# r-barnes/richdem

Hardware: NVIDIA H100
Metric: Priority-Flood fill + D8 flow accumulation throughput (higher is better)
Workload: dtype f32

## Files before the change

### include/richdem_b200.h

```cpp
#ifndef RICHDEM_B200_H_
#define RICHDEM_B200_H_

#include <stdint.h>

#ifdef __cplusplus
extern "C" {
#endif

#define RDB200_VERSION 100

#if defined(__GNUC__)
#define RDB200_API __attribute__((visibility("default")))
#else
#define RDB200_API
#endif


RDB200_API int rdb200_init(int device);
RDB200_API void rdb200_shutdown(void);
RDB200_API const char *rdb200_last_error(void);
RDB200_API int rdb200_version(void);

RDB200_API int rdb200_set_stream(void *cuda_stream);

typedef struct rdb200_stats {
  int64_t cells;
  int64_t kernel_launches;
  int64_t fill_rounds;
  int64_t fill_tile_visits;
  int64_t fill_tile_cells;
  int64_t fill_tile_iters;
  int64_t accum_rounds;
  int64_t flat_bfs_levels;
  int64_t flat_cells_raised;
  double ms_total;
  double ms_main_kernel;
  double ms_h2d, ms_d2h;
} rdb200_stats;
RDB200_API int rdb200_get_stats(rdb200_stats *out);

RDB200_API int rdb200_set_param(const char *name, int64_t value);


RDB200_API int rdb200_fill_depressions_d8_f32(float *dem, int32_t width, int32_t height);

RDB200_API int rdb200_fill_depressions_d4_f32(float *dem, int32_t width, int32_t height);

RDB200_API int rdb200_pit_mask_d8_f32(const float *dem, uint8_t *mask, int32_t width, int32_t height, float nodata);
RDB200_API int rdb200_pit_mask_d4_f32(const float *dem, uint8_t *mask, int32_t width, int32_t height, float nodata);

RDB200_API int rdb200_has_depressions_d8_f32(const float *dem, int32_t width, int32_t height, int32_t *out);
RDB200_API int rdb200_has_depressions_d4_f32(const float *dem, int32_t width, int32_t height, int32_t *out);

RDB200_API int rdb200_resolve_flats_epsilon_f32(float *dem, int32_t width, int32_t height, float nodata);

RDB200_API int rdb200_get_flat_mask_f32(const float *dem, int32_t *flat_mask, int32_t *labels, int32_t width,
                             int32_t height, float nodata);

RDB200_API int rdb200_d8_flow_directions_f32(const float *dem, uint8_t *flowdirs, int32_t width,
                                  int32_t height, float nodata);

RDB200_API int rdb200_d8_flow_directions_flats_f32(float *dem, uint8_t *flowdirs, int32_t width, int32_t height,
                                                   float nodata, int32_t alter);

RDB200_API int rdb200_d8_flow_accum_u8_i32(const uint8_t *flowdirs, int32_t *area, int32_t width,
                                int32_t height);

RDB200_API int rdb200_fm_d8_f32(const float *dem, float *props9, int32_t width, int32_t height, float nodata);

RDB200_API int rdb200_fm_tarboton_f32(const float *dem, float *props9, int32_t width, int32_t height,
                           float nodata);

RDB200_API int rdb200_fm_d4_f32(const float *dem, float *props9, int32_t width, int32_t height, float nodata);
RDB200_API int rdb200_fm_quinn_f32(const float *dem, float *props9, int32_t width, int32_t height, float nodata);
RDB200_API int rdb200_fm_holmgren_f32(const float *dem, float *props9, int32_t width, int32_t height, float nodata,
                                      double xparam);
RDB200_API int rdb200_fm_freeman_f32(const float *dem, float *props9, int32_t width, int32_t height, float nodata,
                                     double xparam);

RDB200_API int rdb200_fa_d4_f32_f64(const float *dem, double *accum_inout, int32_t width, int32_t height, float nodata);
RDB200_API int rdb200_fa_quinn_f32_f64(const float *dem, double *accum_inout, int32_t width, int32_t height,
                                       float nodata);
RDB200_API int rdb200_fa_holmgren_f32_f64(const float *dem, double *accum_inout, int32_t width, int32_t height,
                                          float nodata, double xparam);
RDB200_API int rdb200_fa_freeman_f32_f64(const float *dem, double *accum_inout, int32_t width, int32_t height,
                                         float nodata, double xparam);

RDB200_API int rdb200_fill_depressions_d8_f64(double *dem, int32_t width, int32_t height);
RDB200_API int rdb200_fill_depressions_d4_f64(double *dem, int32_t width, int32_t height);
RDB200_API int rdb200_pit_mask_d8_f64(const double *dem, uint8_t *mask, int32_t width, int32_t height, double nodata);
RDB200_API int rdb200_pit_mask_d4_f64(const double *dem, uint8_t *mask, int32_t width, int32_t height, double nodata);
RDB200_API int rdb200_has_depressions_d8_f64(const double *dem, int32_t width, int32_t height, int32_t *out);
RDB200_API int rdb200_has_depressions_d4_f64(const double *dem, int32_t width, int32_t height, int32_t *out);
RDB200_API int rdb200_resolve_flats_epsilon_f64(double *dem, int32_t width, int32_t height, double nodata);
RDB200_API int rdb200_d8_flow_directions_f64(const double *dem, uint8_t *flowdirs, int32_t width, int32_t height,
                                             double nodata);
RDB200_API int rdb200_fa_d8_f64_f64(const double *dem, double *accum_inout, int32_t width, int32_t height, double nodata,
                                    int32_t accum_is_ones);
RDB200_API int rdb200_fa_d4_f64_f64(const double *dem, double *accum_inout, int32_t width, int32_t height, double nodata);
RDB200_API int rdb200_f64_order_keys(const double *dem, float *keys, int32_t width, int32_t height, double nodata,
                                     float *nodata_key, int32_t *ranked);

enum {
  RDB200_TA_SLOPE_RISERUN = 0,
  RDB200_TA_SLOPE_PERCENTAGE = 1,
  RDB200_TA_SLOPE_DEGREES = 2,
  RDB200_TA_SLOPE_RADIANS = 3,
  RDB200_TA_ASPECT = 4,
  RDB200_TA_CURVATURE = 5,
  RDB200_TA_PLANFORM_CURVATURE = 6,
  RDB200_TA_PROFILE_CURVATURE = 7
};
RDB200_API int rdb200_terrain_attribute_f32(int32_t attribute, const float *dem, float *out, int32_t width, int32_t height,
                                            float nodata_in, float nodata_out, float zscale, double cell_x, double cell_y);

RDB200_API int rdb200_flow_accumulation_props_f64(const float *props9, double *accum_inout, int32_t width,
                                       int32_t height);

RDB200_API int rdb200_fa_d8_f32_f64(const float *dem, double *accum_inout, int32_t width, int32_t height,
                         float nodata, int32_t accum_is_ones);
RDB200_API int rdb200_fa_tarboton_f32_f64(const float *dem, double *accum_inout, int32_t width,
                               int32_t height, float nodata, int32_t accum_is_ones);


RDB200_API int rdb200_dev_fill_depressions_d8_f32(float *d_dem, int32_t width, int32_t height);
RDB200_API int rdb200_dev_fill_depressions_d4_f32(float *d_dem, int32_t width, int32_t height);
RDB200_API int rdb200_dev_pit_mask_d8_f32(const float *d_dem, uint8_t *d_mask, int32_t width, int32_t height, float nodata);
RDB200_API int rdb200_dev_pit_mask_d4_f32(const float *d_dem, uint8_t *d_mask, int32_t width, int32_t height, float nodata);
RDB200_API int rdb200_dev_has_depressions_d8_f32(const float *d_dem, int32_t width, int32_t height, int32_t *out);
RDB200_API int rdb200_dev_has_depressions_d4_f32(const float *d_dem, int32_t width, int32_t height, int32_t *out);
RDB200_API int rdb200_dev_resolve_flats_epsilon_f32(float *d_dem, int32_t width, int32_t height, float nodata);
RDB200_API int rdb200_dev_d8_flow_directions_f32(const float *d_dem, uint8_t *d_flowdirs, int32_t width,
                                      int32_t height, float nodata);
RDB200_API int rdb200_dev_d8_flow_directions_flats_f32(float *d_dem, uint8_t *d_flowdirs, int32_t width, int32_t height,
                                                       float nodata, int32_t alter);
RDB200_API int rdb200_dev_d8_flow_accum_u8_i32(const uint8_t *d_flowdirs, int32_t *d_area, int32_t width,
                                    int32_t height);
RDB200_API int rdb200_dev_fm_d8_f32(const float *d_dem, float *d_props9, int32_t width, int32_t height,
                         float nodata);
RDB200_API int rdb200_dev_fm_tarboton_f32(const float *d_dem, float *d_props9, int32_t width, int32_t height,
                               float nodata);
RDB200_API int rdb200_dev_fm_method_f32(int32_t method, const float *d_dem, float *d_props9, int32_t width,
                                        int32_t height, float nodata, double xparam);
RDB200_API int rdb200_dev_fa_method_f32_f64(int32_t method, const float *d_dem, double *d_accum_inout, int32_t width,
                                            int32_t height, float nodata, double xparam);
RDB200_API int rdb200_dev_terrain_attribute_f32(int32_t attribute, const float *d_dem, float *d_out, int32_t width,
                                                int32_t height, float nodata_in, float nodata_out, float zscale,
                                                double cell_x, double cell_y);
RDB200_API int rdb200_dev_flow_accumulation_props_f64(const float *d_props9, double *d_accum_inout,
                                           int32_t width, int32_t height);
RDB200_API int rdb200_dev_fa_d8_f32_f64(const float *d_dem, double *d_accum_inout, int32_t width,
                             int32_t height, float nodata, int32_t accum_is_ones);
RDB200_API int rdb200_dev_fa_tarboton_f32_f64(const float *d_dem, double *d_accum_inout, int32_t width,
                                   int32_t height, float nodata, int32_t accum_is_ones);
RDB200_API int rdb200_dev_fill_depressions_d8_f64(double *d_dem, int32_t width, int32_t height);
RDB200_API int rdb200_dev_fill_depressions_d4_f64(double *d_dem, int32_t width, int32_t height);
RDB200_API int rdb200_dev_pit_mask_d8_f64(const double *d_dem, uint8_t *d_mask, int32_t width, int32_t height, double nodata);
RDB200_API int rdb200_dev_pit_mask_d4_f64(const double *d_dem, uint8_t *d_mask, int32_t width, int32_t height, double nodata);
RDB200_API int rdb200_dev_has_depressions_d8_f64(const double *d_dem, int32_t width, int32_t height, int32_t *out);
RDB200_API int rdb200_dev_has_depressions_d4_f64(const double *d_dem, int32_t width, int32_t height, int32_t *out);
RDB200_API int rdb200_dev_resolve_flats_epsilon_f64(double *d_dem, int32_t width, int32_t height, double nodata);
RDB200_API int rdb200_dev_d8_flow_directions_f64(const double *d_dem, uint8_t *d_flowdirs, int32_t width, int32_t height,
                                                 double nodata);
RDB200_API int rdb200_dev_fa_d8_f64_f64(const double *d_dem, double *d_accum_inout, int32_t width, int32_t height,
                                        double nodata, int32_t accum_is_ones);
RDB200_API int rdb200_dev_fa_d4_f64_f64(const double *d_dem, double *d_accum_inout, int32_t width, int32_t height,
                                        double nodata);
RDB200_API int rdb200_dev_f64_order_keys(const double *d_dem, float *d_keys, int32_t width, int32_t height, double nodata,
                                         float *nodata_key, int32_t *ranked);

RDB200_API int rdb200_dev_generate_fbm_f32(float *d_dem, int32_t width, int32_t height, int32_t y0,
                                uint32_t seed, int32_t octaves, float quantum);

typedef struct rdb200_comm rdb200_comm;
enum { RDB200_MAX_F32 = 0, RDB200_MIN_F32 = 1, RDB200_MAX_I32 = 2, RDB200_SUM_I32 = 3 };
typedef int (*rdb200_exchange_fn)(void *user, const void *send_up, void *recv_up, const void *send_dn, void *recv_dn,
                                  size_t bytes);
typedef int (*rdb200_allreduce_fn)(void *user, void *buf, size_t count, int op);
RDB200_API int rdb200_nccl_unique_id(uint8_t *out128);
RDB200_API int rdb200_comm_create_nccl(rdb200_comm **comm, int32_t rank, int32_t world, const uint8_t *id128);
RDB200_API int rdb200_comm_create_callbacks(rdb200_comm **comm, int32_t rank, int32_t world, void *user,
                                            rdb200_exchange_fn exchange, rdb200_allreduce_fn allreduce);
RDB200_API int rdb200_comm_destroy(rdb200_comm *comm);

RDB200_API int rdb200_mgpu_fill_depressions_d8_f32(const rdb200_comm *comm, float *d_band, int32_t width, int32_t local_rows,
                                                   int32_t ghost_top, int32_t ghost_bottom, int32_t row0, int32_t height,
                                                   int32_t *exchange_rounds);
RDB200_API int rdb200_mgpu_fill_depressions_d4_f32(const rdb200_comm *comm, float *d_band, int32_t width, int32_t local_rows,
                                                   int32_t ghost_top, int32_t ghost_bottom, int32_t row0, int32_t height,
                                                   int32_t *exchange_rounds);
RDB200_API int rdb200_mgpu_pit_mask_d8_f32(const rdb200_comm *comm, const float *d_band, uint8_t *d_band_mask, int32_t width,
                                           int32_t local_rows, float nodata, int32_t ghost_top, int32_t ghost_bottom, int32_t row0,
                                           int32_t height);
RDB200_API int rdb200_mgpu_pit_mask_d4_f32(const rdb200_comm *comm, const float *d_band, uint8_t *d_band_mask, int32_t width,
                                           int32_t local_rows, float nodata, int32_t ghost_top, int32_t ghost_bottom, int32_t row0,
                                           int32_t height);
RDB200_API int rdb200_mgpu_has_depressions_d8_f32(const rdb200_comm *comm, const float *d_band, int32_t width, int32_t local_rows,
                                                  int32_t ghost_top, int32_t ghost_bottom, int32_t row0, int32_t height,
                                                  int32_t *out);
RDB200_API int rdb200_mgpu_has_depressions_d4_f32(const rdb200_comm *comm, const float *d_band, int32_t width, int32_t local_rows,
                                                  int32_t ghost_top, int32_t ghost_bottom, int32_t row0, int32_t height,
                                                  int32_t *out);
RDB200_API int rdb200_mgpu_resolve_flats_epsilon_f32(const rdb200_comm *comm, float *d_band, int32_t width, int32_t local_rows,
                                                     float nodata, int32_t ghost_top, int32_t ghost_bottom,
                                                     int32_t *seam_iterations);
RDB200_API int rdb200_mgpu_fa_f32_f64(const rdb200_comm *comm, const float *d_band_dem, double *d_band_accum_inout,
                                      int32_t width, int32_t local_rows, float nodata, int32_t ghost_top,
                                      int32_t ghost_bottom, int32_t dinf, int32_t accum_is_ones, int32_t *exchange_rounds);
RDB200_API int rdb200_mgpu_fa_method_f32_f64(const rdb200_comm *comm, const float *d_band_dem, double *d_band_accum_inout,
                                             int32_t width, int32_t local_rows, float nodata, int32_t ghost_top,
                                             int32_t ghost_bottom, int32_t method, double xparam, int32_t accum_is_ones,
                                             int32_t *exchange_rounds);
RDB200_API int rdb200_mgpu_d8_flow_directions_flats_f32(const rdb200_comm *comm, float *d_band_dem, uint8_t *d_band_dirs,
                                                        int32_t width, int32_t local_rows, float nodata, int32_t ghost_top,
                                                        int32_t ghost_bottom, int32_t alter, int32_t *seam_iterations);
RDB200_API int rdb200_mgpu_d8_flow_accum_u8_i32(const rdb200_comm *comm, const uint8_t *d_band_dirs, int32_t *d_band_area,
                                                int32_t width, int32_t local_rows, int32_t ghost_top, int32_t ghost_bottom,
                                                int32_t *exchange_rounds);
RDB200_API int rdb200_mgpu_fm_method_f32(const rdb200_comm *comm, int32_t method, float *d_band_dem, float *d_band_props9,
                                         int32_t width, int32_t local_rows, float nodata, int32_t ghost_top, int32_t ghost_bottom,
                                         double xparam);
RDB200_API int rdb200_mgpu_terrain_attribute_f32(const rdb200_comm *comm, int32_t attribute, float *d_band_dem, float *d_band_out,
                                                 int32_t width, int32_t local_rows, float nodata_in, float nodata_out, float zscale,
                                                 double cell_x, double cell_y, int32_t ghost_top, int32_t ghost_bottom);
RDB200_API int rdb200_mgpu_flow_accumulation_props_f64(const rdb200_comm *comm, float *d_band_props9, double *d_band_accum_inout,
                                                       int32_t width, int32_t local_rows, int32_t ghost_top, int32_t ghost_bottom,
                                                       int32_t *exchange_rounds);

typedef struct rdb200_fill_state rdb200_fill_state;
RDB200_API int rdb200_dev_fill_begin(rdb200_fill_state **state, const float *d_dem, int32_t width,
                          int32_t height);
RDB200_API int rdb200_dev_fill_begin_lifted(rdb200_fill_state **state, const float *d_dem, int32_t width, int32_t height,
                                 const float *d_coarse, int32_t coarse_width, int32_t pool, int32_t row_offset);
RDB200_API int rdb200_dev_fill_blockmax(rdb200_fill_state *state, float *d_blockmax, int32_t coarse_width, int32_t coarse_height,
                             int32_t pool, int32_t row_offset, int32_t skip_top, int32_t skip_bottom);
RDB200_API int rdb200_dev_fill_relax_from_f32(const float *d_dem, float *d_w_inout, int32_t width, int32_t height);
RDB200_API int rdb200_dev_fill_prolong(rdb200_fill_state *state, const float *d_coarse, int32_t coarse_width, int32_t pool,
                            int32_t row_offset, int32_t *tiles_lowered);
RDB200_API int rdb200_dev_maxpool_rows_f32(const float *d_src, int32_t width, int32_t height, int32_t row_offset, int32_t pool,
                                float *d_coarse, int32_t coarse_width, int32_t coarse_height);
RDB200_API int rdb200_dev_fill_run(rdb200_fill_state *state, int32_t *changed_rows);
RDB200_API int rdb200_dev_fill_read_row(rdb200_fill_state *state, int32_t y, float *d_row);
RDB200_API int rdb200_dev_fill_update_row(rdb200_fill_state *state, int32_t y, const float *d_row);
RDB200_API int rdb200_dev_fill_finish(rdb200_fill_state *state, float *d_out);

typedef struct rdb200_facc_state rdb200_facc_state;
RDB200_API int rdb200_dev_facc_begin(rdb200_facc_state **state, const float *d_dem, double *d_accum_inout,
                                     int32_t width, int32_t height, float nodata, int32_t ghost_top,
                                     int32_t ghost_bottom, int32_t dinf, int32_t accum_is_ones);
RDB200_API int rdb200_dev_facc_begin_method(rdb200_facc_state **state, const float *d_dem, double *d_accum_inout,
                                            int32_t width, int32_t height, float nodata, int32_t ghost_top,
                                            int32_t ghost_bottom, int32_t method, double xparam, int32_t accum_is_ones);
RDB200_API int rdb200_dev_facc_get_edge_codes(rdb200_facc_state *state, int32_t which, uint8_t *d_code_row,
                                              float *d_rmax_row);
RDB200_API int rdb200_dev_facc_set_ghost_codes(rdb200_facc_state *state, int32_t which,
                                               const uint8_t *d_code_row, const float *d_rmax_row);
RDB200_API int rdb200_dev_facc_run(rdb200_facc_state *state, int32_t *sent_top, int32_t *sent_bottom);
RDB200_API int rdb200_dev_facc_take_outflow(rdb200_facc_state *state, int32_t which, double *d_sum_row,
                                            int32_t *d_cnt_row);
RDB200_API int rdb200_dev_facc_apply_inflow(rdb200_facc_state *state, int32_t which, const double *d_sum_row,
                                            const int32_t *d_cnt_row);
RDB200_API int rdb200_dev_facc_finish(rdb200_facc_state *state);

typedef struct rdb200_flats_state rdb200_flats_state;
RDB200_API int rdb200_dev_flats_begin(rdb200_flats_state **state, float *d_dem, int32_t width, int32_t height,
                                      float nodata, int32_t ghost_top, int32_t ghost_bottom);
RDB200_API int rdb200_dev_flats_arrays(rdb200_flats_state *state, uint64_t *out6);
RDB200_API int rdb200_dev_flats_edges(rdb200_flats_state *state);
RDB200_API int rdb200_dev_flats_components(rdb200_flats_state *state);
RDB200_API int rdb200_dev_flats_labels(rdb200_flats_state *state);
RDB200_API int rdb200_dev_flats_gradient_begin(rdb200_flats_state *state, int32_t away,
                                               rdb200_fill_state **dist_state);
RDB200_API int rdb200_dev_flats_gradient_end(rdb200_flats_state *state, int32_t away,
                                             rdb200_fill_state *dist_state);
RDB200_API int rdb200_dev_flats_apply(rdb200_flats_state *state);
RDB200_API int rdb200_dev_flats_finish(rdb200_flats_state *state);

#ifdef __cplusplus
}
#endif
#endif
```

### richdem_b200/_lib.py

```python
from __future__ import annotations

import ctypes as C
import os

import numpy as np

_HERE = os.path.dirname(os.path.abspath(__file__))
LIB_PATH = os.environ.get("RICHDEM_B200_LIB") or os.path.join(_HERE, "librichdem_b200.so")

_lib = None


class RichdemB200Error(RuntimeError):
    """Raised for any non-zero status from the C ABI (mirrors the std::runtime_error ->
    RuntimeError translation pybind11 does for the reference, pywrapper.hpp:109-123)."""


class Stats(C.Structure):
    _fields_ = [
        ("cells", C.c_int64), ("kernel_launches", C.c_int64), ("fill_rounds", C.c_int64),
        ("fill_tile_visits", C.c_int64), ("fill_tile_cells", C.c_int64), ("fill_tile_iters", C.c_int64),
        ("accum_rounds", C.c_int64), ("flat_bfs_levels", C.c_int64), ("flat_cells_raised", C.c_int64),
        ("ms_total", C.c_double), ("ms_main_kernel", C.c_double), ("ms_h2d", C.c_double),
        ("ms_d2h", C.c_double),
    ]

    def as_dict(self):
        return {k: getattr(self, k) for k, _ in self._fields_}


_i32, _f32, _f64, _vp = C.c_int32, C.c_float, C.c_double, C.c_void_p
SIGNATURES = {
    "rdb200_init": [C.c_int],
    "rdb200_set_stream": [C.c_void_p],
    "rdb200_get_stats": [C.POINTER(Stats)],
    "rdb200_set_param": [C.c_char_p, C.c_int64],
    "rdb200_fill_depressions_d8_f32": [_vp, _i32, _i32],
    "rdb200_fill_depressions_d4_f32": [_vp, _i32, _i32],
    "rdb200_dev_fill_depressions_d4_f32": [_vp, _i32, _i32],
    "rdb200_pit_mask_d8_f32": [_vp, _vp, _i32, _i32, _f32],
    "rdb200_pit_mask_d4_f32": [_vp, _vp, _i32, _i32, _f32],
    "rdb200_has_depressions_d8_f32": [_vp, _i32, _i32, C.POINTER(_i32)],
    "rdb200_has_depressions_d4_f32": [_vp, _i32, _i32, C.POINTER(_i32)],
    "rdb200_dev_pit_mask_d8_f32": [_vp, _vp, _i32, _i32, _f32],
    "rdb200_dev_pit_mask_d4_f32": [_vp, _vp, _i32, _i32, _f32],
    "rdb200_dev_has_depressions_d8_f32": [_vp, _i32, _i32, C.POINTER(_i32)],
    "rdb200_dev_has_depressions_d4_f32": [_vp, _i32, _i32, C.POINTER(_i32)],
    "rdb200_mgpu_pit_mask_d8_f32": [_vp, _vp, _vp, _i32, _i32, _f32, _i32, _i32, _i32, _i32],
    "rdb200_mgpu_pit_mask_d4_f32": [_vp, _vp, _vp, _i32, _i32, _f32, _i32, _i32, _i32, _i32],
    "rdb200_mgpu_has_depressions_d8_f32": [_vp, _vp, _i32, _i32, _i32, _i32, _i32, _i32, C.POINTER(_i32)],
    "rdb200_mgpu_has_depressions_d4_f32": [_vp, _vp, _i32, _i32, _i32, _i32, _i32, _i32, C.POINTER(_i32)],
    "rdb200_resolve_flats_epsilon_f32": [_vp, _i32, _i32, _f32],
    "rdb200_get_flat_mask_f32": [_vp, _vp, _vp, _i32, _i32, _f32],
    "rdb200_d8_flow_directions_f32": [_vp, _vp, _i32, _i32, _f32],
    "rdb200_d8_flow_directions_flats_f32": [_vp, _vp, _i32, _i32, _f32, _i32],
    "rdb200_dev_d8_flow_directions_flats_f32": [_vp, _vp, _i32, _i32, _f32, _i32],
    "rdb200_d8_flow_accum_u8_i32": [_vp, _vp, _i32, _i32],
    "rdb200_fm_d8_f32": [_vp, _vp, _i32, _i32, _f32],
    "rdb200_fm_tarboton_f32": [_vp, _vp, _i32, _i32, _f32],
    "rdb200_fm_d4_f32": [_vp, _vp, _i32, _i32, _f32],
    "rdb200_fm_quinn_f32": [_vp, _vp, _i32, _i32, _f32],
    "rdb200_fm_holmgren_f32": [_vp, _vp, _i32, _i32, _f32, C.c_double],
    "rdb200_fm_freeman_f32": [_vp, _vp, _i32, _i32, _f32, C.c_double],
    "rdb200_terrain_attribute_f32": [_i32, _vp, _vp, _i32, _i32, _f32, _f32, _f32, C.c_double, C.c_double],
    "rdb200_dev_terrain_attribute_f32": [_i32, _vp, _vp, _i32, _i32, _f32, _f32, _f32, C.c_double, C.c_double],
    "rdb200_fa_d4_f32_f64": [_vp, _vp, _i32, _i32, _f32],
    "rdb200_fa_quinn_f32_f64": [_vp, _vp, _i32, _i32, _f32],
    "rdb200_fa_holmgren_f32_f64": [_vp, _vp, _i32, _i32, _f32, C.c_double],
    "rdb200_fa_freeman_f32_f64": [_vp, _vp, _i32, _i32, _f32, C.c_double],
    "rdb200_dev_fm_method_f32": [_i32, _vp, _vp, _i32, _i32, _f32, C.c_double],
    "rdb200_dev_fa_method_f32_f64": [_i32, _vp, _vp, _i32, _i32, _f32, C.c_double],
    "rdb200_flow_accumulation_props_f64": [_vp, _vp, _i32, _i32],
    "rdb200_fa_d8_f32_f64": [_vp, _vp, _i32, _i32, _f32, _i32],
    "rdb200_fa_tarboton_f32_f64": [_vp, _vp, _i32, _i32, _f32, _i32],
    "rdb200_dev_fill_depressions_d8_f32": [_vp, _i32, _i32],
    "rdb200_dev_resolve_flats_epsilon_f32": [_vp, _i32, _i32, _f32],
    "rdb200_dev_d8_flow_directions_f32": [_vp, _vp, _i32, _i32, _f32],
    "rdb200_dev_d8_flow_accum_u8_i32": [_vp, _vp, _i32, _i32],
    "rdb200_dev_fm_d8_f32": [_vp, _vp, _i32, _i32, _f32],
    "rdb200_dev_fm_tarboton_f32": [_vp, _vp, _i32, _i32, _f32],
    "rdb200_dev_flow_accumulation_props_f64": [_vp, _vp, _i32, _i32],
    "rdb200_dev_fa_d8_f32_f64": [_vp, _vp, _i32, _i32, _f32, _i32],
    "rdb200_dev_fa_tarboton_f32_f64": [_vp, _vp, _i32, _i32, _f32, _i32],
    "rdb200_fill_depressions_d8_f64": [_vp, _i32, _i32],
    "rdb200_fill_depressions_d4_f64": [_vp, _i32, _i32],
    "rdb200_pit_mask_d8_f64": [_vp, _vp, _i32, _i32, _f64],
    "rdb200_pit_mask_d4_f64": [_vp, _vp, _i32, _i32, _f64],
    "rdb200_has_depressions_d8_f64": [_vp, _i32, _i32, C.POINTER(_i32)],
    "rdb200_has_depressions_d4_f64": [_vp, _i32, _i32, C.POINTER(_i32)],
    "rdb200_resolve_flats_epsilon_f64": [_vp, _i32, _i32, _f64],
    "rdb200_d8_flow_directions_f64": [_vp, _vp, _i32, _i32, _f64],
    "rdb200_fa_d8_f64_f64": [_vp, _vp, _i32, _i32, _f64, _i32],
    "rdb200_fa_d4_f64_f64": [_vp, _vp, _i32, _i32, _f64],
    "rdb200_f64_order_keys": [_vp, _vp, _i32, _i32, _f64, C.POINTER(_f32), C.POINTER(_i32)],
    "rdb200_dev_fill_depressions_d8_f64": [_vp, _i32, _i32],
    "rdb200_dev_fill_depressions_d4_f64": [_vp, _i32, _i32],
    "rdb200_dev_pit_mask_d8_f64": [_vp, _vp, _i32, _i32, _f64],
    "rdb200_dev_pit_mask_d4_f64": [_vp, _vp, _i32, _i32, _f64],
    "rdb200_dev_has_depressions_d8_f64": [_vp, _i32, _i32, C.POINTER(_i32)],
    "rdb200_dev_has_depressions_d4_f64": [_vp, _i32, _i32, C.POINTER(_i32)],
    "rdb200_dev_resolve_flats_epsilon_f64": [_vp, _i32, _i32, _f64],
    "rdb200_dev_d8_flow_directions_f64": [_vp, _vp, _i32, _i32, _f64],
    "rdb200_dev_fa_d8_f64_f64": [_vp, _vp, _i32, _i32, _f64, _i32],
    "rdb200_dev_fa_d4_f64_f64": [_vp, _vp, _i32, _i32, _f64],
    "rdb200_dev_f64_order_keys": [_vp, _vp, _i32, _i32, _f64, C.POINTER(_f32), C.POINTER(_i32)],
    "rdb200_dev_generate_fbm_f32": [_vp, _i32, _i32, _i32, C.c_uint32, _i32, _f32],
    "rdb200_nccl_unique_id": [_vp],
    "rdb200_comm_create_nccl": [C.POINTER(_vp), _i32, _i32, _vp],
    "rdb200_comm_create_callbacks": [C.POINTER(_vp), _i32, _i32, _vp, _vp, _vp],
    "rdb200_comm_destroy": [_vp],
    "rdb200_mgpu_fill_depressions_d8_f32": [_vp, _vp, _i32, _i32, _i32, _i32, _i32, _i32, C.POINTER(_i32)],
    "rdb200_mgpu_fill_depressions_d4_f32": [_vp, _vp, _i32, _i32, _i32, _i32, _i32, _i32, C.POINTER(_i32)],
    "rdb200_mgpu_fa_f32_f64": [_vp, _vp, _vp, _i32, _i32, _f32, _i32, _i32, _i32, _i32, C.POINTER(_i32)],
    "rdb200_mgpu_fa_method_f32_f64": [_vp, _vp, _vp, _i32, _i32, _f32, _i32, _i32, _i32, C.c_double, _i32, C.POINTER(_i32)],
    "rdb200_mgpu_resolve_flats_epsilon_f32": [_vp, _vp, _i32, _i32, _f32, _i32, _i32, C.POINTER(_i32)],
    "rdb200_mgpu_d8_flow_directions_flats_f32": [_vp, _vp, _vp, _i32, _i32, _f32, _i32, _i32, _i32, C.POINTER(_i32)],
    "rdb200_mgpu_d8_flow_accum_u8_i32": [_vp, _vp, _vp, _i32, _i32, _i32, _i32, C.POINTER(_i32)],
    "rdb200_mgpu_fm_method_f32": [_vp, _i32, _vp, _vp, _i32, _i32, _f32, _i32, _i32, C.c_double],
    "rdb200_mgpu_terrain_attribute_f32": [_vp, _i32, _vp, _vp, _i32, _i32, _f32, _f32, _f32, C.c_double, C.c_double, _i32, _i32],
    "rdb200_mgpu_flow_accumulation_props_f64": [_vp, _vp, _vp, _i32, _i32, _i32, _i32, C.POINTER(_i32)],
    "rdb200_dev_fill_begin": [C.POINTER(_vp), _vp, _i32, _i32],
    "rdb200_dev_fill_begin_lifted": [C.POINTER(_vp), _vp, _i32, _i32, _vp, _i32, _i32, _i32],
    "rdb200_dev_maxpool_rows_f32": [_vp, _i32, _i32, _i32, _i32, _vp, _i32, _i32],
    "rdb200_dev_fill_blockmax": [_vp, _vp, _i32, _i32, _i32, _i32, _i32, _i32],
    "rdb200_dev_fill_relax_from_f32": [_vp, _vp, _i32, _i32],
    "rdb200_dev_fill_prolong": [_vp, _vp, _i32, _i32, _i32, C.POINTER(C.c_int32)],
    "rdb200_dev_fill_run": [_vp, C.POINTER(_i32)],
    "rdb200_dev_fill_read_row": [_vp, _i32, _vp],
    "rdb200_dev_fill_update_row": [_vp, _i32, _vp],
    "rdb200_dev_fill_finish": [_vp, _vp],
    "rdb200_dev_facc_begin": [C.POINTER(_vp), _vp, _vp, _i32, _i32, _f32, _i32, _i32, _i32, _i32],
    "rdb200_dev_facc_begin_method": [C.POINTER(_vp), _vp, _vp, _i32, _i32, _f32, _i32, _i32, _i32, C.c_double, _i32],
    "rdb200_dev_facc_get_edge_codes": [_vp, _i32, _vp, _vp],
    "rdb200_dev_facc_set_ghost_codes": [_vp, _i32, _vp, _vp],
    "rdb200_dev_facc_run": [_vp, C.POINTER(_i32), C.POINTER(_i32)],
    "rdb200_dev_facc_take_outflow": [_vp, _i32, _vp, _vp],
    "rdb200_dev_facc_apply_inflow": [_vp, _i32, _vp, _vp],
    "rdb200_dev_facc_finish": [_vp],
    "rdb200_dev_flats_begin": [C.POINTER(_vp), _vp, _i32, _i32, _f32, _i32, _i32],
    "rdb200_dev_flats_arrays": [_vp, C.POINTER(C.c_uint64)],
    "rdb200_dev_flats_edges": [_vp],
    "rdb200_dev_flats_components": [_vp],
    "rdb200_dev_flats_labels": [_vp],
    "rdb200_dev_flats_gradient_begin": [_vp, _i32, C.POINTER(_vp)],
    "rdb200_dev_flats_gradient_end": [_vp, _i32, _vp],
    "rdb200_dev_flats_apply": [_vp],
    "rdb200_dev_flats_finish": [_vp],
}
OTHER_SYMBOLS = ["rdb200_shutdown", "rdb200_last_error", "rdb200_version"]


def lib():
    global _lib
    if _lib is None:
        if not os.path.exists(LIB_PATH):
            raise RichdemB200Error(
                f"{LIB_PATH} not found: build it with `python -m richdem_b200.build` "
                "(there is no CPU fallback)")
        L = C.CDLL(LIB_PATH)
        if hasattr(L, "rdb200_emulated"):
            raise RichdemB200Error(
                f"{LIB_PATH} is the CPU kernel-emulation test build, not librichdem_b200 "
                "(there is no CPU fallback)")
        for name, argtypes in SIGNATURES.items():
            f = getattr(L, name)
            f.argtypes = argtypes
            f.restype = C.c_int
        L.rdb200_last_error.restype = C.c_char_p
        L.rdb200_last_error.argtypes = []
        L.rdb200_version.restype = C.c_int
        L.rdb200_shutdown.restype = None
        _lib = L
        for kv in filter(None, os.environ.get("RDB200_PARAMS", "").split(",")):
            k, _, v = kv.partition("=")
            if L.rdb200_set_param(k.strip().encode(), int(v)):
                msg = L.rdb200_last_error()
                raise RichdemB200Error(f"RDB200_PARAMS: {msg.decode('utf-8', 'replace') if msg else kv}")
    return _lib


def check(rc: int) -> None:
    if rc != 0:
        msg = lib().rdb200_last_error()
        raise RichdemB200Error(msg.decode("utf-8", "replace") if msg else f"librichdem_b200 error {rc}")


def ptr(a: np.ndarray) -> int:
    return a.ctypes.data


def stats() -> dict:
    s = Stats()
    check(lib().rdb200_get_stats(C.byref(s)))
    return s.as_dict()


_param_values: dict = {}


def set_param(name: str, value: int) -> None:
    check(lib().rdb200_set_param(name.encode(), int(value)))
    if name == "reset_defaults":
        _param_values.clear()
    elif name != "trim_workspace":
        _param_values[name] = int(value)


def reset_params() -> None:
    set_param("reset_defaults", 1)


class scoped_param:

    def __init__(self, name: str, value: int, default: int = 0):
        self.name, self.value, self.default = name, int(value), int(default)

    def __enter__(self):
        self.previous = _param_values.get(self.name)
        set_param(self.name, self.value)
        return self

    def __exit__(self, *exc):
        if self.previous is None:
            set_param(self.name, self.default)
            _param_values.pop(self.name, None)
        else:
            set_param(self.name, self.previous)
        return False


def init(device: int = 0) -> None:
    check(lib().rdb200_init(int(device)))


def set_stream(cuda_stream) -> None:
    if cuda_stream is None:
        check(lib().rdb200_set_stream(C.c_void_p(None)))
    else:
        h = int(cuda_stream)
        check(lib().rdb200_set_stream(C.c_void_p(h if h != 0 else 1)))


def use_torch_stream() -> None:
    import torch
    set_stream(torch.cuda.current_stream().cuda_stream)


def shutdown() -> None:
    lib().rdb200_shutdown()
```

### richdem_b200/csrc/capi.cu

```cuda
#include "common.cuh"

#include <algorithm>
#include <cstdlib>

namespace rdb {

static thread_local std::string g_last_error;

void capi_set_error(const char *msg) { g_last_error = msg ? msg : "unknown error"; }

Ctx &ctx() {
  static Ctx c;
  return c;
}

static void init_device(int device) {
  Ctx &c = ctx();
  if (c.inited && c.device == device) return;
  if (c.inited) fail("rdb200_init: already initialised on device %d (call rdb200_shutdown first)", c.device);
  int ndev = 0;
  cudaError_t e = cudaGetDeviceCount(&ndev);
  if (e != cudaSuccess || ndev == 0)
    fail("no CUDA device available (%s); librichdem_b200 has no CPU fallback",
         e == cudaSuccess ? "device count is 0" : cudaGetErrorString(e));
  if (device < 0 || device >= ndev) fail("rdb200_init: device %d out of range (0..%d)", device, ndev - 1);
  RDB_CK(cudaSetDevice(device));
  cudaDeviceProp prop;
  RDB_CK(cudaGetDeviceProperties(&prop, device));
  if (prop.major != 9 || prop.minor != 0)
    fail("device %d is sm_%d%d; librichdem_b200 is built for sm_90a (H100) only", device, prop.major,
         prop.minor);
  c.device = device;
  c.num_sms = prop.multiProcessorCount;
  RDB_CK(cudaStreamCreate(&c.own_stream));
  c.stream = c.own_stream;
  RDB_CK(cudaEventCreate(&c.ev0));
  RDB_CK(cudaEventCreate(&c.ev1));
  RDB_CK(cudaEventCreate(&c.evk0));
  RDB_CK(cudaEventCreate(&c.evk1));
  c.pinned_bytes = 1 << 16;
  RDB_CK(cudaMallocHost(&c.pinned, c.pinned_bytes));
  memset(&c.stats, 0, sizeof(c.stats));
  c.inited = true;
}

void ensure_init() {
  Ctx &c = ctx();
  if (c.inited) {
    RDB_CK(cudaSetDevice(c.device));
    return;
  }
  int dev = 0;
  cudaError_t e = cudaGetDevice(&dev);
  if (e != cudaSuccess) dev = 0;
  init_device(dev);
}

void *ws_alloc(size_t bytes) {
  Ctx &c = ctx();
  bytes = (bytes + 511) & ~(size_t)511;
  int best = -1;
  for (int i = 0; i < (int)c.ws.size(); i++)
    if (!c.ws[i].in_use && c.ws[i].bytes >= bytes && (best < 0 || c.ws[i].bytes < c.ws[best].bytes)) best = i;
  if (best >= 0 && c.ws[best].bytes <= bytes + bytes / 4 + (1 << 20)) {
    c.ws[best].in_use = true;
    return c.ws[best].ptr;
  }
  void *p = nullptr;
  cudaError_t e = cudaMalloc(&p, bytes);
  if (e != cudaSuccess) {
    cudaGetLastError();
    for (auto it = c.ws.begin(); it != c.ws.end();) {
      if (!it->in_use) {
        cudaFree(it->ptr);
        it = c.ws.erase(it);
      } else {
        ++it;
      }
    }
    e = cudaMalloc(&p, bytes);
    if (e != cudaSuccess) fail("cudaMalloc(%zu bytes) failed: %s", bytes, cudaGetErrorString(e));
  }
  c.ws.push_back({p, bytes, true});
  return p;
}

void ws_free(void *p) {
  for (auto &b : ctx().ws)
    if (b.ptr == p) {
      b.in_use = false;
      return;
    }
}

void ws_trim() {
  Ctx &c = ctx();
  for (auto it = c.ws.begin(); it != c.ws.end();) {
    if (!it->in_use) {
      cudaFree(it->ptr);
      it = c.ws.erase(it);
    } else {
      ++it;
    }
  }
}

void ws_release_all() {
  Ctx &c = ctx();
  for (auto &b : c.ws) cudaFree(b.ptr);
  c.ws.clear();
}

struct CallScope {
  explicit CallScope(int64_t cells) {
    ensure_init();
    Ctx &c = ctx();
    memset(&c.stats, 0, sizeof(c.stats));
    c.stats.cells = cells;
    RDB_CK(cudaEventRecord(c.ev0, c.stream));
  }
  void done() {
    Ctx &c = ctx();
    RDB_CK(cudaEventRecord(c.ev1, c.stream));
    RDB_CK(cudaStreamSynchronize(c.stream));
    float ms = 0;
    RDB_CK(cudaEventElapsedTime(&ms, c.ev0, c.ev1));
    c.stats.ms_total = ms;
  }
};

static void check_dims(int w, int h) {
  if (w <= 0 || h <= 0) fail("raster dimensions must be positive (got %d x %d)", w, h);
  if ((int64_t)w * h > ((int64_t)1 << 31) - ((int64_t)1 << 25))
    fail("rasters above 2^31 - 2^25 cells per GPU are not supported (got %d x %d); shard by rows", w, h);
}

template <class T>
static void h2d(T *dst, const T *src, size_t n) {
  Ctx &c = ctx();
  cudaEvent_t a = c.evk0, b = c.evk1;
  RDB_CK(cudaEventRecord(a, c.stream));
  RDB_CK(cudaMemcpyAsync(dst, src, n * sizeof(T), cudaMemcpyHostToDevice, c.stream));
  RDB_CK(cudaEventRecord(b, c.stream));
  RDB_CK(cudaStreamSynchronize(c.stream));
  float ms = 0;
  RDB_CK(cudaEventElapsedTime(&ms, a, b));
  c.stats.ms_h2d += ms;
}
template <class T>
static void d2h(T *dst, const T *src, size_t n) {
  Ctx &c = ctx();
  cudaEvent_t a = c.evk0, b = c.evk1;
  RDB_CK(cudaEventRecord(a, c.stream));
  RDB_CK(cudaMemcpyAsync(dst, src, n * sizeof(T), cudaMemcpyDeviceToHost, c.stream));
  RDB_CK(cudaEventRecord(b, c.stream));
  RDB_CK(cudaStreamSynchronize(c.stream));
  float ms = 0;
  RDB_CK(cudaEventElapsedTime(&ms, a, b));
  c.stats.ms_d2h += ms;
}

}

using namespace rdb;

#define CAPI_TRY try {
#define CAPI_END                    \
  }                                 \
  catch (const std::exception &e) { \
    capi_set_error(e.what());       \
    return 1;                       \
  }                                 \
  catch (...) {                     \
    capi_set_error("unknown C++ exception"); \
    return 1;                       \
  }                                 \
  return 0;

extern "C" {

int rdb200_init(int device) {
  CAPI_TRY
  init_device(device);
  CAPI_END
}

void rdb200_shutdown(void) {
  Ctx &c = ctx();
  if (!c.inited) return;
  cudaSetDevice(c.device);
  cudaStreamSynchronize(c.stream);
  ws_release_all();
  if (c.pinned) cudaFreeHost(c.pinned);
  cudaEventDestroy(c.ev0);
  cudaEventDestroy(c.ev1);
  cudaEventDestroy(c.evk0);
  cudaEventDestroy(c.evk1);
  cudaStreamDestroy(c.own_stream);
  for (int k = 0; k < 2; k++)
    if (c.aux_stream[k]) cudaStreamDestroy(c.aux_stream[k]);
  for (int k = 0; k < 3; k++)
    if (c.aux_event[k]) cudaEventDestroy(c.aux_event[k]);
  const Params keep = c.params;
  c = Ctx();
  c.params = keep;
}

const char *rdb200_last_error(void) { return g_last_error.c_str(); }
int rdb200_version(void) { return RDB200_VERSION; }

int rdb200_set_stream(void *cuda_stream) {
  CAPI_TRY
  ensure_init();
  Ctx &c = ctx();
  RDB_CK(cudaStreamSynchronize(c.stream));
  c.stream = cuda_stream ? (cudaStream_t)cuda_stream : c.own_stream;
  CAPI_END
}

int rdb200_get_stats(rdb200_stats *out) {
  CAPI_TRY
  if (!out) fail("rdb200_get_stats: null pointer");
  *out = ctx().stats;
  CAPI_END
}

int rdb200_set_param(const char *name, int64_t value) {
  CAPI_TRY
  if (!name) fail("rdb200_set_param: null name");
  Params &p = ctx().params;
  const std::string n(name);
  if (n == "reset_defaults") p = Params();
  else if (n == "trim_workspace") {
    if (ctx().inited) {
      RDB_CK(cudaStreamSynchronize(ctx().stream));
      ws_trim();
    }
  }
  else if (n == "fill_max_iters") p.fill_max_iters = value;
  else if (n == "fill_rounds_per_sync") p.fill_rounds_per_sync = value > 0 ? value : 16;
  else if (n == "fill_use_tma") p.fill_use_tma = value;
  else if (n == "fill_external_z") p.fill_external_z = value;
  else if (n == "fill_profile") p.fill_profile = value;
  else if (n == "fill_wake_filter") p.fill_wake_filter = value;
  else if (n == "fill_trace") p.fill_trace = value;
  else if (n == "fill_ordered") p.fill_ordered = value;
  else if (n == "fill_order_rounds") p.fill_order_rounds = value;
  else if (n == "fill_band_rounds") p.fill_band_rounds = value;
  else if (n == "accum_threads") p.accum_threads = value > 0 ? value : 256;
  else if (n == "accum_budget") p.accum_budget = value;
  else if (n == "accum_walk_lanes") p.accum_walk_lanes = value;
  else if (n == "accum_fused_prep") p.accum_fused_prep = value;
  else if (n == "flats_tiled") p.flats_tiled = value;
  else if (n == "flats_pair") p.flats_pair = value;
  else if (n == "flats_fused_classify") p.flats_fused_classify = value;
  else if (n == "fill_multigrid") p.fill_multigrid = value;
  else if (n == "fill_multigrid_min") p.fill_multigrid_min = value;
  else if (n == "fill_vcycle") p.fill_vcycle = value;
  else if (n == "fill_band_multigrid") p.fill_band_multigrid = value;
  else if (n == "flats_uf_tiled") p.flats_uf_tiled = value;
  else if (n == "flowdirs_rolling") p.flowdirs_rolling = value;
  else if (n == "accum_packed") p.accum_packed = value;
  else if (n == "accum_dinf_packed") p.accum_dinf_packed = value;
  else if (n == "accum_dinf_share") p.accum_dinf_share = value;
  else if (n == "flowmet_tarboton_filter") p.flowmet_tarboton_filter = value;
  else if (n == "accum_walk_scan") p.accum_walk_scan = value;
  else if (n == "accum_walk_ahead") p.accum_walk_ahead = value;
  else if (n == "accum_dinf_stats") p.accum_dinf_stats = value;
  else if (n == "accum_dinf_wait") p.accum_dinf_wait = value;
  else fail("rdb200_set_param: unknown parameter '%s'", name);
  CAPI_END
}


int rdb200_fill_depressions_d8_f32(float *dem, int32_t w, int32_t h) {
  CAPI_TRY
  if (!dem) fail("fill_depressions: null dem");
  check_dims(w, h);
  CallScope cs((int64_t)w * h);
  const size_t n = (size_t)w * h;
  DevBuf<float> d(n);
  h2d(d.p, dem, n);
  fill_depressions_dev(d.p, w, h);
  d2h(dem, d.p, n);
  cs.done();
  CAPI_END
}

int rdb200_fill_depressions_d4_f32(float *dem, int32_t w, int32_t h) {
  CAPI_TRY
  if (!dem) fail("fill_depressions: null dem");
  check_dims(w, h);
  CallScope cs((int64_t)w * h);
  const size_t n = (size_t)w * h;
  DevBuf<float> d(n);
  h2d(d.p, dem, n);
  fill_depressions_dev(d.p, w, h, true);
  d2h(dem, d.p, n);
  cs.done();
  CAPI_END
}

static int pit_mask_host(const float *dem, uint8_t *mask, int32_t w, int32_t h, float nodata, bool topo4) {
  CAPI_TRY
  if (!dem || !mask) fail("pit_mask: null pointer");
  check_dims(w, h);
  CallScope cs((int64_t)w * h);
  const size_t n = (size_t)w * h;
  DevBuf<float> d(n);
  DevBuf<uint8_t> m(n);
  h2d(d.p, dem, n);
  pit_mask_dev(d.p, m.p, w, h, nodata, topo4);
  d2h(mask, m.p, n);
  cs.done();
  CAPI_END
}
int rdb200_pit_mask_d8_f32(const float *dem, uint8_t *mask, int32_t w, int32_t h, float nodata) {
  return pit_mask_host(dem, mask, w, h, nodata, false);
}
int rdb200_pit_mask_d4_f32(const float *dem, uint8_t *mask, int32_t w, int32_t h, float nodata) {
  return pit_mask_host(dem, mask, w, h, nodata, true);
}

static int has_depressions_host(const float *dem, int32_t w, int32_t h, int32_t *out, bool topo4) {
  CAPI_TRY
  if (!dem || !out) fail("has_depressions: null pointer");
  check_dims(w, h);
  CallScope cs((int64_t)w * h);
  const size_t n = (size_t)w * h;
  DevBuf<float> d(n);
  h2d(d.p, dem, n);
  const bool any = has_depressions_dev(d.p, w, h, topo4);
  cs.done();
  *out = any ? 1 : 0;
  CAPI_END
}
int rdb200_has_depressions_d8_f32(const float *dem, int32_t w, int32_t h, int32_t *out) {
  return has_depressions_host(dem, w, h, out, false);
}
int rdb200_has_depressions_d4_f32(const float *dem, int32_t w, int32_t h, int32_t *out) {
  return has_depressions_host(dem, w, h, out, true);
}

int rdb200_resolve_flats_epsilon_f32(float *dem, int32_t w, int32_t h, float nodata) {
  CAPI_TRY
  if (!dem) fail("resolve_flats: null dem");
  check_dims(w, h);
  CallScope cs((int64_t)w * h);
  const size_t n = (size_t)w * h;
  DevBuf<float> d(n);
  h2d(d.p, dem, n);
  resolve_flats_dev(d.p, w, h, nodata, nullptr, nullptr, true);
  d2h(dem, d.p, n);
  cs.done();
  CAPI_END
}

int rdb200_get_flat_mask_f32(const float *dem, int32_t *flat_mask, int32_t *labels, int32_t w, int32_t h,
                             float nodata) {
  CAPI_TRY
  if (!dem || !flat_mask || !labels) fail("get_flat_mask: null pointer");
  check_dims(w, h);
  CallScope cs((int64_t)w * h);
  const size_t n = (size_t)w * h;
  DevBuf<float> d(n);
  DevBuf<int32_t> m(n), l(n);
  h2d(d.p, dem, n);
  resolve_flats_dev(d.p, w, h, nodata, m.p, l.p, false);
  d2h(flat_mask, m.p, n);
  d2h(labels, l.p, n);
  cs.done();
  CAPI_END
}

int rdb200_d8_flow_directions_f32(const float *dem, uint8_t *dirs, int32_t w, int32_t h, float nodata) {
  CAPI_TRY
  if (!dem || !dirs) fail("d8_flow_directions: null pointer");
  check_dims(w, h);
  CallScope cs((int64_t)w * h);
  const size_t n = (size_t)w * h;
  DevBuf<float> d(n);
  DevBuf<uint8_t> o(n);
  h2d(d.p, dem, n);
  d8_flow_directions_dev(d.p, o.p, w, h, nodata);
  d2h(dirs, o.p, n);
  cs.done();
  CAPI_END
}

int rdb200_d8_flow_directions_flats_f32(float *dem, uint8_t *dirs, int32_t w, int32_t h, float nodata, int32_t alter) {
  CAPI_TRY
  if (!dem || !dirs) fail("d8_flow_directions_flats: null pointer");
  check_dims(w, h);
  CallScope cs((int64_t)w * h);
  const size_t n = (size_t)w * h;
  DevBuf<float> d(n);
  DevBuf<uint8_t> o(n);
  h2d(d.p, dem, n);
  d8_flow_directions_flats_dev(d.p, o.p, w, h, nodata, alter != 0);
  d2h(dirs, o.p, n);
  if (alter) d2h(dem, d.p, n);
  cs.done();
  CAPI_END
}

int rdb200_d8_flow_accum_u8_i32(const uint8_t *dirs, int32_t *area, int32_t w, int32_t h) {
  CAPI_TRY
  if (!dirs || !area) fail("d8_flow_accum: null pointer");
  check_dims(w, h);
  CallScope cs((int64_t)w * h);
  const size_t n = (size_t)w * h;
  DevBuf<uint8_t> d(n);
  DevBuf<int32_t> o(n);
  h2d(d.p, dirs, n);
  d8_flow_accum_dev(d.p, o.p, w, h);
  d2h(area, o.p, n);
  cs.done();
  CAPI_END
}

static void fm_dispatch_dev(int method, const float *d_dem, float *d_props, int w, int h, float nodata, double xparam) {
  switch (method) {
    case 0: fm_d8_dev(d_dem, d_props, w, h, nodata); break;
    case 1: fm_tarboton_dev(d_dem, d_props, w, h, nodata); break;
    case 2: fm_d4_dev(d_dem, d_props, w, h, nodata); break;
    case 3: fm_holmgren_dev(d_dem, d_props, w, h, nodata, xparam); break;
    case 4: fm_freeman_dev(d_dem, d_props, w, h, nodata, xparam); break;
    default: fail("unknown flow metric %d", method);
  }
}

static int fm_host(const float *dem, float *props, int32_t w, int32_t h, float nodata, int method, double xparam = 0) {
  CAPI_TRY
  if (!dem || !props) fail("flow metric: null pointer");
  check_dims(w, h);
  CallScope cs((int64_t)w * h);
  const size_t n = (size_t)w * h;
  DevBuf<float> d(n), p(9 * n);
  h2d(d.p, dem, n);
  fm_dispatch_dev(method, d.p, p.p, w, h, nodata, xparam);
  d2h(props, p.p, 9 * n);
  cs.done();
  CAPI_END
}
int rdb200_fm_d8_f32(const float *dem, float *props, int32_t w, int32_t h, float nodata) {
  return fm_host(dem, props, w, h, nodata, 0);
}
int rdb200_fm_tarboton_f32(const float *dem, float *props, int32_t w, int32_t h, float nodata) {
  return fm_host(dem, props, w, h, nodata, 1);
}
int rdb200_fm_d4_f32(const float *dem, float *props, int32_t w, int32_t h, float nodata) {
  return fm_host(dem, props, w, h, nodata, 2);
}
int rdb200_fm_quinn_f32(const float *dem, float *props, int32_t w, int32_t h, float nodata) {
  return fm_host(dem, props, w, h, nodata, 3, 1.0);
}
int rdb200_fm_holmgren_f32(const float *dem, float *props, int32_t w, int32_t h, float nodata, double xparam) {
  return fm_host(dem, props, w, h, nodata, 3, xparam);
}
int rdb200_fm_freeman_f32(const float *dem, float *props, int32_t w, int32_t h, float nodata, double xparam) {
  return fm_host(dem, props, w, h, nodata, 4, xparam);
}

int rdb200_terrain_attribute_f32(int32_t attribute, const float *dem, float *out, int32_t w, int32_t h, float nodata_in,
                                 float nodata_out, float zscale, double cell_x, double cell_y) {
  CAPI_TRY
  if (!dem || !out) fail("terrain attribute: null pointer");
  check_dims(w, h);
  CallScope cs((int64_t)w * h);
  const size_t n = (size_t)w * h;
  DevBuf<float> d(n), o(n);
  h2d(d.p, dem, n);
  terrain_attribute_dev(attribute, d.p, o.p, w, h, nodata_in, nodata_out, zscale, cell_x, cell_y);
  d2h(out, o.p, n);
  cs.done();
  CAPI_END
}

static void fa_via_props_dev(int method, const float *d_dem, double *d_accum, int w, int h, float nodata, double xparam) {
  DevBuf<float> p(9 * (size_t)w * h);
  fm_dispatch_dev(method, d_dem, p.p, w, h, nodata, xparam);
  flow_accumulation_props_dev(p.p, d_accum, w, h);
}
static int fa_via_props_host(int method, const float *dem, double *accum, int32_t w, int32_t h, float nodata, double xparam) {
  CAPI_TRY
  if (!dem || !accum) fail("flow accumulation: null pointer");
  check_dims(w, h);
  CallScope cs((int64_t)w * h);
  const size_t n = (size_t)w * h;
  DevBuf<float> d(n);
  DevBuf<double> a(n);
  h2d(d.p, dem, n);
  h2d(a.p, accum, n);
  fa_via_props_dev(method, d.p, a.p, w, h, nodata, xparam);
  d2h(accum, a.p, n);
  cs.done();
  CAPI_END
}
int rdb200_fa_d4_f32_f64(const float *dem, double *accum, int32_t w, int32_t h, float nodata) {
  return fa_via_props_host(2, dem, accum, w, h, nodata, 0);
}
int rdb200_fa_quinn_f32_f64(const float *dem, double *accum, int32_t w, int32_t h, float nodata) {
  return fa_via_props_host(3, dem, accum, w, h, nodata, 1.0);
}
int rdb200_fa_holmgren_f32_f64(const float *dem, double *accum, int32_t w, int32_t h, float nodata, double xparam) {
  return fa_via_props_host(3, dem, accum, w, h, nodata, xparam);
}
int rdb200_fa_freeman_f32_f64(const float *dem, double *accum, int32_t w, int32_t h, float nodata, double xparam) {
  return fa_via_props_host(4, dem, accum, w, h, nodata, xparam);
}

int rdb200_flow_accumulation_props_f64(const float *props, double *accum, int32_t w, int32_t h) {
  CAPI_TRY
  if (!props || !accum) fail("flow_accumulation: null pointer");
  check_dims(w, h);
  CallScope cs((int64_t)w * h);
  const size_t n = (size_t)w * h;
  DevBuf<float> p(9 * n);
  DevBuf<double> a(n);
  h2d(p.p, props, 9 * n);
  h2d(a.p, accum, n);
  flow_accumulation_props_dev(p.p, a.p, w, h);
  d2h(accum, a.p, n);
  cs.done();
  CAPI_END
}

static int fa_host(const float *dem, double *accum, int32_t w, int32_t h, float nodata, int32_t ones,
                   bool dinf) {
  CAPI_TRY
  if (!dem || !accum) fail("flow accumulation: null pointer");
  check_dims(w, h);
  CallScope cs((int64_t)w * h);
  const size_t n = (size_t)w * h;
  DevBuf<float> d(n);
  DevBuf<double> a(n);
  h2d(d.p, dem, n);
  if (!ones) h2d(a.p, accum, n);
  fa_fused_dev(d.p, a.p, w, h, nodata, ones != 0, dinf);
  d2h(accum, a.p, n);
  cs.done();
  CAPI_END
}
int rdb200_fa_d8_f32_f64(const float *dem, double *accum, int32_t w, int32_t h, float nodata, int32_t ones) {
  return fa_host(dem, accum, w, h, nodata, ones, false);
}
int rdb200_fa_tarboton_f32_f64(const float *dem, double *accum, int32_t w, int32_t h, float nodata,
// ... 487 lines not shown
```

### richdem_b200/csrc/common.cuh

```cuda
#pragma once

#include <cuda.h>
#include <cuda_runtime.h>

#include <cstdarg>
#include <cstdint>
#include <cstdio>
#include <cstring>
#include <stdexcept>
#include <string>
#include <vector>

#include "../../include/richdem_b200.h"

struct rdb200_fill_state;

namespace rdb {

struct Error : std::runtime_error {
  using std::runtime_error::runtime_error;
};

[[noreturn]] inline void fail(const char *fmt, ...) {
  char buf[1024];
  va_list ap;
  va_start(ap, fmt);
  vsnprintf(buf, sizeof(buf), fmt, ap);
  va_end(ap);
  throw Error(buf);
}

#define RDB_CK(expr)                                                                        \
  do {                                                                                      \
    cudaError_t _e = (expr);                                                                \
    if (_e != cudaSuccess)                                                                  \
      ::rdb::fail("%s failed at %s:%d: %s", #expr, __FILE__, __LINE__, cudaGetErrorString(_e)); \
  } while (0)

__host__ __device__ __forceinline__ int d8dx(int n) {
  return (int)((0x6a41u >> (2 * n)) & 3u) - 1;
}
__host__ __device__ __forceinline__ int d8dy(int n) {
  return (int)((0x2a405u >> (2 * n)) & 3u) - 1;
}

struct Params {
  int64_t fill_max_iters = 0;
  int64_t fill_rounds_per_sync = 16;
  int64_t fill_use_tma = 1;
  int64_t fill_external_z = 1;
  int64_t fill_ordered = 1;
  int64_t fill_order_rounds = 0;
  int64_t fill_band_rounds = 0;
  int64_t fill_profile = 0;
  int64_t fill_wake_filter = 1;
  int64_t fill_trace = 0;
  int64_t fill_multigrid = 8;
  int64_t fill_vcycle = 8;
  int64_t fill_band_multigrid = 0;
  int64_t fill_multigrid_min = 0;
  int64_t flowdirs_rolling = 1;
  int64_t flats_uf_tiled = 1;
  int64_t flats_fused_classify = 1;
  int64_t flats_pair = 1;
  int64_t flats_tiled = 1;
  int64_t accum_dinf_packed = 1;
  int64_t flowmet_tarboton_filter = 1;
  int64_t accum_walk_ahead = 0;
  int64_t accum_walk_scan = 0;
  int64_t accum_dinf_stats = 0;
  int64_t accum_dinf_share = -1;
  int64_t accum_dinf_wait = 0;
  int64_t accum_packed = 1;
  int64_t accum_fused_prep = 1;
  int64_t accum_walk_lanes = 1;
  int64_t accum_threads = 256;
  int64_t accum_budget = 0;
};

struct WsBlock {
  void *ptr;
  size_t bytes;
  bool in_use;
};

struct Ctx {
  bool inited = false;
  int device = -1;
  int num_sms = 0;
  cudaStream_t stream = nullptr;
  cudaStream_t own_stream = nullptr;
  cudaEvent_t ev0 = nullptr, ev1 = nullptr, evk0 = nullptr, evk1 = nullptr;
  cudaStream_t aux_stream[2] = {nullptr, nullptr};
  cudaEvent_t aux_event[3] = {nullptr, nullptr, nullptr};
  std::vector<WsBlock> ws;
  void *pinned = nullptr;
  size_t pinned_bytes = 0;
  rdb200_stats stats;
  Params params;
};

Ctx &ctx();
void ensure_init();
void *ws_alloc(size_t bytes);
void ws_free(void *p);
void ws_release_all();

template <class T>
struct DevBuf {
  T *p = nullptr;
  size_t n = 0;
  DevBuf() = default;
  explicit DevBuf(size_t count) { alloc(count); }
  void alloc(size_t count) {
    reset();
    n = count;
    p = (T *)ws_alloc((count ? count : 1) * sizeof(T));
  }
  void reset() {
    if (p) ws_free(p);
    p = nullptr;
    n = 0;
  }
  ~DevBuf() { reset(); }
  DevBuf(const DevBuf &) = delete;
  DevBuf &operator=(const DevBuf &) = delete;
  operator T *() const { return p; }
};

inline void count_launch(int64_t k = 1) { ctx().stats.kernel_launches += k; }

struct KernelTimer {
  bool active;
  explicit KernelTimer(bool on = true) : active(on) {
    if (active) RDB_CK(cudaEventRecord(ctx().evk0, ctx().stream));
  }
  void stop_async() {
    if (active) RDB_CK(cudaEventRecord(ctx().evk1, ctx().stream));
  }
  double ms() {
    float t = 0;
    if (active) RDB_CK(cudaEventElapsedTime(&t, ctx().evk0, ctx().evk1));
    return t;
  }
};

int comm_rank(const rdb200_comm *c);
int comm_world(const rdb200_comm *c);
void comm_exchange(const rdb200_comm *c, const void *send_up, void *recv_up, const void *send_dn, void *recv_dn, size_t bytes);
void comm_allreduce(const rdb200_comm *c, void *buf, size_t count, int op);
void check_band_args(const char *what, const rdb200_comm *comm, const void *d_band, int w, int hloc, int gt, int gb);
void exchange_band_rows(const rdb200_comm *comm, void *d_band, size_t elem, int w, int hloc, int gt, int gb);
void mgpu_fill_band(const rdb200_comm *comm, float *d_local, int w, int hloc, int gt, int gb, int row0, int H, int *xrounds,
                    bool topo4 = false);
void mgpu_fa_band(const rdb200_comm *comm, const float *d_dem, double *d_accum, int w, int hloc, float nodata, int gt, int gb,
                  int method, double xparam, bool ones, int *xrounds);
void mgpu_flow_accumulation_props_band(const rdb200_comm *comm, float *d_props, double *d_accum, int w, int hloc, int gt, int gb,
                                       int *xrounds);
void mgpu_resolve_flats_band(const rdb200_comm *comm, float *d_local, int w, int hloc, float nodata, int gt, int gb,
                             int *seam_iters);
void mgpu_d8_flow_directions_flats_band(const rdb200_comm *comm, float *d_dem, uint8_t *d_dirs, int w, int hloc, float nodata,
                                        int gt, int gb, bool alter, int *seam_iters);
void mgpu_d8_flow_accum_band(const rdb200_comm *comm, const uint8_t *d_dirs, int32_t *d_area, int w, int hloc, int gt, int gb,
                             int *xrounds);
int mgpu_relax_band(const rdb200_comm *comm, rdb200_fill_state *state, int gt, int gb, int R);

void fill_depressions_dev(float *d_dem, int w, int h, bool topo4 = false);
void geodesic_distance_dev(const uint8_t *d_open, int open_bit, float *d_w_inout, int w, int h);
void geodesic_distance_pair_dev(const uint8_t *d_open, int open_bit, float *d_wa, float *d_wb, int w, int h);
rdb200_fill_state *new_band_distance_state(const uint8_t *d_open, int open_bit, const float *d_winit, int w, int h,
                                           int ghost_top, int ghost_bottom);
void finish_band_distance_state(rdb200_fill_state *s, float *d_out);
void resolve_flats_dev(float *d_dem, int w, int h, float nodata, int32_t *d_mask_out,
                       int32_t *d_labels_out, bool apply, const uint8_t *d_dirs = nullptr);
void d8_flow_directions_flats_dev(float *d_dem, uint8_t *d_dirs, int w, int h, float nodata, bool alter);
void d8_flow_directions_dev(const float *d_dem, uint8_t *d_dirs, int w, int h, float nodata);
void d8_flow_accum_dev(const uint8_t *d_dirs, int32_t *d_area, int w, int h);
void fm_d8_dev(const float *d_dem, float *d_props, int w, int h, float nodata);
void fm_tarboton_dev(const float *d_dem, float *d_props, int w, int h, float nodata);
void fm_d4_dev(const float *d_dem, float *d_props, int w, int h, float nodata);
void fm_holmgren_dev(const float *d_dem, float *d_props, int w, int h, float nodata, double xparam);
void fm_freeman_dev(const float *d_dem, float *d_props, int w, int h, float nodata, double xparam);
void flow_accumulation_props_dev(const float *d_props, double *d_accum, int w, int h);
void fa_fused_dev(const float *d_dem, double *d_accum, int w, int h, float nodata, bool ones,
                  bool dinf);
void terrain_attribute_dev(int attribute_id, const float *d_dem, float *d_out, int w, int h, float nodata_in, float nodata_out,
                           float zscale, double cell_x, double cell_y);
void generate_fbm_dev(float *d_dem, int w, int h, int y0, uint32_t seed, int octaves, float quantum);
void pit_mask_dev(const float *d_dem, uint8_t *d_mask, int w, int h, float nodata, bool topo4);
bool has_depressions_dev(const float *d_dem, int w, int h, bool topo4);
void mgpu_pit_mask_band(const rdb200_comm *comm, const float *d_band, uint8_t *d_mask, int w, int hloc, float nodata, int gt,
                        int gb, int row0, int H, bool topo4);
bool mgpu_has_depressions_band(const rdb200_comm *comm, const float *d_band, int w, int hloc, int gt, int gb, int row0, int H,
                               bool topo4);
void pit_mask_compare_dev(const float *d_z, const float *d_l, uint8_t *d_mask, size_t n, float nodata, int *d_any);
void strict_pit_f64_dev(const double *d_z, int w, int h, bool topo4, int *d_flag);
void d8_flow_directions_f64_dev(const double *d_dem, uint8_t *d_dirs, int w, int h, double nodata);

float f64_keys_dev(const double *d_z, float *d_key, size_t n, double nodata, DevBuf<double> *table, int *ranked);
void fill_depressions_f64_dev(double *d_z, int w, int h, bool topo4);
void pit_mask_f64_dev(const double *d_z, uint8_t *d_mask, int w, int h, double nodata, bool topo4);
bool has_depressions_f64_dev(const double *d_z, int w, int h, bool topo4);
void resolve_flats_f64_dev(double *d_z, int w, int h, double nodata);
void fa_d8_f64_dev(const double *d_z, double *d_accum, int w, int h, double nodata, bool ones);

}
```

### richdem_b200/csrc/fill.cu

```cuda
#include "common.cuh"

#include <chrono>

namespace rdb {

namespace {

#ifndef RDB_TX
#define RDB_TX 64
#endif
#ifndef RDB_TY
#define RDB_TY 64
#endif
#ifndef RDB_FILL_THREADS
#define RDB_FILL_THREADS 128
#endif
#ifndef RDB_FILL_MIN_CTAS
#define RDB_FILL_MIN_CTAS 6
#endif
constexpr int TX = RDB_TX;
constexpr int TY = RDB_TY;
constexpr int BXN = TX / 4;
constexpr int BYN = TY / 4;
constexpr int PADL = 4;
constexpr int SP = TX + 2 * PADL;
constexpr int SROWS = TY + 2;
constexpr int FILL_THREADS = RDB_FILL_THREADS;
constexpr int FILL_MIN_CTAS = RDB_FILL_MIN_CTAS;
static_assert(BYN <= 16 && BXN * BYN <= 256 && TX % 4 == 0 && TY % 4 == 0, "tile shape");
constexpr uint32_t W_TILE_BYTES = SP * SROWS * 4;
constexpr uint32_t Z_TILE_BYTES = TX * TY * 4;

struct RoundCtl {
  int count;
  int take;
};

struct FillDev {
  RoundCtl ctl[3];
  RoundCtl proc[3];
  unsigned long long visits;
  unsigned long long iters;
  unsigned long long block_updates;
  unsigned long long warp_updates;
  unsigned long long idle_visits;
  unsigned long long wakes_dropped;
  unsigned long long iter_hist[8];
  int edge_changed;
  int zmin_ord, zmax_ord;
  unsigned long long deferred;
  unsigned long long live_rounds;
  float level, step, step_min, level_max;
  int target, ordered;
  int ndefer[3];
};

struct FillArgs {
  const float *Z;
  int zpitch, zox, zoy;
  int inplace;
  const float *coarse;
  int Wc, pool, yoff;
  int *staged;
  float *zcopy;
  float *Wp;
  int pitch;
  int wox, woy;
  int W, H;
  int tilesX, tilesY;
  int *list0, *list1;
  int *stamp;
  int *sides;
  int *keys;
  float level;
  int *plist;
  int use_proc;
  FillDev *dev;
  int round;
  int max_iters;
  int use_tma;
  int profile;
  int *dirty;
  unsigned long long *edge_above;
};

__device__ __forceinline__ uint32_t smem_u32(const void *p) {
  return (uint32_t)__cvta_generic_to_shared(p);
}
__device__ __forceinline__ void mbar_init(unsigned long long *bar, int count) {
  asm volatile("mbarrier.init.shared::cta.b64 [%0], %1;" ::"r"(smem_u32(bar)), "r"(count) : "memory");
}
__device__ __forceinline__ void mbar_arrive_expect_tx(unsigned long long *bar, uint32_t bytes) {
  asm volatile("mbarrier.arrive.expect_tx.shared::cta.b64 _, [%0], %1;" ::"r"(smem_u32(bar)),
               "r"(bytes)
               : "memory");
}
__device__ __forceinline__ void mbar_wait(unsigned long long *bar, uint32_t parity) {
  uint32_t ok;
  const uint32_t addr = smem_u32(bar);
  do {
    asm volatile(
        "{\n"
        "  .reg .pred p;\n"
        "  mbarrier.try_wait.parity.shared::cta.b64 p, [%1], %2;\n"
        "  selp.u32 %0, 1, 0, p;\n"
        "}\n"
        : "=r"(ok)
        : "r"(addr), "r"(parity)
        : "memory");
  } while (!ok);
}
__device__ __forceinline__ void tma_load_2d(void *smem_dst, const CUtensorMap *map, int c0, int c1,
                                            unsigned long long *bar) {
  asm volatile(
      "cp.async.bulk.tensor.2d.shared::cluster.global.mbarrier::complete_tx::bytes [%0], [%1, {%2, %3}], [%4];"
      ::"r"(smem_u32(smem_dst)),
      "l"((unsigned long long)map), "r"(c0), "r"(c1), "r"(smem_u32(bar))
      : "memory");
}
__device__ __forceinline__ void fence_proxy_async() {
  asm volatile("fence.proxy.async.shared::cta;" ::: "memory");
}
__device__ __forceinline__ void tma_store_2d(const CUtensorMap *map, int c0, int c1, const void *smem_src) {
  asm volatile("cp.async.bulk.tensor.2d.global.shared::cta.bulk_group [%0, {%1, %2}], [%3];" ::"l"((unsigned long long)map),
               "r"(c0), "r"(c1), "r"(smem_u32(smem_src))
               : "memory");
  asm volatile("cp.async.bulk.commit_group;" ::: "memory");
}
__device__ __forceinline__ void bulk_wait_read() { asm volatile("cp.async.bulk.wait_group.read 0;" ::: "memory"); }
__device__ __forceinline__ void bulk_wait_all() { asm volatile("cp.async.bulk.wait_group 0;" ::: "memory"); }

constexpr int NBLK = BXN * BYN;
constexpr int MKP = BXN + 2;
constexpr int NWARP = FILL_THREADS / 32;
constexpr int SEG = ((NBLK + NWARP - 1) / NWARP + 31) / 32 * 32;
enum : int { SIDE_N = 1, SIDE_S = 2, SIDE_W = 4, SIDE_E = 8, SIDE_NW = 16, SIDE_NE = 32, SIDE_SW = 64,
             SIDE_SE = 128, SIDE_FULL = 256 };

__host__ __device__ __forceinline__ int f2ord(float f) {
  int b;
  memcpy(&b, &f, 4);
  return b >= 0 ? b : (b ^ 0x7fffffff);
}
__host__ __device__ __forceinline__ float ord2f(int o) {
  const int b = o >= 0 ? o : (o ^ 0x7fffffff);
  float f;
  memcpy(&f, &b, 4);
  return f;
}
constexpr int ORD_POS_INF = 0x7f800000;

__device__ __forceinline__ void enqueue_tile(const FillArgs &a, RoundCtl *next, int *list_next, int t,
                                             int stampval, int side_bits, int key_ord) {
  atomicOr(&a.sides[(stampval & 1) * a.tilesX * a.tilesY + t], side_bits);
  atomicMin(&a.keys[(stampval & 1) * a.tilesX * a.tilesY + t], key_ord);
  if (atomicExch(&a.stamp[t], stampval) != stampval) {
    const int idx = atomicAdd(&next->count, 1);
    list_next[idx] = t;
  }
}

__device__ __forceinline__ float min3f(float a, float b, float c) { return fminf(fminf(a, b), c); }

constexpr bool WAKE_WORDS = TX <= 64 && TY <= 64;

struct EdgeLine {
  int len, o, st, da, zo, zs;
};
__device__ __forceinline__ EdgeLine edge_line(int s) {
  switch (s) {
    case 0: return {TX, SP + PADL, 1, -SP, 0, 1};
    case 1: return {TX, TY * SP + PADL, 1, SP, (TY - 1) * TX, 1};
    case 2: return {TY, SP + PADL, SP, -1, 0, TX};
    default: return {TY, SP + PADL + TX - 1, SP, 1, TX - 1, TX};
  }
}

constexpr bool DRAIN_SWEEPS = TX == 64 && TY == 64 && FILL_THREADS == 128;

template <bool TOPO4>
__device__ __forceinline__ void fill_drain_sweeps(float *sW, const float *sZ, int y0, int H, int *sFlags, int *sKey) {
  const unsigned FULL = 0xffffffffu;
  const int tid = threadIdx.x, lane = tid & 31, wrp = tid >> 5;
  const int x = 32 * (wrp & 1) + lane;
  const bool down = wrp < 2;
  const int dy = down ? 1 : -1;
  const bool ecol = x < 4 || x >= TX - 4;
  unsigned long long rows = 0;
  float kmin = __int_as_float(0x7f800000);
  int y = down ? 0 : TY - 1;
  float p = sW[(y - dy + 1) * SP + PADL + x];
#pragma unroll 1
  for (int half = 0; half < 2; half++) {
#pragma unroll 8
    for (int s = 0; s < TY / 2; s++, y += dy) {
      const float zz = sZ[y * TX + x];
      float *cell = &sW[(y + 1) * SP + PADL + x];
      const float w = *cell;
      float m = p;
      if (!TOPO4) {
        float pl = __shfl_up_sync(FULL, p, 1), pr = __shfl_down_sync(FULL, p, 1);
        const float *prow = &sW[(y - dy + 1) * SP + PADL + x];
        if (lane == 0) pl = prow[-1];
        if (lane == 31) pr = prow[1];
        m = min3f(pl, p, pr);
      }
      const float nw = fminf(w, fmaxf(zz, m));
      p = w;
      if (nw < w) {
        *cell = nw;
        p = nw;
        rows |= 1ull << y;
        if (ecol || y < 4 || y >= TY - 4) kmin = fminf(kmin, nw);
      }
    }
    __syncthreads();
  }
  int f = 0;
#pragma unroll
  for (int by = 0; by < BYN; by++)
    if ((rows >> (4 * by)) & 0xFull) f |= 1 << (12 + by);
  if (rows & 1ull) f |= SIDE_N;
  if (rows >> (TY - 1)) f |= SIDE_S;
  if (x == 0 && rows) f |= SIDE_W | (rows & 1ull ? SIDE_NW : 0) | (rows >> (TY - 1) ? SIDE_SW : 0);
  if (x == TX - 1 && rows) f |= SIDE_E | (rows & 1ull ? SIDE_NE : 0) | (rows >> (TY - 1) ? SIDE_SE : 0);
  const int j1 = 1 - y0, j2 = (H - 2) - y0;
  if (j1 >= 0 && j1 < TY && ((rows >> j1) & 1ull)) f |= 1 << 9;
  if (j2 >= 0 && j2 < TY && ((rows >> j2) & 1ull)) f |= 1 << 10;
#pragma unroll
  for (int o = 16; o > 0; o >>= 1) {
    f |= __shfl_xor_sync(FULL, f, o);
    kmin = fminf(kmin, __shfl_xor_sync(FULL, kmin, o));
  }
  if (lane == 0 && f) {
    atomicOr(sFlags, f);
    if (f & 0xFF) atomicMin(sKey, f2ord(kmin));
  }
}

#ifndef __noinline__
#define __noinline__ __attribute__((noinline))
#endif
template <bool TOPO4>
__device__ __noinline__ void fill_wake_neighbours(const FillArgs &a, const float *sW, const float *sZ, int t, int fl, int key,
                                                  RoundCtl *next, int *list_next) {
  const unsigned FULL = 0xffffffffu;
  const int lane = threadIdx.x & 31;
  const int tyT = t / a.tilesX, txT = t - tyT * a.tilesX;
  const bool n_ok = tyT > 0, s_ok = tyT < a.tilesY - 1, w_ok = txT > 0, e_ok = txT < a.tilesX - 1;
  const int sv = a.round + 1;
  for (int s = threadIdx.x >> 5; s < 4; s += NWARP) {
    const EdgeLine e = edge_line(s);
    unsigned long long word = 0;
    for (int i0 = 0; i0 < e.len; i0 += 32) {
      const int i = i0 + lane;
      const bool above = i < e.len && !(sW[e.o + i * e.st] == sZ[e.zo + i * e.zs]);
      word |= (unsigned long long)__ballot_sync(FULL, above) << i0;
    }
    if (lane == 0) __stcg(&a.edge_above[(size_t)t * 4 + s], word);
    if (!((fl >> 12) & 0xFFFF)) continue;
    if (!TOPO4 && lane == 1 && (fl & (SIDE_NW << s))) {
      const bool north = s < 2, west = (s & 1) == 0;
      if ((north ? n_ok : s_ok) && (west ? w_ok : e_ok)) {
        const int nb = t + (north ? -a.tilesX : a.tilesX) + (west ? -1 : 1);
        const int own = (north ? SP : TY * SP) + PADL + (west ? 0 : TX - 1);
        const int across = own + (north ? -SP : SP) + (west ? -1 : 1);
        const unsigned long long nword = __ldcg(&a.edge_above[(size_t)nb * 4 + (north ? 1 : 0)]);
        if (((nword >> (west ? TX - 1 : 0)) & 1ull) && sW[own] < sW[across])
          enqueue_tile(a, next, list_next, nb, sv, SIDE_NW << (3 - s), key);
        else if (a.profile)
          atomicAdd(&a.dev->wakes_dropped, 1ull);
      }
    }
    if (!((fl >> s) & 1) || !(s == 0 ? n_ok : s == 1 ? s_ok : s == 2 ? w_ok : e_ok)) continue;
    const int nb = s == 0 ? t - a.tilesX : s == 1 ? t + a.tilesX : s == 2 ? t - 1 : t + 1;
    const unsigned long long nword = __ldcg(&a.edge_above[(size_t)nb * 4 + (s ^ 1)]);
    bool need = false;
    for (int i = lane; i < e.len; i += 32) {
      if (!((nword >> i) & 1ull)) continue;
      float m = sW[e.o + i * e.st];
      if (!TOPO4) {
        if (i > 0) m = fminf(m, sW[e.o + (i - 1) * e.st]);
        if (i < e.len - 1) m = fminf(m, sW[e.o + (i + 1) * e.st]);
      }
      need |= m < sW[e.o + i * e.st + e.da];
    }
    if (__ballot_sync(FULL, need)) {
      if (lane == 0) enqueue_tile(a, next, list_next, nb, sv, 1 << (s ^ 1), key);
    } else if (lane == 0 && a.profile) {
      atomicAdd(&a.dev->wakes_dropped, 1ull);
    }
  }
}

template <int STEP, bool TOPO4 = false, bool STAGE = false>
__global__ void __launch_bounds__(FILL_THREADS, FILL_MIN_CTAS)
    fill_sweep_kernel(const __grid_constant__ CUtensorMap mapW, const __grid_constant__ CUtensorMap mapZ,
                      const __grid_constant__ CUtensorMap mapZout, const __grid_constant__ FillArgs a) {
  __shared__ __align__(128) float sW[SROWS * SP];
  __shared__ __align__(128) float sZ[TY * TX];
  __shared__ __align__(8) unsigned long long mbar;
  __shared__ unsigned char sMark[MKP * (BYN + 2)];
  __shared__ unsigned char sList[2][NWARP][SEG];
  __shared__ __align__(16) int sCnt[2][NWARP];
  __shared__ int sTile;
  __shared__ int sFlags;
  __shared__ int sKey;
  __shared__ int sProf[2];
  __shared__ int sNbDone;

  const int tid = threadIdx.x;
  const int r = a.round;
  RoundCtl *cur = &a.dev->ctl[r % 3];
  RoundCtl *next = &a.dev->ctl[(r + 1) % 3];
  const int *list_cur = (r & 1) ? a.list1 : a.list0;
  int *list_next = (r & 1) ? a.list0 : a.list1;
  const int ntiles = a.tilesX * a.tilesY;
  if (a.use_proc) {
    cur = &a.dev->proc[r % 3];
    list_cur = a.plist;
  }
  const int n = cur->count;

  if (blockIdx.x == 0 && tid == 0) {
    RoundCtl *z = &a.dev->ctl[(r + 2) % 3];
    z->count = 0;
    z->take = 0;
    RoundCtl *zp = &a.dev->proc[(r + 1) % 3];
    zp->count = 0;
    zp->take = 0;
    if (n > 0) {
      atomicAdd(&a.dev->visits, (unsigned long long)n);
      a.dev->live_rounds++;
    }
  }
  if (n == 0) return;

  if (tid == 0) {
    mbar_init(&mbar, 1);
    asm volatile("fence.mbarrier_init.release.cluster;" ::: "memory");
  }
  uint32_t phase = 0;
  const int max_iters = a.max_iters;

  for (;;) {
    if (tid == 0) sTile = atomicAdd(&cur->take, 1);
    for (int k = tid; k < MKP * (BYN + 2); k += FILL_THREADS) sMark[k] = 0;
    __syncthreads();
    const int li = sTile;
    if (li >= n) break;
    const int t = list_cur[li];
    const int tyT = t / a.tilesX, txT = t - tyT * a.tilesX;
    const int x0 = txT * TX, y0 = tyT * TY;

    constexpr bool stage = STAGE;
    if (tid == 0) {
      sFlags = 0;
      sKey = ORD_POS_INF;
      sProf[0] = sProf[1] = 0;
      if (stage) {
        int nb = 0;
        for (int dy = -1; dy <= 1; dy++)
          for (int dx = -1; dx <= 1; dx++) {
            const int ty = tyT + dy, tx = txT + dx;
            if ((dx | dy) && ty >= 0 && ty < a.tilesY && tx >= 0 && tx < a.tilesX &&
                *reinterpret_cast<volatile int *>(&a.staged[ty * a.tilesX + tx]))
              nb |= 1 << ((dy + 1) * 3 + dx + 1);
          }
        __threadfence();
        sNbDone = nb;
      }
    }
    if (a.use_tma) {
      if (tid == 0) {
        fence_proxy_async();
        if (STAGE) bulk_wait_read();
        mbar_arrive_expect_tx(&mbar, (stage ? 0u : W_TILE_BYTES) + Z_TILE_BYTES);
        if (!stage) tma_load_2d(sW, &mapW, x0 - PADL + a.wox, y0 - 1 + a.woy, &mbar);
        tma_load_2d(sZ, &mapZ, x0 + a.zox, y0 + a.zoy, &mbar);
      }
    } else {
      const float inf = __int_as_float(0x7f800000);
      if (!stage) {
        for (int k = tid; k < SROWS * (SP / 4); k += FILL_THREADS) {
          const int rr = k / (SP / 4), cc = k - rr * (SP / 4);
          const int y = y0 + rr - 1, x = x0 + 4 * cc - PADL;
          reinterpret_cast<float4 *>(sW)[k] =
              a.inplace && (y < 0 || y >= a.H || x < 0 || x >= a.W)
                  ? make_float4(inf, inf, inf, inf)
                  : __ldcg(reinterpret_cast<const float4 *>(a.Wp + (size_t)(y + a.woy) * a.pitch + x + a.wox));
        }
      }
      for (int k = tid; k < TY * (TX / 4); k += FILL_THREADS) {
        const int rr = k / (TX / 4), cc = k - rr * (TX / 4);
        reinterpret_cast<float4 *>(sZ)[k] =
            a.inplace && (y0 + rr >= a.H || x0 + 4 * cc >= a.W)
                ? make_float4(inf, inf, inf, inf)
                : __ldg(reinterpret_cast<const float4 *>(a.Z + (size_t)(y0 + a.zoy + rr) * a.zpitch + x0 + a.zox) + cc);
      }
    }
    int sides = a.sides[(r & 1) * ntiles + t];
    __syncthreads();
    if (tid == 0) {
      a.sides[(r & 1) * ntiles + t] = 0;
      a.keys[(r & 1) * ntiles + t] = ORD_POS_INF;
    }
    if (stage) {
      const float inf = __int_as_float(0x7f800000);
      const int nbdone = sNbDone;
      constexpr int C4N = SP / 4, RSTEP = FILL_THREADS / C4N;
      static_assert(RSTEP >= 1, "a CTA covers one row of the window");
      if (tid < RSTEP * C4N) {
        const int c4 = 4 * (tid % C4N);
        int rr = tid / C4N;
        const int dx = c4 < PADL ? -1 : (c4 >= PADL + TX ? 1 : 0);
        const int xb = x0 + c4 - PADL;
        const int cx = xb >= 0 ? xb / a.pool : 0, rx = xb - cx * a.pool;
        const int yy = y0 + rr - 1 + a.yoff;
        int cy = (yy + a.pool) / a.pool - 1, ry = yy - cy * a.pool;
        const int dq = RSTEP / a.pool, dr = RSTEP - dq * a.pool;
        for (; rr < SROWS; rr += RSTEP) {
          const int dy = rr == 0 ? -1 : (rr == SROWS - 1 ? 1 : 0);
          float4 v4;
          if (((nbdone >> ((dy + 1) * 3 + dx + 1)) & 1) && y0 + rr - 1 < a.H && xb < a.W) {
            v4 = __ldcg(reinterpret_cast<const float4 *>(a.Wp + (size_t)(y0 + rr - 1 + a.woy) * a.pitch + xb + a.wox));
          } else {
            const int y = y0 + rr - 1;
            float v[4] = {inf, inf, inf, inf};
            if (y >= 0 && y < a.H) {
              const float *crow = a.coarse + (size_t)cy * a.Wc;
              const float *zrow = a.Z + (size_t)(y + a.zoy) * a.zpitch + a.zox;
              const bool brow = y == 0 || y == a.H - 1;
              const float c0 = (a.pool & 3) == 0 && xb >= 0 && xb < a.W ? __ldg(crow + cx) : inf;
              int cc = cx, rc = rx;
#pragma unroll
              for (int j = 0; j < 4; j++) {
                const int x = xb + j;
                if (j > 0 && ++rc == a.pool) {
                  rc = 0;
                  cc++;
                }
                if (x >= 0 && x < a.W)
                  v[j] = brow || x == 0 || x == a.W - 1 ? __ldcg(zrow + x) : (a.pool & 3) == 0 ? c0 : __ldg(crow + cc);
              }
            }
            v4 = make_float4(v[0], v[1], v[2], v[3]);
          }
          *reinterpret_cast<float4 *>(&sW[rr * SP + c4]) = v4;
          cy += dq;
          ry += dr;
          if (ry >= a.pool) {
            ry -= a.pool;
            cy++;
          }
        }
      }
    }
#include "fill_relax_body.inc"

    if (f) {
      atomicOr(&sFlags, f);
      if (f & 0xFF) atomicMin(&sKey, f2ord(kmin));
    }
    __syncthreads();
    const int fl = sFlags;
    const int rowch = (fl >> 12) & 0xFFFF;
    const int rowout = stage ? (1 << BYN) - 1 : rowch;
    if (rowout) {
      for (int k = tid; k < TY * (TX / 4); k += FILL_THREADS) {
        const int rr = k / (TX / 4), cc = k % (TX / 4);
        const int y = y0 + rr, x = x0 + 4 * cc;
        if ((rowout & (1 << (rr >> 2))) && !(a.inplace && (y >= a.H || x >= a.W))) {
          const float4 val = *reinterpret_cast<const float4 *>(&sW[(rr + 1) * SP + PADL + 4 * cc]);
          __stcg(reinterpret_cast<float4 *>(a.Wp + (size_t)(y + a.woy) * a.pitch + x + a.wox), val);
          if (STAGE && !a.use_tma)
            __stcg(reinterpret_cast<float4 *>(a.zcopy + (size_t)y * a.W + x),
                   *reinterpret_cast<const float4 *>(&sZ[rr * TX + 4 * cc]));
        }
      }
    }
    if (stage) {
      __syncthreads();
      if (tid == 0) {
        __threadfence();
        atomicExch(&a.staged[t], 1);
      }
    }
    if (STEP == 0 && WAKE_WORDS && a.edge_above) {
      fill_wake_neighbours<TOPO4>(a, sW, sZ, t, fl, sKey, next, list_next);
      if (rowch && tid == 0) {
        if (fl & (3 << 9)) atomicOr(&a.dev->edge_changed, (fl >> 9) & 3);
        if (a.dirty) a.dirty[t] = 1;
      }
    } else if (rowch) {
      if (tid < 8) {
        const int sv = r + 1;
        const bool n_ok = tyT > 0, s_ok = tyT < a.tilesY - 1, w_ok = txT > 0, e_ok = txT < a.tilesX - 1;
        int nb = -1, bits = 0;
        switch (tid) {
          case 0: if ((fl & SIDE_N) && n_ok) { nb = t - a.tilesX; bits = SIDE_S; } break;
          case 1: if ((fl & SIDE_S) && s_ok) { nb = t + a.tilesX; bits = SIDE_N; } break;
          case 2: if ((fl & SIDE_W) && w_ok) { nb = t - 1; bits = SIDE_E; } break;
          case 3: if ((fl & SIDE_E) && e_ok) { nb = t + 1; bits = SIDE_W; } break;
          case 4: if ((fl & SIDE_NW) && n_ok && w_ok) { nb = t - a.tilesX - 1; bits = SIDE_SE; } break;
          case 5: if ((fl & SIDE_NE) && n_ok && e_ok) { nb = t - a.tilesX + 1; bits = SIDE_SW; } break;
          case 6: if ((fl & SIDE_SW) && s_ok && w_ok) { nb = t + a.tilesX - 1; bits = SIDE_NE; } break;
          default: if ((fl & SIDE_SE) && s_ok && e_ok) { nb = t + a.tilesX + 1; bits = SIDE_NW; } break;
        }
        if (nb >= 0) enqueue_tile(a, next, list_next, nb, sv, bits, sKey);
        if (tid == 0 && (fl & (3 << 9))) atomicOr(&a.dev->edge_changed, (fl >> 9) & 3);
        if (tid == 0 && a.dirty) a.dirty[t] = 1;
      }
    }
    if (tid == 0) {
      if (again) enqueue_tile(a, next, list_next, t, r + 1, SIDE_FULL, f2ord(-__int_as_float(0x7f800000)));
      atomicAdd(&a.dev->iters, (unsigned long long)iters);
      if (a.profile) {
        if (!rowch) atomicAdd(&a.dev->idle_visits, 1ull);
        atomicAdd(&a.dev->block_updates, (unsigned long long)sProf[0]);
        atomicAdd(&a.dev->warp_updates, (unsigned long long)sProf[1]);
        const int hb = iters <= 1 ? 0 : iters <= 2 ? 1 : iters <= 4 ? 2 : iters <= 8 ? 3 : iters <= 16 ? 4 : iters <= 32 ? 5 : iters <= 64 ? 6 : 7;
        atomicAdd(&a.dev->iter_hist[hb], 1ull);
      }
    }
  }
  if (STAGE && a.use_tma && tid == 0) bulk_wait_all();
}

__global__ void __launch_bounds__(256) fill_admit_kernel(const FillArgs a) {
  const int r = a.round;
  const RoundCtl *cur = &a.dev->ctl[r % 3];
  RoundCtl *next = &a.dev->ctl[(r + 1) % 3];
  RoundCtl *proc = &a.dev->proc[r % 3];
  const int *list_cur = (r & 1) ? a.list1 : a.list0;
  int *list_next = (r & 1) ? a.list0 : a.list1;
  const int n = cur->count;
  const int ntiles = a.tilesX * a.tilesY;
  const float level = a.level;
  int nd = 0;
  for (int i = blockIdx.x * blockDim.x + threadIdx.x; i < n; i += gridDim.x * blockDim.x) {
    const int t = list_cur[i];
    const int kord = a.keys[(r & 1) * ntiles + t];
    if (ord2f(kord) <= level) {
      a.plist[atomicAdd(&proc->count, 1)] = t;
    } else {
      int bits = a.sides[(r & 1) * ntiles + t];
      if (bits == 0) bits = SIDE_FULL;
      a.sides[(r & 1) * ntiles + t] = 0;
      a.keys[(r & 1) * ntiles + t] = ORD_POS_INF;
      enqueue_tile(a, next, list_next, t, r + 1, bits, kord);
      nd++;
    }
  }
  for (int o = 16; o > 0; o >>= 1) nd += __shfl_xor_sync(0xffffffffu, nd, o);
  if ((threadIdx.x & 31) == 0 && nd) atomicAdd(&a.dev->ndefer[r % 3], nd);
}

__global__ void __launch_bounds__(256) fill_seed_kernel(const FillArgs a, const int *__restrict__ tiles, int n) {
  const int i = blockIdx.x * blockDim.x + threadIdx.x;
  if (i >= n) return;
  const int r = a.round;
  RoundCtl *cur = &a.dev->ctl[r % 3];
  int *list_cur = (r & 1) ? a.list1 : a.list0;
  enqueue_tile(a, cur, list_cur, tiles[i], r, SIDE_FULL, f2ord(-__int_as_float(0x7f800000)));
}

__global__ void __launch_bounds__(256) fill_seed_flags_kernel(const FillArgs a, const int *__restrict__ flag, int ntiles,
                                                               int *count) {
  const int t = blockIdx.x * blockDim.x + threadIdx.x;
  if (t >= ntiles || !flag[t]) return;
  const int r = a.round;
  RoundCtl *cur = &a.dev->ctl[r % 3];
  int *list_cur = (r & 1) ? a.list1 : a.list0;
  enqueue_tile(a, cur, list_cur, t, r, SIDE_FULL, f2ord(-__int_as_float(0x7f800000)));
  if (count) atomicAdd(count, 1);
}

__global__ void __launch_bounds__(256) fill_ghost_update_kernel(float *Wp, float *Zp, int pitch, int W, int H, int y,
                                                                 const float *__restrict__ row, int *tile_flag, int tilesX,
                                                                 int *lowered) {
  const int x = blockIdx.x * blockDim.x + threadIdx.x;
  if (x >= W) return;
  const size_t o = (size_t)(y + 1) * pitch + x + PADL;
  const float v = row[x];
  if (v < Wp[o]) {
    Wp[o] = v;
    Zp[o] = v;
    *lowered = 1;
    const int ya = y > 0 ? y - 1 : 0, yb = y < H - 1 ? y + 1 : H - 1, xa = x > 0 ? x - 1 : 0, xb = x < W - 1 ? x + 1 : W - 1;
    const int ty0 = ya / TY, ty1 = yb / TY, tx0 = xa / TX, tx1 = xb / TX;
    tile_flag[ty0 * tilesX + tx0] = 1;
    if (tx1 != tx0) tile_flag[ty0 * tilesX + tx1] = 1;
    if (ty1 != ty0) {
      tile_flag[ty1 * tilesX + tx0] = 1;
      if (tx1 != tx0) tile_flag[ty1 * tilesX + tx1] = 1;
    }
  }
}

__global__ void __launch_bounds__(256) fill_lift_row_kernel(float *row, int W, const float *__restrict__ coarse_row, int k) {
  const int x = blockIdx.x * blockDim.x + threadIdx.x;
  if (x < W) row[x] = coarse_row[x / k];
}

template <bool LIFT>
__global__ void fill_init_kernel(const float *dem, float *__restrict__ Zo, float *Wo, int W, int H, int pitch, int rows,
                                 int ox, int oy, FillDev *dev, const float *__restrict__ coarse, int Wc, int pool, int yoff) {
  const int px4 = (blockIdx.x * blockDim.x + threadIdx.x) * 4;
  const float inf = __int_as_float(0x7f800000);
  float lo = inf, hi = -inf;
  for (int py = blockIdx.y; py < rows && px4 < pitch; py += gridDim.y) {
    float zv[4], wv[4];
    const int y = py - oy;
#pragma unroll
    for (int k = 0; k < 4; k++) {
      const int x = px4 + k - ox;
      float zz = inf, ww = inf;
      if (x >= 0 && x < W && y >= 0 && y < H) {
        zz = dem[(size_t)y * W + x];
        const bool border = (x == 0) | (y == 0) | (x == W - 1) | (y == H - 1);
        ww = border ? zz : (LIFT ? __ldg(coarse + (size_t)((y + yoff) / pool) * Wc + x / pool) : inf);
        if (zz < inf && zz > -inf) {
          lo = fminf(lo, zz);
          hi = fmaxf(hi, zz);
        }
      }
      zv[k] = zz;
      wv[k] = ww;
    }
    const size_t o = (size_t)py * pitch + px4;
    *reinterpret_cast<float4 *>(Zo + o) = make_float4(zv[0], zv[1], zv[2], zv[3]);
    *reinterpret_cast<float4 *>(Wo + o) = make_float4(wv[0], wv[1], wv[2], wv[3]);
  }
  for (int o = 16; o > 0; o >>= 1) {
    lo = fminf(lo, __shfl_xor_sync(0xffffffffu, lo, o));
    hi = fmaxf(hi, __shfl_xor_sync(0xffffffffu, hi, o));
  }
  __shared__ float slo[4], shi[4];
  if ((threadIdx.x & 31) == 0) {
    slo[threadIdx.x >> 5] = lo;
    shi[threadIdx.x >> 5] = hi;
  }
  __syncthreads();
  if (threadIdx.x == 0) {
    lo = fminf(fminf(slo[0], slo[1]), fminf(slo[2], slo[3]));
    hi = fmaxf(fmaxf(shi[0], shi[1]), fmaxf(shi[2], shi[3]));
    if (lo <= hi) {
      atomicMin(&dev->zmin_ord, f2ord(lo));
      atomicMax(&dev->zmax_ord, f2ord(hi));
    }
  }
}

constexpr int HIST_BINS = 1024;
__global__ void __launch_bounds__(256) fill_hist_kernel(const float *__restrict__ Z, int zpitch, int ncols, int nrows,
                                                         int row_stride, float zmin, float inv_range, unsigned int *hist) {
  __shared__ unsigned int sh[HIST_BINS];
  for (int k = threadIdx.x; k < HIST_BINS; k += blockDim.x) sh[k] = 0;
  __syncthreads();
  const int row = blockIdx.x * row_stride;
  if (row < nrows) {
    for (int x = threadIdx.x; x < ncols; x += blockDim.x) {
      const float zv = Z[(size_t)row * zpitch + x];
      if (zv < __int_as_float(0x7f800000) && zv > -__int_as_float(0x7f800000)) {
        int b = (int)((zv - zmin) * inv_range * HIST_BINS);
        b = b < 0 ? 0 : (b >= HIST_BINS ? HIST_BINS - 1 : b);
        atomicAdd(&sh[b], 1u);
      }
    }
  }
  __syncthreads();
  for (int k = threadIdx.x; k < HIST_BINS; k += blockDim.x)
    if (sh[k]) atomicAdd(&hist[k], sh[k]);
}

__global__ void __launch_bounds__(128) dist_pad_init_kernel(const uint8_t *__restrict__ open, int open_bit,
                                                             const float *__restrict__ winit, float *__restrict__ Zp,
                                                             float *__restrict__ Wp, int W, int H, int pitch, int rows,
                                                             int ghost_top, int ghost_bottom, int *tile_flag, int tilesX) {
  const int px = blockIdx.x * blockDim.x + threadIdx.x;
  if (px >= pitch) return;
  const float inf = __int_as_float(0x7f800000);
  for (int py = blockIdx.y; py < rows; py += gridDim.y) {
    const int x = px - PADL, y = py - 1;
    float zz = inf, ww = inf;
    if (x >= 0 && x < W && y >= 0 && y < H) {
      const size_t i = (size_t)y * W + x;
      if (!((ghost_top && y == 0) || (ghost_bottom && y == H - 1))) {
        if (open[i] & open_bit) zz = 0.0f;
        ww = winit[i];
        if (ww < inf) {
          const int ya = y > 0 ? y - 1 : 0, yb = y < H - 1 ? y + 1 : H - 1, xa = x > 0 ? x - 1 : 0, xb = x < W - 1 ? x + 1 : W - 1;
          const int ty0 = ya / TY, ty1 = yb / TY, tx0 = xa / TX, tx1 = xb / TX;
          tile_flag[ty0 * tilesX + tx0] = 1;
          if (tx1 != tx0) tile_flag[ty0 * tilesX + tx1] = 1;
          if (ty1 != ty0) {
            tile_flag[ty1 * tilesX + tx0] = 1;
            if (tx1 != tx0) tile_flag[ty1 * tilesX + tx1] = 1;
          }
        }
      }
    }
    Zp[(size_t)py * pitch + px] = zz;
    Wp[(size_t)py * pitch + px] = ww;
  }
}

__global__ void fill_i32_kernel(int *p, int v, int n) {
  const int i = blockIdx.x * blockDim.x + threadIdx.x;
  if (i < n) p[i] = v;
}

__global__ void __launch_bounds__(256) fill_maxpool_kernel(const float *__restrict__ src, int W, int H, int yoff, float *dst, int Wc,
                                                            int Hc, int k, int combine) {
  const int bx = blockIdx.x * blockDim.x + threadIdx.x;
  if (bx >= Wc) return;
  const int by_lo = yoff / k, by_hi = (yoff + H - 1) / k;
  for (int by = by_lo + blockIdx.y; by <= by_hi && by < Hc; by += gridDim.y) {
    float m = -__int_as_float(0x7f800000);
    const bool vec = (k & 3) == 0 && (W & 3) == 0 && bx * k + k <= W && ((uintptr_t)src & 15) == 0;
    for (int j = 0; j < k; j++) {
      const int y = by * k + j - yoff;
      if (y < 0) continue;
      if (y >= H) break;
      if (vec) {
        const float4 *row = reinterpret_cast<const float4 *>(src + (size_t)y * W + bx * k);
        for (int i = 0; i < k / 4; i++) {
          const float4 q = __ldg(row + i);
          m = fmaxf(fmaxf(m, fmaxf(q.x, q.y)), fmaxf(q.z, q.w));
        }
      } else {
        for (int i = 0; i < k; i++) {
          const int x = bx * k + i;
          if (x < W) m = fmaxf(m, __ldg(src + (size_t)y * W + x));
        }
      }
    }
    float *o = dst + (size_t)by * Wc + bx;
    *o = combine ? fmaxf(*o, m) : m;
  }
}

__global__ void __launch_bounds__(256) fill_restrict_kernel(const float *__restrict__ Wp, int pitch, int wox, int woy, int W,
                                                             int H, float *Wc, int cpitch, int cox, int coy, int Wcw, int Hc,
                                                             int k, const int *__restrict__ dirty, int tilesX,
                                                             int *ctile_flag, int ctilesX) {
  const int bx = blockIdx.x * blockDim.x + threadIdx.x;
  if (bx >= Wcw) return;
  for (int by = blockIdx.y; by < Hc; by += gridDim.y) {
    if (dirty && !dirty[((by * k) / TY) * tilesX + (bx * k) / TX]) continue;
    float m = -__int_as_float(0x7f800000);
    if ((k & 3) == 0 && bx * k + k <= W && by * k + k <= H) {
      for (int j = 0; j < k; j++) {
        const float4 *row = reinterpret_cast<const float4 *>(Wp + (size_t)(by * k + j + woy) * pitch + bx * k + wox);
        for (int i = 0; i < k / 4; i++) {
          const float4 q = __ldcg(row + i);
          m = fmaxf(fmaxf(m, fmaxf(q.x, q.y)), fmaxf(q.z, q.w));
        }
      }
    } else {
      for (int j = 0; j < k; j++) {
        const int y = by * k + j;
        if (y >= H) break;
        for (int i = 0; i < k; i++) {
          const int x = bx * k + i;
          if (x < W) m = fmaxf(m, __ldcg(Wp + (size_t)(y + woy) * pitch + x + wox));
        }
      }
    }
    float *o = Wc + (size_t)(by + coy) * cpitch + bx + cox;
    if (m < *o && bx > 0 && by > 0 && bx < Wcw - 1 && by < Hc - 1) {
      *o = m;
      const int ty0 = (by - 1) / TY, ty1 = (by + 1) / TY, tx0 = (bx - 1) / TX, tx1 = (bx + 1) / TX;
      ctile_flag[ty0 * ctilesX + tx0] = 1;
      if (tx1 != tx0) ctile_flag[ty0 * ctilesX + tx1] = 1;
      if (ty1 != ty0) {
        ctile_flag[ty1 * ctilesX + tx0] = 1;
        if (tx1 != tx0) ctile_flag[ty1 * ctilesX + tx1] = 1;
      }
    }
  }
}

__global__ void __launch_bounds__(256) fill_blockmax_kernel(const float *__restrict__ Wp, int pitch, int wox, int woy, int W,
                                                             int y_lo, int y_hi,
                                                             int yoff, float *out, int Wcw, int Hc, int k,
                                                             const int *__restrict__ dirty, int tilesX) {
  const int bx = blockIdx.x * blockDim.x + threadIdx.x;
  if (bx >= Wcw) return;
  const int by_lo = (yoff + y_lo) / k, by_hi = (yoff + y_hi - 1) / k;
  for (int by = by_lo + blockIdx.y; by <= by_hi && by < Hc; by += gridDim.y) {
    if (dirty) {
      int l0 = by * k - yoff, l1 = l0 + k - 1;
      l0 = l0 < y_lo ? y_lo : l0;
      l1 = l1 >= y_hi ? y_hi - 1 : l1;
      const int tx = (bx * k) / TX;
      if (!dirty[(l0 / TY) * tilesX + tx] && !dirty[(l1 / TY) * tilesX + tx]) {
        out[(size_t)by * Wcw + bx] = __int_as_float(0x7f800000);
        continue;
      }
    }
    float m = -__int_as_float(0x7f800000);
    for (int j = 0; j < k; j++) {
      const int y = by * k + j - yoff;
      if (y < y_lo) continue;
      if (y >= y_hi) break;
      for (int i = 0; i < k; i++) {
        const int x = bx * k + i;
        if (x < W) m = fmaxf(m, __ldcg(Wp + (size_t)(y + woy) * pitch + x + wox));
      }
    }
    float *o = out + (size_t)by * Wcw + bx;
    *o = fmaxf(*o, m);
  }
}

__global__ void __launch_bounds__(256) fill_prolong_kernel(float *Wp, int pitch, int wox, int woy, int W, int H,
                                                            const float *__restrict__ Wc,
                                                            int cpitch, int coff_x, int coff_y, int k, int *tile_flag,
                                                            int tilesX, int yoff, const int *__restrict__ cdirty,
                                                            int ctilesX) {
  const int t = blockIdx.x;
  const int tyT = t / tilesX, txT = t - tyT * tilesX;
  const int x0 = txT * TX, y0 = tyT * TY;
  if (cdirty) {
    const int cx0 = (x0 / k) / TX, cx1 = ((x0 + TX - 1) / k) / TX;
    const int cy0 = ((y0 + yoff) / k) / TY, cy1 = ((y0 + TY - 1 + yoff) / k) / TY;
    bool any = false;
    for (int cy = cy0; cy <= cy1; cy++)
      for (int cx = cx0; cx <= cx1; cx++) any |= cdirty[cy * ctilesX + cx] != 0;
    if (!any) return;
  }
  bool lowered = false, lo_n = false, lo_s = false, lo_w = false, lo_e = false;
  for (int g = threadIdx.x; g < TX * TY / 4; g += blockDim.x) {
    const int ly = g / (TX / 4), lx4 = (g - ly * (TX / 4)) * 4;
    const int y = y0 + ly;
    if (y < 1 || y >= H - 1 || x0 + lx4 >= W) continue;
    float4 *wp4 = reinterpret_cast<float4 *>(Wp + (size_t)(y + woy) * pitch + x0 + lx4 + wox);
    const float4 w4 = *wp4;
    float wv[4] = {w4.x, w4.y, w4.z, w4.w};
    const float *crow = Wc + (size_t)((y + yoff) / k + coff_y) * cpitch + coff_x;
    bool any = false;
#pragma unroll
    for (int j = 0; j < 4; j++) {
      const int lx = lx4 + j, x = x0 + lx;
      if (x < 1 || x >= W - 1) continue;
      const float l = __ldg(crow + x / k);
      if (l < wv[j]) {
        wv[j] = l;
        any = true;
        lo_w |= lx == 0;
        lo_e |= lx == TX - 1;
      }
    }
    if (any) {
      *wp4 = make_float4(wv[0], wv[1], wv[2], wv[3]);
      lowered = true;
      lo_n |= ly == 0;
      lo_s |= ly == TY - 1;
    }
  }
  if (lowered) {
    const int tilesY = (H + TY - 1) / TY;
    tile_flag[t] = 1;
    const bool n_ok = tyT > 0, s_ok = tyT < tilesY - 1, w_ok = txT > 0, e_ok = txT < tilesX - 1;
    if (lo_n && n_ok) tile_flag[t - tilesX] = 1;
    if (lo_s && s_ok) tile_flag[t + tilesX] = 1;
    if (lo_w && w_ok) tile_flag[t - 1] = 1;
    if (lo_e && e_ok) tile_flag[t + 1] = 1;
    if (lo_n && lo_w && n_ok && w_ok) tile_flag[t - tilesX - 1] = 1;
    if (lo_n && lo_e && n_ok && e_ok) tile_flag[t - tilesX + 1] = 1;
    if (lo_s && lo_w && s_ok && w_ok) tile_flag[t + tilesX - 1] = 1;
    if (lo_s && lo_e && s_ok && e_ok) tile_flag[t + tilesX + 1] = 1;
  }
}

__global__ void __launch_bounds__(256) fill_finish_x4_kernel(const float *__restrict__ Wp, float *__restrict__ out, int W,
                                                              int H, int pitch, int wox, int woy) {
  const int x4 = (blockIdx.x * blockDim.x + threadIdx.x) * 4;
  if (x4 >= W) return;
  for (int y = blockIdx.y; y < H; y += gridDim.y) {
    const float4 v = __ldcs(reinterpret_cast<const float4 *>(Wp + (size_t)(y + woy) * pitch + x4 + wox));
    __stcs(reinterpret_cast<float4 *>(out + (size_t)y * W + x4), v);
  }
}

__global__ void fill_finish_kernel(const float *__restrict__ Wp, float *__restrict__ out, int W, int H,
                                   int pitch, int wox, int woy) {
  const int x = blockIdx.x * blockDim.x + threadIdx.x;
  if (x >= W) return;
  for (int y = blockIdx.y; y < H; y += gridDim.y) out[(size_t)y * W + x] = Wp[(size_t)(y + woy) * pitch + x + wox];
}

typedef CUresult (*EncodeTiledFn)(CUtensorMap *, CUtensorMapDataType, cuuint32_t, void *, const cuuint64_t *,
                                  const cuuint64_t *, const cuuint32_t *, const cuuint32_t *,
                                  CUtensorMapInterleave, CUtensorMapSwizzle, CUtensorMapL2promotion,
                                  CUtensorMapFloatOOBfill);

EncodeTiledFn get_encode_fn() {
  static EncodeTiledFn fn = nullptr;
  if (!fn) {
    void *p = nullptr;
    cudaDriverEntryPointQueryResult q;
    RDB_CK(cudaGetDriverEntryPoint("cuTensorMapEncodeTiled", &p, cudaEnableDefault, &q));
    if (!p || q != cudaDriverEntryPointSuccess) fail("cuTensorMapEncodeTiled not available from the driver");
    fn = (EncodeTiledFn)p;
  }
  return fn;
}

CUtensorMap make_map(float *base, int pitch, int rows, int boxw, int boxh) {
  CUtensorMap m;
  const cuuint64_t gdim[2] = {(cuuint64_t)pitch, (cuuint64_t)rows};
  const cuuint64_t gstride[1] = {(cuuint64_t)pitch * 4};
  const cuuint32_t box[2] = {(cuuint32_t)boxw, (cuuint32_t)boxh};
  const cuuint32_t estr[2] = {1, 1};
  CUresult rc = get_encode_fn()(&m, CU_TENSOR_MAP_DATA_TYPE_FLOAT32, 2, base, gdim, gstride, box, estr,
                                CU_TENSOR_MAP_INTERLEAVE_NONE, CU_TENSOR_MAP_SWIZZLE_NONE,
                                CU_TENSOR_MAP_L2_PROMOTION_L2_128B, CU_TENSOR_MAP_FLOAT_OOB_FILL_NONE);
  if (rc != CUDA_SUCCESS) fail("cuTensorMapEncodeTiled failed with CUresult %d", (int)rc);
  return m;
}

}

struct FillState {
  int W = 0, H = 0, pitch = 0, rows = 0, tilesX = 0, tilesY = 0;
  DevBuf<float> Zp, Wp;
  DevBuf<int> list0, list1, plist, stamp, sides, keys;
  DevBuf<int> dirty, tflag;
  DevBuf<int> staged;
  DevBuf<unsigned long long> edge_above;
  float zmin = 0.f, zmax = 0.f;
  bool first_run = true;
  bool ordered = false;
  int step_mode = 0;
  bool topo4 = false;
  std::vector<float> levels;
  DevBuf<FillDev> dev;
  CUtensorMap mapW, mapZ;
  int round = 0;
  int grid = 0;
  int64_t rounds_run = 0;
  int64_t live_rounds = 0;
  int64_t visits_seen = 0;
  bool still_active = false;
  int64_t sched_round = 0;

  float *Wb = nullptr;
  int wpitch = 0, wox = 0, woy = 0;
  bool inplace = false;
  DevBuf<float> Zc;
  const float *stage_coarse = nullptr;
  int stage_wc = 0, stage_k = 1, stage_yoff = 0;
  CUtensorMap mapZstage;

  void use_padded_layout(size_t np) {
    inplace = false;
    Zc.reset();
    Zp.alloc(np);
    Wp.alloc(np);
    Wb = Wp.p;
    wpitch = pitch;
    wox = PADL;
    woy = 1;
  }

  void begin(const float *d_dem, int w, int h, const float *d_coarse = nullptr, int coarse_w = 0, int coarse_k = 0,
             int coarse_yoff = 0, bool in_place = false) {
    Ctx &c = ctx();
    W = w;
    H = h;
    tilesX = (w + TX - 1) / TX;
    tilesY = (h + TY - 1) / TY;
    pitch = tilesX * TX + 2 * PADL;
    rows = tilesY * TY + 2;
    const size_t np = (size_t)pitch * rows;
    if (in_place && c.params.fill_external_z != 0 && (w & 3) == 0 && ((uintptr_t)d_dem & 15) == 0) {
      inplace = true;
      Zp.reset();
      Wp.reset();
      Zc.alloc((size_t)w * h);
      Wb = const_cast<float *>(d_dem);
      wpitch = w;
      wox = woy = 0;
    } else {
      use_padded_layout(np);
    }
    stage_coarse = inplace && d_coarse ? d_coarse : nullptr;
    stage_wc = coarse_w;
    stage_k = coarse_k;
    stage_yoff = coarse_yoff;
    const size_t nt = (size_t)tilesX * tilesY;
    list0.alloc(nt);
    list1.alloc(nt);
    plist.alloc(nt);
    stamp.alloc(nt);
    sides.alloc(2 * nt);
    keys.alloc(2 * nt);
    dev.alloc(1);
    RDB_CK(cudaMemsetAsync(stamp.p, 0, nt * sizeof(int), c.stream));
    RDB_CK(cudaMemsetAsync(sides.p, 0, 2 * nt * sizeof(int), c.stream));
    if (stage_coarse) {
      staged.alloc(nt);
      RDB_CK(cudaMemsetAsync(staged.p, 0, nt * sizeof(int), c.stream));
    }
    edge_above.alloc(4 * nt);
    RDB_CK(cudaMemsetAsync(edge_above.p, 0xff, 4 * nt * sizeof(unsigned long long), c.stream));
    {
      FillDev h0;
      memset(&h0, 0, sizeof(h0));
      h0.zmin_ord = ORD_POS_INF;
      h0.zmax_ord = f2ord(-__builtin_inff());
      memcpy(c.pinned, &h0, sizeof(h0));
      RDB_CK(cudaMemcpyAsync(dev.p, c.pinned, sizeof(FillDev), cudaMemcpyHostToDevice, c.stream));
    }
    {
      const int n2 = (int)(2 * nt);
      fill_i32_kernel<<<(n2 + 255) / 256, 256, 0, c.stream>>>(keys.p, ORD_POS_INF, n2);
      count_launch();
      dim3 blk(128), grd((pitch / 4 + 127) / 128, rows < 2048 ? rows : 2048);
      if (stage_coarse) {
      } else if (inplace) {
        dim3 grdc((W / 4 + 127) / 128, H < 2048 ? H : 2048);
        fill_init_kernel<false><<<grdc, blk, 0, c.stream>>>(d_dem, Zc.p, Wb, W, H, W, H, 0, 0, dev.p, nullptr, 0, 1, 0);
        count_launch();
      } else if (d_coarse) {
        fill_init_kernel<true><<<grd, blk, 0, c.stream>>>(d_dem, Zp.p, Wp.p, W, H, pitch, rows, PADL, 1, dev.p, d_coarse,
                                                         coarse_w, coarse_k, coarse_yoff);
        count_launch();
      } else {
        fill_init_kernel<false><<<grd, blk, 0, c.stream>>>(d_dem, Zp.p, Wp.p, W, H, pitch, rows, PADL, 1, dev.p, nullptr, 0, 1,
                                                          0);
        count_launch();
      }
      RDB_CK(cudaGetLastError());
      zmin = zmax = 0.f;
      if (!d_coarse) {
        FillDev *hd = (FillDev *)c.pinned;
        RDB_CK(cudaMemcpyAsync(hd, dev.p, sizeof(FillDev), cudaMemcpyDeviceToHost, c.stream));
        RDB_CK(cudaStreamSynchronize(c.stream));
        zmin = ord2f(hd->zmin_ord);
        zmax = ord2f(hd->zmax_ord);
        if (!(zmin <= zmax)) zmin = zmax = 0.f;
      }
      ordered = c.params.fill_ordered != 0 && zmax > zmin && !d_coarse;
      levels.clear();
      if (ordered) {
        int64_t R = c.params.fill_order_rounds;
        if (R <= 0) R = (int64_t)(0.8 * (tilesX > tilesY ? tilesX : tilesY));
        if (R < 8) {
          ordered = false;
        } else {
          DevBuf<unsigned int> hist(HIST_BINS);
          RDB_CK(cudaMemsetAsync(hist.p, 0, HIST_BINS * sizeof(unsigned int), c.stream));
          const int stride = rows > 4096 ? 16 : (rows > 512 ? 4 : 1);
          const int nb = (rows - 2 + stride - 1) / stride;
          if (inplace)
            fill_hist_kernel<<<nb, 256, 0, c.stream>>>(Zc.p, W, W, H, stride, zmin, 1.0f / (zmax - zmin), hist.p);
          else
            fill_hist_kernel<<<nb, 256, 0, c.stream>>>(Zp.p + pitch, pitch, pitch, rows - 1, stride, zmin, 1.0f / (zmax - zmin),
                                                       hist.p);
          RDB_CK(cudaGetLastError());
          count_launch();
          unsigned int *hh = (unsigned int *)c.pinned;
          RDB_CK(cudaMemcpyAsync(hh, hist.p, HIST_BINS * sizeof(unsigned int), cudaMemcpyDeviceToHost, c.stream));
          RDB_CK(cudaStreamSynchronize(c.stream));
          double total = 0;
          for (int k = 0; k < HIST_BINS; k++) total += hh[k];
          levels.resize((size_t)R);
          double cum = 0;
          int bin = 0;
          for (int64_t k = 0; k < R; k++) {
            const double want = total * (double)(k + 1) / (double)R;
            while (bin < HIST_BINS - 1 && cum + hh[bin] < want) cum += hh[bin++];
            levels[(size_t)k] = zmin + (zmax - zmin) * (float)(bin + 1) / (float)HIST_BINS;
          }
        }
      }
    }
    if (inplace) {
      mapW = make_map(Wb, W, H, SP, SROWS);
      mapZ = make_map(Zc.p, W, H, TX, TY);
      if (stage_coarse) mapZstage = make_map(Wb, W, H, TX, TY);
    } else {
      mapW = make_map(Wp.p, pitch, rows, SP, SROWS);
      mapZ = make_map(Zp.p, pitch, rows, TX, TY);
    }
    int per_sm = 0;
    RDB_CK(cudaOccupancyMaxActiveBlocksPerMultiprocessor(&per_sm, fill_sweep_kernel<0>, FILL_THREADS, 0));
    if (per_sm < 1) per_sm = 1;
    grid = c.num_sms * per_sm;
    round = 1;
    std::vector<int> init;
    for (int ty = 0; ty < tilesY; ty++)
      for (int tx = 0; tx < tilesX; tx++)
        if (d_coarse || ty == 0 || tx == 0 || ty == tilesY - 1 || tx == tilesX - 1) init.push_back(ty * tilesX + tx);
    seed_worklist(init);
  }

  void begin_dist(const uint8_t *d_open, int open_bit, const float *d_winit, int w, int h, int ghost_top = 0,
                  int ghost_bottom = 0) {
    Ctx &c = ctx();
    step_mode = 1;
    W = w;
    H = h;
    tilesX = (w + TX - 1) / TX;
    tilesY = (h + TY - 1) / TY;
    pitch = tilesX * TX + 2 * PADL;
    rows = tilesY * TY + 2;
    use_padded_layout((size_t)pitch * rows);
    const size_t nt = (size_t)tilesX * tilesY;
    list0.alloc(nt);
    list1.alloc(nt);
    plist.alloc(nt);
    stamp.alloc(nt);
    sides.alloc(2 * nt);
    keys.alloc(2 * nt);
    dev.alloc(1);
    RDB_CK(cudaMemsetAsync(stamp.p, 0, nt * sizeof(int), c.stream));
    RDB_CK(cudaMemsetAsync(sides.p, 0, 2 * nt * sizeof(int), c.stream));
    RDB_CK(cudaMemsetAsync(dev.p, 0, sizeof(FillDev), c.stream));
    const int n2 = (int)(2 * nt);
    fill_i32_kernel<<<(n2 + 255) / 256, 256, 0, c.stream>>>(keys.p, ORD_POS_INF, n2);
    dim3 blk(128), grd((pitch + 127) / 128, rows < 2048 ? rows : 2048);
    clear_flags();
    dist_pad_init_kernel<<<grd, blk, 0, c.stream>>>(d_open, open_bit, d_winit, Zp.p, Wp.p, W, H, pitch, rows, ghost_top,
                                                    ghost_bottom, tflag.p, tilesX);
    RDB_CK(cudaGetLastError());
    count_launch(2);
    ordered = false;
    mapW = make_map(Wp.p, pitch, rows, SP, SROWS);
    mapZ = make_map(Zp.p, pitch, rows, TX, TY);
    int per_sm = 0;
    RDB_CK(cudaOccupancyMaxActiveBlocksPerMultiprocessor(&per_sm, fill_sweep_kernel<1>, FILL_THREADS, 0));
    if (per_sm < 1) per_sm = 1;
    grid = c.num_sms * per_sm;
    round = 1;
    seed_from_flags();
  }

  void seed_worklist(const std::vector<int> &tiles) {
    Ctx &c = ctx();
    if (tiles.empty()) return;
    DevBuf<int> d(tiles.size());
    RDB_CK(cudaMemcpyAsync(d.p, tiles.data(), tiles.size() * sizeof(int), cudaMemcpyHostToDevice, c.stream));
    FillArgs a = make_args();
    a.round = round;
    fill_seed_kernel<<<(unsigned)((tiles.size() + 255) / 256), 256, 0, c.stream>>>(a, d.p, (int)tiles.size());
    RDB_CK(cudaGetLastError());
    count_launch();
    RDB_CK(cudaStreamSynchronize(c.stream));
  }

  FillArgs make_args() {
    Ctx &c = ctx();
    FillArgs a;
    memset(&a, 0, sizeof(a));
    if (inplace) {
      a.Z = Zc.p;
      a.zpitch = W;
      a.inplace = 1;
    } else {
      a.Z = Zp.p;
      a.zpitch = pitch;
      a.zox = PADL;
      a.zoy = 1;
    }
    a.Wc = stage_wc;
    a.pool = stage_k;
    a.yoff = stage_yoff;
    a.staged = staged.p;
    a.Wp = Wb;
    a.pitch = wpitch;
    a.wox = wox;
    a.woy = woy;
    a.W = W;
    a.H = H;
    a.tilesX = tilesX;
    a.tilesY = tilesY;
    a.list0 = list0.p;
    a.list1 = list1.p;
    a.stamp = stamp.p;
    a.sides = sides.p;
    a.keys = keys.p;
    a.plist = plist.p;
    a.dev = dev.p;
    a.max_iters = (int)c.params.fill_max_iters;
    a.use_tma = (int)c.params.fill_use_tma;
    a.profile = (int)c.params.fill_profile;
    a.level = __builtin_inff();
    a.dirty = dirty.p;
    a.edge_above = step_mode == 0 && c.params.fill_wake_filter != 0 ? edge_above.p : nullptr;
    return a;
  }

  bool timed = true;
  int batch_edge = 0;
  void launch_batch(int per_sync) {
    Ctx &c = ctx();
    FillArgs a = make_args();
    if (timed) RDB_CK(cudaEventRecord(c.evk0, c.stream));
    for (int k = 0; k < per_sync; k++) {
      a.round = round;
      if (ordered && sched_round < (int64_t)levels.size()) {
        a.level = levels[(size_t)sched_round];
        a.use_proc = 1;
        fill_admit_kernel<<<c.num_sms * 2, 256, 0, c.stream>>>(a);
        c.stats.kernel_launches++;
      } else {
        a.level = __builtin_inff();
        a.use_proc = 0;
      }
      sched_round++;
      a.coarse = round == 1 ? stage_coarse : nullptr;
      a.Z = a.coarse ? Wb : (inplace ? Zc.p : Zp.p);
      a.zcopy = a.coarse ? Zc.p : nullptr;
      const CUtensorMap &mz = a.coarse ? mapZstage : mapZ;
      if (step_mode) fill_sweep_kernel<1><<<grid, FILL_THREADS, 0, c.stream>>>(mapW, mz, mapZ, a);
      else if (a.coarse && topo4) fill_sweep_kernel<0, true, true><<<grid, FILL_THREADS, 0, c.stream>>>(mapW, mz, mapZ, a);
      else if (a.coarse) fill_sweep_kernel<0, false, true><<<grid, FILL_THREADS, 0, c.stream>>>(mapW, mz, mapZ, a);
      else if (topo4) fill_sweep_kernel<0, true><<<grid, FILL_THREADS, 0, c.stream>>>(mapW, mz, mapZ, a);
      else fill_sweep_kernel<0><<<grid, FILL_THREADS, 0, c.stream>>>(mapW, mz, mapZ, a);
      round++;
    }
    if (timed) RDB_CK(cudaEventRecord(c.evk1, c.stream));
    RDB_CK(cudaGetLastError());
    RDB_CK(cudaMemcpyAsync(c.pinned, dev.p, sizeof(FillDev), cudaMemcpyDeviceToHost, c.stream));
    c.stats.kernel_launches += per_sync;
    rounds_run += per_sync;
    if (round > (1 << 30)) fail("fill: round counter overflow");
  }
  bool collect() {
    Ctx &c = ctx();
    RDB_CK(cudaStreamSynchronize(c.stream));
    if (timed) {
      float t = 0;
      RDB_CK(cudaEventElapsedTime(&t, c.evk0, c.evk1));
      c.stats.ms_main_kernel += t;
    }
    const FillDev *hd = (const FillDev *)c.pinned;
    still_active = hd->ctl[round % 3].count != 0;
    if (!still_active) first_run = false;
    live_rounds = (int64_t)hd->live_rounds;
    visits_seen = (int64_t)hd->visits;
    iters_seen = (int64_t)hd->iters;
    batch_edge = hd->edge_changed;
    return still_active;
  }
  int64_t iters_seen = 0;

  int run(int64_t max_rounds = 0) {
    Ctx &c = ctx();
    int64_t rounds_this_call = 0;
    int per_sync = (int)(c.params.fill_rounds_per_sync > 0 ? c.params.fill_rounds_per_sync : 16);
    if (max_rounds > 0 && max_rounds < per_sync) per_sync = (int)max_rounds;
    RDB_CK(cudaMemsetAsync(&dev.p->edge_changed, 0, sizeof(int), c.stream));
    for (;;) {
      launch_batch(per_sync);
      collect();
      rounds_this_call += per_sync;
      if (!still_active) break;
      if (max_rounds > 0 && rounds_this_call >= max_rounds) break;
    }
    const FillDev *hd = (const FillDev *)c.pinned;
    c.stats.fill_rounds = live_rounds;
    c.stats.fill_tile_visits = visits_seen;
    c.stats.fill_tile_iters = iters_seen;
    c.stats.fill_tile_cells = TX * TY;
    if (c.params.fill_profile) {
      fprintf(stderr, "[fill profile] deferred=%llu visits=%llu iters=%llu block_updates=%llu (%.1f%% of 256/iter) warp_updates=%llu (%.1f%% of 8/iter) idle_visits=%llu wakes_dropped=%llu hist(1,2,3-4,5-8,9-16,17-32,33-64,65+)=",
              hd->deferred, hd->visits, hd->iters, hd->block_updates, 100.0 * hd->block_updates / (256.0 * hd->iters + 1),
              hd->warp_updates, 100.0 * hd->warp_updates / (8.0 * hd->iters + 1), hd->idle_visits, hd->wakes_dropped);
      for (int k = 0; k < 8; k++) fprintf(stderr, "%llu ", hd->iter_hist[k]);
      fprintf(stderr, "\n");
      fprintf(stderr, "[fill wake] visits=%llu idle_visits=%llu wakes_dropped=%llu\n", hd->visits - prof_seen[0],
              hd->idle_visits - prof_seen[1], hd->wakes_dropped - prof_seen[2]);
      prof_seen[0] = hd->visits;
      prof_seen[1] = hd->idle_visits;
      prof_seen[2] = hd->wakes_dropped;
    }
    return batch_edge | (still_active ? 4 : 0);
  }
  unsigned long long prof_seen[3] = {0, 0, 0};

  void track_dirty() {
    Ctx &c = ctx();
    const size_t nt = (size_t)tilesX * tilesY;
    dirty.alloc(nt);
    RDB_CK(cudaMemsetAsync(dirty.p, 0, nt * sizeof(int), c.stream));
  }
  void clear_dirty() {
    if (dirty.p) RDB_CK(cudaMemsetAsync(dirty.p, 0, (size_t)tilesX * tilesY * sizeof(int), ctx().stream));
  }
  void seed_from_flags(int *d_count = nullptr) {
    Ctx &c = ctx();
    const int nt = tilesX * tilesY;
    FillArgs a = make_args();
    a.round = round;
    fill_seed_flags_kernel<<<(nt + 255) / 256, 256, 0, c.stream>>>(a, tflag.p, nt, d_count);
    RDB_CK(cudaGetLastError());
    count_launch();
  }
  void clear_flags() {
    const size_t nt = (size_t)tilesX * tilesY;
    if (!tflag.p) tflag.alloc(nt);
    RDB_CK(cudaMemsetAsync(tflag.p, 0, nt * sizeof(int), ctx().stream));
  }
  void restrict_into(FillState &cs, int k) {
    Ctx &c = ctx();
    cs.clear_flags();
    const bool selective = dirty.p && TX % k == 0 && TY % k == 0;
    dim3 blk(256), grd((unsigned)((cs.W + 255) / 256), (unsigned)(cs.H < 4096 ? cs.H : 4096));
    fill_restrict_kernel<<<grd, blk, 0, c.stream>>>(Wb, wpitch, wox, woy, W, H, cs.Wb, cs.wpitch, cs.wox, cs.woy, cs.W, cs.H,
                                                    k, selective ? dirty.p : nullptr, tilesX, cs.tflag.p, cs.tilesX);
    RDB_CK(cudaGetLastError());
    count_launch();
    cs.seed_from_flags();
    clear_dirty();
  }
  void blockmax_into(float *d_out, int wc, int hc, int k, int yoff, int y_lo, int y_hi, bool selective = false) {
    Ctx &c = ctx();
    dim3 blk(256), grd((unsigned)((wc + 255) / 256), (unsigned)((y_hi - y_lo) / k + 2 < 4096 ? (y_hi - y_lo) / k + 2 : 4096));
    const bool sel = selective && dirty.p && TX % k == 0;
    fill_blockmax_kernel<<<grd, blk, 0, c.stream>>>(Wb, wpitch, wox, woy, W, y_lo, y_hi, yoff, d_out, wc, hc, k,
                                                    sel ? dirty.p : nullptr, tilesX);
    RDB_CK(cudaGetLastError());
    count_launch();
    if (sel) clear_dirty();
  }
  void prolong_from(const float *d_wc, int cpitch, int coff_x, int coff_y, int k, int yoff = 0, const int *cdirty = nullptr,
                    int ctilesX = 0, int *d_count = nullptr) {
    Ctx &c = ctx();
    clear_flags();
    const int nt = tilesX * tilesY;
    fill_prolong_kernel<<<nt, 256, 0, c.stream>>>(Wb, wpitch, wox, woy, W, H, d_wc, cpitch, coff_x, coff_y, k, tflag.p, tilesX,
                                                  yoff, cdirty, ctilesX);
    RDB_CK(cudaGetLastError());
    count_launch();
    seed_from_flags(d_count);
  }
  void prolong_from_level(FillState &cs, int k, int yoff = 0, int *d_count = nullptr) {
    prolong_from(cs.Wb, cs.wpitch, cs.wox, cs.woy, k, yoff, cs.dirty.p, cs.tilesX, d_count);
    cs.clear_dirty();
  }
  void ghost_update(int y, const float *d_row, int *d_lowered) {
    Ctx &c = ctx();
    clear_flags();
    fill_ghost_update_kernel<<<(W + 255) / 256, 256, 0, c.stream>>>(Wp.p, Zp.p, pitch, W, H, y, d_row, tflag.p, tilesX, d_lowered);
    RDB_CK(cudaGetLastError());
    count_launch();
    seed_from_flags();
  }

  void read_row(int y, float *d_row) {
    if (y < 0 || y >= H) fail("fill_read_row: row %d out of range", y);
    RDB_CK(cudaMemcpyAsync(d_row, Wb + (size_t)(y + woy) * wpitch + wox, (size_t)W * 4,
                           cudaMemcpyDeviceToDevice, ctx().stream));
  }

  void update_row(int y, const float *d_row) {
    if (y != 0 && y != H - 1) fail("fill_update_row: only boundary rows (0, height-1) can be replaced");
    Ctx &c = ctx();
    const size_t o = (size_t)(y + 1) * pitch + PADL;
    RDB_CK(cudaMemcpyAsync(Wp.p + o, d_row, (size_t)W * 4, cudaMemcpyDeviceToDevice, c.stream));
    RDB_CK(cudaMemcpyAsync(Zp.p + o, d_row, (size_t)W * 4, cudaMemcpyDeviceToDevice, c.stream));
    pending_rows.push_back(y);
  }
  std::vector<int> pending_rows;

  void activate_pending() {
    if (pending_rows.empty()) return;
    std::vector<char> mark((size_t)tilesX * tilesY, 0);
    std::vector<int> tiles;
    for (int y : pending_rows) {
      for (int yy = y - 1; yy <= y + 1; yy++) {
        if (yy < 0 || yy >= H) continue;
        const int tyT = yy / TY;
        for (int tx = 0; tx < tilesX; tx++) {
          const int t = tyT * tilesX + tx;
          if (!mark[t]) {
            mark[t] = 1;
            tiles.push_back(t);
          }
        }
      }
    }
    pending_rows.clear();
    seed_worklist(tiles);
  }

  void finish(float *d_out) {
    Ctx &c = ctx();
    if (d_out == Wb) return;
    if ((W & 3) == 0 && ((uintptr_t)d_out & 15) == 0) {
      dim3 blk(256), grd((W / 4 + 255) / 256, H < 4096 ? H : 4096);
      fill_finish_x4_kernel<<<grd, blk, 0, c.stream>>>(Wb, d_out, W, H, wpitch, wox, woy);
    } else {
      dim3 blk(256), grd((W + 255) / 256, H < 32768 ? H : 32768);
      fill_finish_kernel<<<grd, blk, 0, c.stream>>>(Wb, d_out, W, H, wpitch, wox, woy);
    }
    RDB_CK(cudaGetLastError());
    count_launch();
  }
};

void geodesic_distance_dev(const uint8_t *d_open, int open_bit, float *d_w_inout, int w, int h) {
  Ctx &c = ctx();
  FillState st;
  const rdb200_stats saved = c.stats;
  st.begin_dist(d_open, open_bit, d_w_inout, w, h);
  st.run();
  st.finish(d_w_inout);
  RDB_CK(cudaStreamSynchronize(c.stream));
  const int64_t launches = c.stats.kernel_launches;
  const int64_t rounds = c.stats.fill_rounds;
  c.stats = saved;
  c.stats.kernel_launches = launches;
  c.stats.flat_bfs_levels += rounds;
}

void geodesic_distance_pair_dev(const uint8_t *d_open, int open_bit, float *d_wa, float *d_wb, int w, int h) {
  Ctx &c = ctx();
  if (!c.aux_stream[0]) {
    RDB_CK(cudaStreamCreateWithFlags(&c.aux_stream[0], cudaStreamNonBlocking));
    RDB_CK(cudaStreamCreateWithFlags(&c.aux_stream[1], cudaStreamNonBlocking));
    RDB_CK(cudaEventCreateWithFlags(&c.aux_event[0], cudaEventDisableTiming));
    RDB_CK(cudaEventCreateWithFlags(&c.aux_event[1], cudaEventDisableTiming));
    RDB_CK(cudaEventCreateWithFlags(&c.aux_event[2], cudaEventDisableTiming));
  }
  const rdb200_stats saved = c.stats;
  cudaStream_t main_stream = c.stream;
  void *main_pinned = c.pinned;
  RDB_CK(cudaEventRecord(c.aux_event[2], main_stream));
  FillState st[2];
  float *wbuf[2] = {d_wa, d_wb};
  auto lane = [&](int k, auto &&fn) {
    c.stream = c.aux_stream[k];
    c.pinned = (char *)main_pinned + 8192 * (k + 1);
    try {
      fn(st[k]);
    } catch (...) {
      c.stream = main_stream;
      c.pinned = main_pinned;
      throw;
    }
    c.stream = main_stream;
    c.pinned = main_pinned;
  };
  static_assert(sizeof(FillDev) <= 8192, "pinned slot");
  try {
    for (int k = 0; k < 2; k++) {
      RDB_CK(cudaStreamWaitEvent(c.aux_stream[k], c.aux_event[2], 0));
      lane(k, [&](FillState &s) {
        s.timed = false;
        s.begin_dist(d_open, open_bit, wbuf[k], w, h);
        s.grid = s.grid > 1 ? s.grid / 2 : 1;
      });
    }
    const int per_sync = (int)(c.params.fill_rounds_per_sync > 0 ? c.params.fill_rounds_per_sync : 16);
    bool live[2] = {true, true};
    while (live[0] || live[1]) {
      for (int k = 0; k < 2; k++)
        if (live[k]) lane(k, [&](FillState &s) { s.launch_batch(per_sync); });
      for (int k = 0; k < 2; k++)
        if (live[k]) lane(k, [&](FillState &s) { live[k] = s.collect(); });
    }
    for (int k = 0; k < 2; k++) {
      lane(k, [&](FillState &s) { s.finish(wbuf[k]); });
      RDB_CK(cudaEventRecord(c.aux_event[k], c.aux_stream[k]));
      RDB_CK(cudaStreamWaitEvent(main_stream, c.aux_event[k], 0));
    }
  } catch (...) {
    cudaStreamSynchronize(c.aux_stream[0]);
    cudaStreamSynchronize(c.aux_stream[1]);
    throw;
  }
  RDB_CK(cudaStreamSynchronize(c.aux_stream[0]));
  RDB_CK(cudaStreamSynchronize(c.aux_stream[1]));
  const int64_t launches = c.stats.kernel_launches;
  c.stats = saved;
  c.stats.kernel_launches = launches;
  c.stats.flat_bfs_levels += st[0].live_rounds + st[1].live_rounds;
}

static void fill_depressions_level(float *d_dem, int w, int h, int depth, bool topo4 = false) {
  Ctx &c = ctx();
  const int k = (int)c.params.fill_multigrid;
  const int min_side = (int)(c.params.fill_multigrid_min > 0 ? c.params.fill_multigrid_min : 1024);
  FillState st;
  st.topo4 = topo4;
  if (k >= 2 && depth < 8 && w >= min_side && h >= min_side && w / k >= 3 && h / k >= 3) {
    const int wc = (w + k - 1) / k, hc = (h + k - 1) / k;
    DevBuf<float> coarse((size_t)wc * hc);
    dim3 blk(256), grd((unsigned)((wc + 255) / 256), (unsigned)(hc < 4096 ? hc : 4096));
    fill_maxpool_kernel<<<grd, blk, 0, c.stream>>>(d_dem, w, h, 0, coarse.p, wc, hc, k, 0);
    RDB_CK(cudaGetLastError());
    count_launch();
    const int every = (int)c.params.fill_vcycle;
    DevBuf<float> zc;
    if (every > 0) {
      zc.alloc((size_t)wc * hc);
      RDB_CK(cudaMemcpyAsync(zc.p, coarse.p, (size_t)wc * hc * sizeof(float), cudaMemcpyDeviceToDevice, c.stream));
    }
    const rdb200_stats before = c.stats;
    fill_depressions_level(coarse.p, wc, hc, depth + 1, topo4);
    rdb200_stats extra = c.stats;
    extra.fill_rounds -= before.fill_rounds;
    extra.fill_tile_visits -= before.fill_tile_visits;
    extra.fill_tile_iters -= before.fill_tile_iters;
    st.begin(d_dem, w, h, coarse.p, wc, k, 0, true);
    if (every <= 0) {
      st.run();
    } else {
      FillState cst;
      cst.topo4 = topo4;
      cst.begin(zc.p, wc, hc, coarse.p, wc, 1, 0, true);
      cst.run();
      cst.track_dirty();
      st.track_dirty();
      int64_t coarse_visits0 = c.stats.fill_tile_visits, coarse_iters0 = c.stats.fill_tile_iters;
      const bool trace = c.params.fill_trace != 0;
      auto now_ms = [&]() {
        RDB_CK(cudaStreamSynchronize(c.stream));
        return std::chrono::duration<double, std::milli>(std::chrono::steady_clock::now().time_since_epoch()).count();
      };
      for (int cycle = 0;; cycle++) {
        const double t0 = trace ? now_ms() : 0;
        const int64_t v0 = st.visits_seen, r0 = st.live_rounds;
        const bool active = (st.run(every) & 4) != 0;
        const double t1 = trace ? now_ms() : 0;
        if (trace)
          fprintf(stderr, "[fill trace] depth %d cycle %d: fine run %.3f ms (%lld live rounds, %lld visits)%s\n", depth, cycle,
                  t1 - t0, (long long)(st.live_rounds - r0), (long long)(st.visits_seen - v0), active ? "" : " -> converged");
        if (!active) break;
        if (cycle >= 1000) {
          st.run();
          break;
        }
        st.restrict_into(cst, k);
        const double t2 = trace ? now_ms() : 0;
        const int64_t cv0 = cst.visits_seen, cr0 = cst.live_rounds;
        cst.run();
        const double t3 = trace ? now_ms() : 0;
        st.prolong_from_level(cst, k);
        if (trace) {
          const double t4 = now_ms();
          fprintf(stderr, "[fill trace] depth %d cycle %d: restrict %.3f ms, coarse run %.3f ms (%lld live rounds, %lld visits), "
                          "prolong %.3f ms\n", depth, cycle, t2 - t1, t3 - t2, (long long)(cst.live_rounds - cr0),
                  (long long)(cst.visits_seen - cv0), t4 - t3);
        }
      }
      cst.run(1);
      extra.fill_rounds += cst.live_rounds;
      extra.fill_tile_visits += c.stats.fill_tile_visits;
      extra.fill_tile_iters += c.stats.fill_tile_iters;
      (void)coarse_visits0;
      (void)coarse_iters0;
      st.run(1);
    }
    st.finish(d_dem);
    RDB_CK(cudaStreamSynchronize(c.stream));
    c.stats.fill_rounds = st.live_rounds + extra.fill_rounds;
    c.stats.fill_tile_visits += extra.fill_tile_visits;
    c.stats.fill_tile_iters += extra.fill_tile_iters;
    return;
  }
  if (w <= 2 || h <= 2) return;
  st.begin(d_dem, w, h, nullptr, 0, 0, 0, true);
  st.run();
  st.finish(d_dem);
  RDB_CK(cudaStreamSynchronize(c.stream));
}

void fill_relax_from_dev(const float *d_dem, float *d_w, int w, int h) {
  Ctx &c = ctx();
  c.stats.cells = (int64_t)w * h;
  if (w <= 2 || h <= 2) {
    RDB_CK(cudaMemcpyAsync(d_w, d_dem, (size_t)w * h * sizeof(float), cudaMemcpyDeviceToDevice, c.stream));
    RDB_CK(cudaStreamSynchronize(c.stream));
    return;
  }
  FillState st;
  st.begin(d_dem, w, h, d_w, w, 1);
  st.run();
  st.finish(d_w);
  RDB_CK(cudaStreamSynchronize(c.stream));
}

void fill_maxpool_rows(const float *d_src, int w, int h, int yoff, float *d_coarse, int wc, int hc, int k, dim3 grd, dim3 blk) {
  fill_maxpool_kernel<<<grd, blk, 0, ctx().stream>>>(d_src, w, h, yoff, d_coarse, wc, hc, k, 1);
  RDB_CK(cudaGetLastError());
  count_launch();
}

void mgpu_fill_band(const rdb200_comm *comm, float *d_local, int w, int hloc, int gt, int gb, int row0, int H, int *xrounds,
                    bool topo4) {
  Ctx &c = ctx();
  const int world = comm_world(comm);
  gt = gt ? 1 : 0;
  gb = gb ? 1 : 0;
  if (w < 3 || hloc - gt - gb < 1 || hloc < 3) fail("mgpu_fill: band too small (%d x %d)", w, hloc);
  if (row0 < 0 || row0 + hloc > H) fail("mgpu_fill: rows [%d, %d) are outside the raster (%d rows)", row0, row0 + hloc, H);
  int k = (int)c.params.fill_band_multigrid;
  if (k <= 0) {
    k = (int)c.params.fill_multigrid;
    if (k >= 2 && world > 2 && TX % (2 * k) == 0) k *= 2;
  }
  const int min_side = (int)(c.params.fill_multigrid_min > 0 ? c.params.fill_multigrid_min : 1024);
  const bool mg = k >= 2 && w >= min_side && H >= min_side && w / k >= 3 && H / k >= 3 && c.params.fill_multigrid >= 2;
  const int R = (int)(c.params.fill_vcycle > 0 ? c.params.fill_vcycle : 8);
  const float inf = __builtin_inff();
  DevBuf<float> rows(4 * (size_t)w);
  DevBuf<int> flags(4);
  float *send_up = rows.p, *send_dn = rows.p + w, *recv_up = rows.p + 2 * (size_t)w, *recv_dn = rows.p + 3 * (size_t)w;
  FillState st, cst;
  DevBuf<float> zc, wcoarse, bm;
  int wc = 0, hc = 0;
  auto fill_f32 = [&](float *p, size_t n, float v) {
    int bits;
    memcpy(&bits, &v, 4);
    fill_i32_kernel<<<(unsigned)((n + 255) / 256), 256, 0, c.stream>>>(reinterpret_cast<int *>(p), bits, (int)n);
    RDB_CK(cudaGetLastError());
  };
  const bool trace0 = c.params.fill_trace != 0;
  double t0_prev = 0;
  auto lap0 = [&](const char *what) {
    if (!trace0) return;
    RDB_CK(cudaStreamSynchronize(c.stream));
    const double t = std::chrono::duration<double, std::milli>(std::chrono::steady_clock::now().time_since_epoch()).count();
    if (what) fprintf(stderr, "[mgpu fill trace] rank %d begin: %-32s %8.3f ms\n", comm_rank(comm), what, t - t0_prev);
    t0_prev = t;
  };
  lap0(nullptr);
  if (mg) {
    wc = (w + k - 1) / k;
    hc = (H + k - 1) / k;
    const size_t nc = (size_t)wc * hc;
    zc.alloc(nc);
    wcoarse.alloc(nc);
    bm.alloc(nc);
    fill_f32(zc.p, nc, -inf);
    {
      const int hown = hloc - gt - gb;
      dim3 blk(256), grd((unsigned)((wc + 255) / 256), (unsigned)(hown / k + 2 < 4096 ? hown / k + 2 : 4096));
      fill_maxpool_rows(d_local + (size_t)gt * w, w, hown, row0 + gt, zc.p, wc, hc, k, grd, blk);
    }
    lap0("max-pool own rows");
    comm_allreduce(comm, zc.p, nc, RDB200_MAX_F32);
    lap0("all-reduce pooled raster");
    RDB_CK(cudaMemcpyAsync(wcoarse.p, zc.p, nc * sizeof(float), cudaMemcpyDeviceToDevice, c.stream));
    fill_depressions_level(wcoarse.p, wc, hc, 1, topo4);
    lap0("coarse fill (replicated)");
    for (int side = 0; side < 2; side++) {
      if (!(side == 0 ? gt : gb)) continue;
      const int y = side == 0 ? 0 : hloc - 1;
      fill_lift_row_kernel<<<(w + 255) / 256, 256, 0, c.stream>>>(d_local + (size_t)y * w, w, wcoarse.p + (size_t)((row0 + y) / k) * wc, k);
    }
    RDB_CK(cudaGetLastError());
    st.topo4 = topo4;
    st.begin(d_local, w, hloc, wcoarse.p, wc, k, row0);
    lap0("band start (lifted)");
    cst.topo4 = topo4;
    cst.begin(zc.p, wc, hc, wcoarse.p, wc, 1);
    cst.run();
    cst.track_dirty();
    st.track_dirty();
    lap0("coarse solver setup");
  } else {
    if (gt) fill_f32(d_local, (size_t)w, inf);
    if (gb) fill_f32(d_local + (size_t)(hloc - 1) * w, (size_t)w, inf);
    st.topo4 = topo4;
    st.begin(d_local, w, hloc);
  }
  int cycles = 0;
  bool vcycle_on = true;
  int *hflags = (int *)c.pinned + 1024;
  const bool trace = c.params.fill_trace != 0;
  double t_prev = 0;
  auto lap = [&](const char *what) {
    if (!trace) return;
    RDB_CK(cudaStreamSynchronize(c.stream));
    const double t = std::chrono::duration<double, std::milli>(std::chrono::steady_clock::now().time_since_epoch()).count();
    if (what) fprintf(stderr, "[mgpu fill trace] rank %d cycle %d: %-28s %8.3f ms\n", comm_rank(comm), cycles, what, t - t_prev);
    t_prev = t;
  };
  lap(nullptr);
  for (;; cycles++) {
    if (cycles > 100000) fail("mgpu_fill: no convergence");
    const bool active = (st.run(world > 1 || mg ? R : 0) & 4) != 0;
    lap("band sweeps");
    RDB_CK(cudaMemsetAsync(flags.p, 0, 4 * sizeof(int), c.stream));
    if (world > 1) {
      if (gt) st.read_row(1, send_up);
      if (gb) st.read_row(hloc - 2, send_dn);
      comm_exchange(comm, send_up, recv_up, send_dn, recv_dn, (size_t)w * sizeof(float));
      if (gt) st.ghost_update(0, recv_up, flags.p + 1);
      if (gb) st.ghost_update(hloc - 1, recv_dn, flags.p + 1);
      lap("halo exchange");
    }
    if (mg && vcycle_on) {
      fill_f32(bm.p, (size_t)wc * hc, -inf);
      st.blockmax_into(bm.p, wc, hc, k, row0, gt, hloc - gb, true);
      lap("block maxima");
      comm_allreduce(comm, bm.p, (size_t)wc * hc, RDB200_MAX_F32);
      lap("all-reduce coarse");
      cst.prolong_from(bm.p, wc, 0, 0, 1, 0, nullptr, 0, flags.p + 2);
      cst.run();
      lap("coarse relaxation");
      st.prolong_from_level(cst, k, row0, flags.p + 3);
      lap("prolongation");
    }
    if (active) fill_i32_kernel<<<1, 1, 0, c.stream>>>(flags.p, 1, 1);
    comm_allreduce(comm, flags.p, 4, RDB200_MAX_I32);
    RDB_CK(cudaMemcpyAsync(hflags, flags.p, 4 * sizeof(int), cudaMemcpyDeviceToHost, c.stream));
    RDB_CK(cudaStreamSynchronize(c.stream));
    lap("termination vote");
    if (!(hflags[0] | hflags[1] | hflags[2] | hflags[3])) break;
    const int few = st.tilesX * st.tilesY / 64 > 32 ? st.tilesX * st.tilesY / 64 : 32;
    if (trace) fprintf(stderr, "[mgpu fill trace] rank %d cycle %d: flags active=%d ghost=%d coarse=%d fine=%d (cut-off %d)\n",
                       comm_rank(comm), cycles, hflags[0], hflags[1], hflags[2], hflags[3], few);
    if (hflags[2] + hflags[3] < few) vcycle_on = false;
  }
  st.run(1);
  const int64_t visits = st.visits_seen, iters = st.iters_seen, rounds = st.live_rounds;
  st.finish(d_local);
  RDB_CK(cudaStreamSynchronize(c.stream));
  lap("finish");
  c.stats.fill_rounds = rounds + (mg ? cst.live_rounds : 0);
  c.stats.fill_tile_visits = visits;
  c.stats.fill_tile_iters = iters;
  c.stats.fill_tile_cells = TX * TY;
  if (xrounds) *xrounds = cycles + 1;
}

void fill_depressions_dev(float *d_dem, int w, int h, bool topo4) {
  Ctx &c = ctx();
  c.stats.cells = (int64_t)w * h;
  if (w <= 2 || h <= 2) return;
  fill_depressions_level(d_dem, w, h, 0, topo4);
}

}

struct rdb200_fill_state {
  rdb::FillState st;
};

namespace rdb {
rdb200_fill_state *new_band_distance_state(const uint8_t *d_open, int open_bit, const float *d_winit, int w, int h,
                                           int ghost_top, int ghost_bottom) {
  auto *s = new rdb200_fill_state();
  try {
    s->st.begin_dist(d_open, open_bit, d_winit, w, h, ghost_top, ghost_bottom);
  } catch (...) {
    delete s;
    throw;
  }
  return s;
}
void finish_band_distance_state(rdb200_fill_state *s, float *d_out) {
  s->st.finish(d_out);
  RDB_CK(cudaStreamSynchronize(ctx().stream));
  delete s;
}

int mgpu_relax_band(const rdb200_comm *comm, rdb200_fill_state *state, int gt, int gb, int R) {
  Ctx &c = ctx();
  FillState &st = state->st;
  const int world = comm_world(comm), w = st.W, h = st.H;
  DevBuf<float> rows(4 * (size_t)w);
  DevBuf<int> flags(2);
  float *send_up = rows.p, *send_dn = rows.p + w, *recv_up = rows.p + 2 * (size_t)w, *recv_dn = rows.p + 3 * (size_t)w;
  int *hflags = (int *)c.pinned + 1024;
  for (int cycles = 1;; cycles++) {
    if (cycles > 100000) fail("mgpu_relax_band: no convergence");
    const bool active = (st.run(world > 1 ? R : 0) & 4) != 0;
    if (world == 1) {
      if (active) continue;
      RDB_CK(cudaStreamSynchronize(c.stream));
      return cycles;
    }
    RDB_CK(cudaMemsetAsync(flags.p, 0, 2 * sizeof(int), c.stream));
    if (gt) st.read_row(1, send_up);
    if (gb) st.read_row(h - 2, send_dn);
    comm_exchange(comm, send_up, recv_up, send_dn, recv_dn, (size_t)w * sizeof(float));
    if (gt) st.ghost_update(0, recv_up, flags.p + 1);
    if (gb) st.ghost_update(h - 1, recv_dn, flags.p + 1);
    if (active) fill_i32_kernel<<<1, 1, 0, c.stream>>>(flags.p, 1, 1);
    comm_allreduce(comm, flags.p, 2, RDB200_MAX_I32);
    RDB_CK(cudaMemcpyAsync(hflags, flags.p, 2 * sizeof(int), cudaMemcpyDeviceToHost, c.stream));
    RDB_CK(cudaStreamSynchronize(c.stream));
    if (!(hflags[0] | hflags[1])) return cycles;
  }
}
}

namespace rdb {
void capi_set_error(const char *msg);
}

#define RDB_CAPI_TRY try {
#define RDB_CAPI_END                 \
  }                                  \
  catch (const std::exception &e) {  \
    rdb::capi_set_error(e.what());   \
    return 1;                        \
  }                                  \
  return 0;

extern "C" {

int rdb200_dev_fill_begin(rdb200_fill_state **state, const float *d_dem, int32_t width, int32_t height) {
  RDB_CAPI_TRY
  rdb::ensure_init();
  if (!state) rdb::fail("fill_begin: null state pointer");
  if (width < 3 || height < 3) rdb::fail("fill_begin: band must be at least 3x3");
  auto *s = new rdb200_fill_state();
  try {
    s->st.begin(d_dem, width, height);
  } catch (...) {
    delete s;
    throw;
  }
  *state = s;
  RDB_CAPI_END
}

int rdb200_dev_fill_begin_lifted(rdb200_fill_state **state, const float *d_dem, int32_t width, int32_t height,
                                 const float *d_coarse, int32_t coarse_width, int32_t pool, int32_t row_offset) {
  RDB_CAPI_TRY
  rdb::ensure_init();
  if (!state) rdb::fail("fill_begin_lifted: null state pointer");
  if (width < 3 || height < 3) rdb::fail("fill_begin_lifted: band must be at least 3x3");
  if (!d_coarse || pool < 2 || coarse_width < (width + pool - 1) / pool || row_offset < 0)
    rdb::fail("fill_begin_lifted: bad coarse raster (pool %d, coarse_width %d, row_offset %d)", pool, coarse_width, row_offset);
  auto *s = new rdb200_fill_state();
  try {
    s->st.begin(d_dem, width, height, d_coarse, coarse_width, pool, row_offset);
  } catch (...) {
    delete s;
    throw;
  }
  *state = s;
  RDB_CAPI_END
}

int rdb200_dev_maxpool_rows_f32(const float *d_src, int32_t width, int32_t height, int32_t row_offset, int32_t pool,
                                float *d_coarse, int32_t coarse_width, int32_t coarse_height) {
  RDB_CAPI_TRY
  rdb::ensure_init();
  if (width < 1 || height < 1 || pool < 2 || row_offset < 0 || coarse_width < (width + pool - 1) / pool ||
      coarse_height < (row_offset + height + pool - 1) / pool)
    rdb::fail("maxpool_rows: bad geometry");
  rdb::Ctx &c = rdb::ctx();
  dim3 blk(256), grd((unsigned)((coarse_width + 255) / 256), (unsigned)(height / pool + 2 < 4096 ? height / pool + 2 : 4096));
  rdb::fill_maxpool_rows(d_src, width, height, row_offset, d_coarse, coarse_width, coarse_height, pool, grd, blk);
  RDB_CK(cudaStreamSynchronize(c.stream));
  RDB_CAPI_END
}

int rdb200_dev_fill_relax_from_f32(const float *d_dem, float *d_w_inout, int32_t width, int32_t height) {
  RDB_CAPI_TRY
  rdb::ensure_init();
  if (width < 1 || height < 1) rdb::fail("fill_relax_from: raster dimensions must be positive");
  rdb::fill_relax_from_dev(d_dem, d_w_inout, width, height);
  RDB_CAPI_END
}

int rdb200_dev_fill_blockmax(rdb200_fill_state *state, float *d_blockmax, int32_t coarse_width, int32_t coarse_height, int32_t pool,
                             int32_t row_offset, int32_t skip_top, int32_t skip_bottom) {
  RDB_CAPI_TRY
  if (!state) rdb::fail("fill_blockmax: null state");
  rdb::FillState &st = state->st;
  if (pool < 2 || row_offset < 0 || skip_top < 0 || skip_bottom < 0 || skip_top + skip_bottom >= st.H ||
      coarse_width < (st.W + pool - 1) / pool || coarse_height < (row_offset + st.H - skip_bottom + pool - 1) / pool)
    rdb::fail("fill_blockmax: bad geometry");
  st.blockmax_into(d_blockmax, coarse_width, coarse_height, pool, row_offset, skip_top, st.H - skip_bottom);
  RDB_CK(cudaStreamSynchronize(rdb::ctx().stream));
  RDB_CAPI_END
}

int rdb200_dev_fill_prolong(rdb200_fill_state *state, const float *d_coarse, int32_t coarse_width, int32_t pool, int32_t row_offset,
                            int32_t *tiles_lowered) {
  RDB_CAPI_TRY
  if (!state) rdb::fail("fill_prolong: null state");
  if (!d_coarse || pool < 2 || row_offset < 0) rdb::fail("fill_prolong: bad arguments");
  rdb::Ctx &c = rdb::ctx();
  rdb::DevBuf<int> cnt(1);
  RDB_CK(cudaMemsetAsync(cnt.p, 0, sizeof(int), c.stream));
  state->st.prolong_from(d_coarse, coarse_width, 0, 0, pool, row_offset, nullptr, 0, cnt.p);
  int *h = (int *)c.pinned;
  RDB_CK(cudaMemcpyAsync(h, cnt.p, sizeof(int), cudaMemcpyDeviceToHost, c.stream));
  RDB_CK(cudaStreamSynchronize(c.stream));
// ... 42 lines not shown
```

### richdem_b200/csrc/fill_relax_body.inc

```
    if (sides == 0) sides = SIDE_FULL;
    const int lane = tid & 31, wrp = tid >> 5;
    {
      int cntw = 0;
#pragma unroll
      for (int q = 0; q < SEG / 32; q++) {
        const int b = wrp * SEG + 32 * q + lane;
        const int bx = b % BXN, by = b / BXN;
        bool on = (sides & SIDE_FULL) != 0;
        on |= (sides & SIDE_N) && by == 0;
        on |= (sides & SIDE_S) && by == BYN - 1;
        on |= (sides & SIDE_W) && bx == 0;
        on |= (sides & SIDE_E) && bx == BXN - 1;
        on |= (sides & SIDE_NW) && b == 0;
        on |= (sides & SIDE_NE) && b == BXN - 1;
        on |= (sides & SIDE_SW) && b == NBLK - BXN;
        on |= (sides & SIDE_SE) && b == NBLK - 1;
        on &= b < NBLK;
        const unsigned bal = __ballot_sync(0xffffffffu, on);
        if (on) sList[0][wrp][cntw + __popc(bal & ((1u << lane) - 1u))] = (unsigned char)b;
        cntw += __popc(bal);
      }
      if (lane == 0) sCnt[0][wrp] = cntw;
    }
    if (a.use_tma) {
      mbar_wait(&mbar, phase);
      phase ^= 1;
      if (a.inplace) {
        const float inf = __int_as_float(0x7f800000);
        if (!STAGE && (x0 == 0 || y0 == 0 || x0 + TX + PADL > a.W || y0 + TY + 1 > a.H)) {
          for (int k = tid; k < SROWS * SP; k += FILL_THREADS) {
            const int rr = k / SP, cc = k - rr * SP;
            const int y = y0 + rr - 1, x = x0 + cc - PADL;
            if (y < 0 || y >= a.H || x < 0 || x >= a.W) sW[k] = inf;
          }
        }
        if (x0 + TX > a.W || y0 + TY > a.H) {
          for (int k = tid; k < TX * TY; k += FILL_THREADS) {
            const int rr = k / TX, cc = k - rr * TX;
            if (y0 + rr >= a.H || x0 + cc >= a.W) sZ[k] = inf;
          }
          if (STAGE) fence_proxy_async();
        }
      }
    }
    __syncthreads();
    if (STAGE && a.use_tma && tid == 0) tma_store_2d(&mapZout, x0, y0, sZ);
    if constexpr (STAGE && DRAIN_SWEEPS) fill_drain_sweeps<TOPO4>(sW, sZ, y0, a.H, &sFlags, &sKey);

    int f = 0;
    float kmin = __int_as_float(0x7f800000);
    int iters = 0;
    int cl = 0;
    bool again = false;
    int segn[NWARP];
    int nlist = 0;
#pragma unroll
    for (int w2 = 0; w2 < NWARP; w2++) {
      segn[w2] = sCnt[0][w2];
      nlist += segn[w2];
    }
    while (nlist > 0) {
      for (int i = tid; i < nlist; i += FILL_THREADS) {
        int seg = 0, off = i;
#pragma unroll
        for (int w2 = 0; w2 < NWARP - 1; w2++) {
          if (seg == w2 && off >= segn[w2]) {
            off -= segn[w2];
            seg = w2 + 1;
          }
        }
        const int b = sList[cl][seg][off];
        const int bx = b % BXN, by = b / BXN;
        const int srow = 4 * by + 1, scol = 4 * bx + PADL;
        float v[6][6];
        float z[4][4];
        bool at_floor = true;
#pragma unroll
        for (int j = 0; j < 4; j++) {
          const float4 z4 = *reinterpret_cast<const float4 *>(&sZ[(4 * by + j) * TX + 4 * bx]);
          const float4 m4 = *reinterpret_cast<const float4 *>(&sW[(srow + j) * SP + scol]);
          z[j][0] = z4.x; z[j][1] = z4.y; z[j][2] = z4.z; z[j][3] = z4.w;
          v[j + 1][1] = m4.x; v[j + 1][2] = m4.y; v[j + 1][3] = m4.z; v[j + 1][4] = m4.w;
          at_floor &= (z4.x == m4.x) & (z4.y == m4.y) & (z4.z == m4.z) & (z4.w == m4.w);
        }
        if (at_floor) continue;
#pragma unroll
        for (int j = 0; j < 6; j++) {
          const float *row = &sW[(srow - 1 + j) * SP + scol];
          if (j == 0 || j == 5) {
            const float4 m4 = *reinterpret_cast<const float4 *>(row);
            v[j][1] = m4.x; v[j][2] = m4.y; v[j][3] = m4.z; v[j][4] = m4.w;
          }
          v[j][0] = row[-1];
          v[j][5] = row[4];
        }
        uint32_t ch = 0;
#pragma unroll
        for (int j = 1; j <= 4; j++) {
#pragma unroll
          for (int i2 = 1; i2 <= 4; i2++) {
            const float zz = z[j - 1][i2 - 1];
            const float others = TOPO4 ? min3f(v[j - 1][i2], v[j + 1][i2], v[j][i2 + 1])
                                       : min3f(min3f(v[j - 1][i2 - 1], v[j - 1][i2], v[j - 1][i2 + 1]),
                                               min3f(v[j + 1][i2 - 1], v[j + 1][i2], v[j + 1][i2 + 1]), v[j][i2 + 1]);
            const float b0 = fminf(v[j][i2], fmaxf(zz, STEP ? others + 1.0f : others));
            const float nw = fminf(b0, fmaxf(zz, STEP ? v[j][i2 - 1] + 1.0f : v[j][i2 - 1]));
            if (nw < v[j][i2]) ch |= 1u << ((j - 1) * 4 + (i2 - 1));
            v[j][i2] = nw;
          }
        }
#pragma unroll
        for (int j = 4; j >= 1; j--) {
#pragma unroll
          for (int i2 = 4; i2 >= 1; i2--) {
            const float zz = z[j - 1][i2 - 1];
            const float others = TOPO4 ? min3f(v[j - 1][i2], v[j + 1][i2], v[j][i2 - 1])
                                       : min3f(min3f(v[j - 1][i2 - 1], v[j - 1][i2], v[j - 1][i2 + 1]),
                                               min3f(v[j + 1][i2 - 1], v[j + 1][i2], v[j + 1][i2 + 1]), v[j][i2 - 1]);
            const float b0 = fminf(v[j][i2], fmaxf(zz, STEP ? others + 1.0f : others));
            const float nw = fminf(b0, fmaxf(zz, STEP ? v[j][i2 + 1] + 1.0f : v[j][i2 + 1]));
            if (nw < v[j][i2]) ch |= 1u << ((j - 1) * 4 + (i2 - 1));
            v[j][i2] = nw;
          }
        }
        if (ch) {
#pragma unroll
          for (int j = 0; j < 4; j++) {
            if (ch & (0xFu << (4 * j))) {
              *reinterpret_cast<float4 *>(&sW[(srow + j) * SP + scol]) =
                  make_float4(v[j + 1][1], v[j + 1][2], v[j + 1][3], v[j + 1][4]);
            }
          }
          unsigned char *mk = &sMark[(by + 1) * MKP + (bx + 1)];
          mk[0] = 1;
          if (ch & 0x000Fu) mk[-MKP] = 1;
          if (ch & 0xF000u) mk[MKP] = 1;
          if (ch & 0x1111u) mk[-1] = 1;
          if (ch & 0x8888u) mk[1] = 1;
          if (ch & 0x0001u) mk[-MKP - 1] = 1;
          if (ch & 0x0008u) mk[-MKP + 1] = 1;
          if (ch & 0x1000u) mk[MKP - 1] = 1;
          if (ch & 0x8000u) mk[MKP + 1] = 1;
          if (by == 0 && (ch & 0x000Fu)) f |= SIDE_N;
          if (by == BYN - 1 && (ch & 0xF000u)) f |= SIDE_S;
          if (bx == 0 && (ch & 0x1111u)) f |= SIDE_W;
          if (bx == BXN - 1 && (ch & 0x8888u)) f |= SIDE_E;
          if (b == 0 && (ch & 0x0001u)) f |= SIDE_NW;
          if (b == BXN - 1 && (ch & 0x0008u)) f |= SIDE_NE;
          if (b == NBLK - BXN && (ch & 0x1000u)) f |= SIDE_SW;
          if (b == NBLK - 1 && (ch & 0x8000u)) f |= SIDE_SE;
          {
            const int gy0 = y0 + 4 * by;
            const int j1 = 1 - gy0, j2 = (a.H - 2) - gy0;
            if (j1 >= 0 && j1 < 4 && (ch & (0xFu << (4 * j1)))) f |= 1 << 9;
            if (j2 >= 0 && j2 < 4 && (ch & (0xFu << (4 * j2)))) f |= 1 << 10;
          }
          f |= 1 << (12 + by);
          if (bx == 0 || by == 0 || bx == BXN - 1 || by == BYN - 1) {
#pragma unroll
            for (int j = 0; j < 4; j++)
#pragma unroll
              for (int i2 = 0; i2 < 4; i2++)
                if (ch & (1u << (4 * j + i2))) kmin = fminf(kmin, v[j + 1][i2 + 1]);
          }
        }
      }
      if (a.profile && tid == 0) {
        sProf[0] += nlist;
        sProf[1] += (nlist + 31) / 32;
      }
      iters++;
      __syncthreads();
      {
        int cntw = 0;
#pragma unroll
        for (int q = 0; q < SEG / 32; q++) {
          const int b = wrp * SEG + 32 * q + lane;
          const int mi = (b / BXN + 1) * MKP + (b % BXN) + 1;
          const bool on = (b < NBLK) && sMark[mi] != 0;
          if (on) sMark[mi] = 0;
          const unsigned bal = __ballot_sync(0xffffffffu, on);
          if (on) sList[cl ^ 1][wrp][cntw + __popc(bal & ((1u << lane) - 1u))] = (unsigned char)b;
          cntw += __popc(bal);
        }
        if (lane == 0) sCnt[cl ^ 1][wrp] = cntw;
      }
      __syncthreads();
      cl ^= 1;
      nlist = 0;
#pragma unroll
      for (int w2 = 0; w2 < NWARP; w2++) {
        segn[w2] = sCnt[cl][w2];
        nlist += segn[w2];
      }
      if (nlist > 0 && max_iters > 0 && iters >= max_iters) {
        again = true;
        break;
      }
    }
```

Measured before the change: 22400.

## Relax fill in integer key space when DEM has no negative or NaN values

Adds an integer-key variant of the tiled fill relaxation. When a maxpool pre-pass finds no negative values or NaNs (bit patterns above 0x7f800000), floats are compared as signed ints, and the min/max network is rewritten as max(z, min3(self, others, prev)) using the three-way integer min instruction. The goal is fewer ALU ops per cell update in the hot relaxation loop. It adds a flag reduction in the maxpool kernel, a device-to-host flag copy into pinned memory, and more kernel template instantiations. Optional clock64 instrumentation is included behind a compile-time macro.

```diff
diff --git a/include/richdem_b200.h b/include/richdem_b200.h
--- a/include/richdem_b200.h
+++ b/include/richdem_b200.h
@@ -36,6 +36,7 @@
   double ms_total;
   double ms_main_kernel;
   double ms_h2d, ms_d2h;
+  int64_t fill_key_rounds;
 } rdb200_stats;
 RDB200_API int rdb200_get_stats(rdb200_stats *out);
 
diff --git a/richdem_b200/_lib.py b/richdem_b200/_lib.py
--- a/richdem_b200/_lib.py
+++ b/richdem_b200/_lib.py
@@ -22,7 +22,7 @@
         ("fill_tile_visits", C.c_int64), ("fill_tile_cells", C.c_int64), ("fill_tile_iters", C.c_int64),
         ("accum_rounds", C.c_int64), ("flat_bfs_levels", C.c_int64), ("flat_cells_raised", C.c_int64),
         ("ms_total", C.c_double), ("ms_main_kernel", C.c_double), ("ms_h2d", C.c_double),
-        ("ms_d2h", C.c_double),
+        ("ms_d2h", C.c_double), ("fill_key_rounds", C.c_int64),
     ]
 
     def as_dict(self):
diff --git a/richdem_b200/csrc/capi.cu b/richdem_b200/csrc/capi.cu
--- a/richdem_b200/csrc/capi.cu
+++ b/richdem_b200/csrc/capi.cu
@@ -243,6 +243,7 @@
   else if (n == "fill_external_z") p.fill_external_z = value;
   else if (n == "fill_profile") p.fill_profile = value;
   else if (n == "fill_wake_filter") p.fill_wake_filter = value;
+  else if (n == "fill_int_keys") p.fill_int_keys = value;
   else if (n == "fill_trace") p.fill_trace = value;
   else if (n == "fill_ordered") p.fill_ordered = value;
   else if (n == "fill_order_rounds") p.fill_order_rounds = value;
diff --git a/richdem_b200/csrc/common.cuh b/richdem_b200/csrc/common.cuh
--- a/richdem_b200/csrc/common.cuh
+++ b/richdem_b200/csrc/common.cuh
@@ -54,6 +54,7 @@
   int64_t fill_band_rounds = 0;
   int64_t fill_profile = 0;
   int64_t fill_wake_filter = 1;
+  int64_t fill_int_keys = 1;
   int64_t fill_trace = 0;
   int64_t fill_multigrid = 8;
   int64_t fill_vcycle = 8;
diff --git a/richdem_b200/csrc/fill.cu b/richdem_b200/csrc/fill.cu
--- a/richdem_b200/csrc/fill.cu
+++ b/richdem_b200/csrc/fill.cu
@@ -53,6 +53,7 @@
   float level, step, step_min, level_max;
   int target, ordered;
   int ndefer[3];
+  unsigned long long clk_visit, clk_update;
 };
 
 struct FillArgs {
@@ -162,6 +163,36 @@
 
 __device__ __forceinline__ float min3f(float a, float b, float c) { return fminf(fminf(a, b), c); }
 
+template <bool KEYS>
+struct Lv {
+  typedef float T;
+  static __device__ __forceinline__ T of(float f) { return f; }
+  static __device__ __forceinline__ float to_f(T v) { return v; }
+  static __device__ __forceinline__ T mn(T a, T b) { return fminf(a, b); }
+  static __device__ __forceinline__ T mx(T a, T b) { return fmaxf(a, b); }
+  static __device__ __forceinline__ T mn3(T a, T b, T c) { return min3f(a, b, c); }
+};
+template <>
+struct Lv<true> {
+  typedef int T;
+  static __device__ __forceinline__ T of(float f) { return __float_as_int(f); }
+  static __device__ __forceinline__ float to_f(T v) { return __int_as_float(v); }
+  static __device__ __forceinline__ T mn(T a, T b) { return a < b ? a : b; }
+  static __device__ __forceinline__ T mx(T a, T b) { return a > b ? a : b; }
+  static __device__ __forceinline__ T mn3(T a, T b, T c) {
+#ifdef __CUDA_ARCH__
+    return __vimin3_s32(a, b, c);
+#else
+    return mn(mn(a, b), c);
+#endif
+  }
+};
+template <int STEP, class T>
+__device__ __forceinline__ T step_up(T x) {
+  if constexpr (STEP != 0) return x + 1.0f;
+  else return x;
+}
+
 constexpr bool WAKE_WORDS = TX <= 64 && TY <= 64;
 
 struct EdgeLine {
@@ -178,8 +209,10 @@
 
 constexpr bool DRAIN_SWEEPS = TX == 64 && TY == 64 && FILL_THREADS == 128;
 
-template <bool TOPO4>
+template <bool TOPO4, bool KEYS>
 __device__ __forceinline__ void fill_drain_sweeps(float *sW, const float *sZ, int y0, int H, int *sFlags, int *sKey) {
+  typedef Lv<KEYS> L;
+  typedef typename L::T V;
   const unsigned FULL = 0xffffffffu;
   const int tid = threadIdx.x, lane = tid & 31, wrp = tid >> 5;
   const int x = 32 * (wrp & 1) + lane;
@@ -187,31 +220,31 @@
   const int dy = down ? 1 : -1;
   const bool ecol = x < 4 || x >= TX - 4;
   unsigned long long rows = 0;
-  float kmin = __int_as_float(0x7f800000);
+  V kmin = L::of(__int_as_float(0x7f800000));
   int y = down ? 0 : TY - 1;
-  float p = sW[(y - dy + 1) * SP + PADL + x];
+  V p = L::of(sW[(y - dy + 1) * SP + PADL + x]);
 #pragma unroll 1
   for (int half = 0; half < 2; half++) {
 #pragma unroll 8
     for (int s = 0; s < TY / 2; s++, y += dy) {
-      const float zz = sZ[y * TX + x];
+      const V zz = L::of(sZ[y * TX + x]);
       float *cell = &sW[(y + 1) * SP + PADL + x];
-      const float w = *cell;
-      float m = p;
+      const V w = L::of(*cell);
+      V m = p;
       if (!TOPO4) {
-        float pl = __shfl_up_sync(FULL, p, 1), pr = __shfl_down_sync(FULL, p, 1);
+        V pl = __shfl_up_sync(FULL, p, 1), pr = __shfl_down_sync(FULL, p, 1);
         const float *prow = &sW[(y - dy + 1) * SP + PADL + x];
-        if (lane == 0) pl = prow[-1];
-        if (lane == 31) pr = prow[1];
-        m = min3f(pl, p, pr);
-      }
-      const float nw = fminf(w, fmaxf(zz, m));
+        if (lane == 0) pl = L::of(prow[-1]);
+        if (lane == 31) pr = L::of(prow[1]);
+        m = L::mn3(pl, p, pr);
+      }
+      const V nw = L::mn(w, L::mx(zz, m));
       p = w;
       if (nw < w) {
-        *cell = nw;
+        *cell = L::to_f(nw);
         p = nw;
         rows |= 1ull << y;
-        if (ecol || y < 4 || y >= TY - 4) kmin = fminf(kmin, nw);
+        if (ecol || y < 4 || y >= TY - 4) kmin = L::mn(kmin, nw);
       }
     }
     __syncthreads();
@@ -230,20 +263,23 @@
 #pragma unroll
   for (int o = 16; o > 0; o >>= 1) {
     f |= __shfl_xor_sync(FULL, f, o);
-    kmin = fminf(kmin, __shfl_xor_sync(FULL, kmin, o));
+    kmin = L::mn(kmin, __shfl_xor_sync(FULL, kmin, o));
   }
   if (lane == 0 && f) {
     atomicOr(sFlags, f);
-    if (f & 0xFF) atomicMin(sKey, f2ord(kmin));
+    if (f & 0xFF) atomicMin(sKey, f2ord(L::to_f(kmin)));
   }
 }
 
 #ifndef __noinline__
 #define __noinline__ __attribute__((noinline))
 #endif
-template <bool TOPO4>
-__device__ __noinline__ void fill_wake_neighbours(const FillArgs &a, const float *sW, const float *sZ, int t, int fl, int key,
+template <bool TOPO4, bool KEYS>
+__device__ __noinline__ void fill_wake_neighbours(const FillArgs &a, const float *sWf, const float *sZf, int t, int fl, int key,
                                                   RoundCtl *next, int *list_next) {
+  typedef Lv<KEYS> L;
+  typedef typename L::T V;
+  const V *sW = reinterpret_cast<const V *>(sWf), *sZ = reinterpret_cast<const V *>(sZf);
   const unsigned FULL = 0xffffffffu;
   const int lane = threadIdx.x & 31;
   const int tyT = t / a.tilesX, txT = t - tyT * a.tilesX;
@@ -278,10 +314,10 @@
     bool need = false;
     for (int i = lane; i < e.len; i += 32) {
       if (!((nword >> i) & 1ull)) continue;
-      float m = sW[e.o + i * e.st];
+      V m = sW[e.o + i * e.st];
       if (!TOPO4) {
-        if (i > 0) m = fminf(m, sW[e.o + (i - 1) * e.st]);
-        if (i < e.len - 1) m = fminf(m, sW[e.o + (i + 1) * e.st]);
+        if (i > 0) m = L::mn(m, sW[e.o + (i - 1) * e.st]);
+        if (i < e.len - 1) m = L::mn(m, sW[e.o + (i + 1) * e.st]);
       }
       need |= m < sW[e.o + i * e.st + e.da];
     }
@@ -293,10 +329,11 @@
   }
 }
 
-template <int STEP, bool TOPO4 = false, bool STAGE = false>
+template <int STEP, bool TOPO4 = false, bool STAGE = false, bool KEYS = false>
 __global__ void __launch_bounds__(FILL_THREADS, FILL_MIN_CTAS)
     fill_sweep_kernel(const __grid_constant__ CUtensorMap mapW, const __grid_constant__ CUtensorMap mapZ,
                       const __grid_constant__ CUtensorMap mapZout, const __grid_constant__ FillArgs a) {
+  static_assert(!(KEYS && STEP), "the distance mode adds 1.0f: floats only");
   __shared__ __align__(128) float sW[SROWS * SP];
   __shared__ __align__(128) float sZ[TY * TX];
   __shared__ __align__(8) unsigned long long mbar;
@@ -349,6 +386,10 @@
     __syncthreads();
     const int li = sTile;
     if (li >= n) break;
+#ifdef RDB_FILL_CLOCKS
+    const long long clk_visit0 = clock64();
+    long long clk_update = 0;
+#endif
     const int t = list_cur[li];
     const int tyT = t / a.tilesX, txT = t - tyT * a.tilesX;
     const int x0 = txT * TX, y0 = tyT * TY;
@@ -460,7 +501,7 @@
 
     if (f) {
       atomicOr(&sFlags, f);
-      if (f & 0xFF) atomicMin(&sKey, f2ord(kmin));
+      if (f & 0xFF) atomicMin(&sKey, f2ord(L::to_f(kmin)));
     }
     __syncthreads();
     const int fl = sFlags;
@@ -487,7 +528,7 @@
       }
     }
     if (STEP == 0 && WAKE_WORDS && a.edge_above) {
-      fill_wake_neighbours<TOPO4>(a, sW, sZ, t, fl, sKey, next, list_next);
+      fill_wake_neighbours<TOPO4, KEYS>(a, sW, sZ, t, fl, sKey, next, list_next);
       if (rowch && tid == 0) {
         if (fl & (3 << 9)) atomicOr(&a.dev->edge_changed, (fl >> 9) & 3);
         if (a.dirty) a.dirty[t] = 1;
@@ -512,6 +553,12 @@
         if (tid == 0 && a.dirty) a.dirty[t] = 1;
       }
     }
+#ifdef RDB_FILL_CLOCKS
+    if ((tid & 31) == 0) {
+      atomicAdd(&a.dev->clk_visit, (unsigned long long)(clock64() - clk_visit0));
+      atomicAdd(&a.dev->clk_update, (unsigned long long)clk_update);
+    }
+#endif
     if (tid == 0) {
       if (again) enqueue_tile(a, next, list_next, t, r + 1, SIDE_FULL, f2ord(-__int_as_float(0x7f800000)));
       atomicAdd(&a.dev->iters, (unsigned long long)iters);
@@ -711,12 +758,14 @@
   if (i < n) p[i] = v;
 }
 
+__device__ __forceinline__ bool not_a_key(float v) { return __float_as_uint(v) > 0x7f800000u; }
+
 __global__ void __launch_bounds__(256) fill_maxpool_kernel(const float *__restrict__ src, int W, int H, int yoff, float *dst, int Wc,
-                                                            int Hc, int k, int combine) {
+                                                            int Hc, int k, int combine, int *unkeyed) {
   const int bx = blockIdx.x * blockDim.x + threadIdx.x;
-  if (bx >= Wc) return;
+  bool bad = false;
   const int by_lo = yoff / k, by_hi = (yoff + H - 1) / k;
-  for (int by = by_lo + blockIdx.y; by <= by_hi && by < Hc; by += gridDim.y) {
+  for (int by = by_lo + blockIdx.y; bx < Wc && by <= by_hi && by < Hc; by += gridDim.y) {
     float m = -__int_as_float(0x7f800000);
     const bool vec = (k & 3) == 0 && (W & 3) == 0 && bx * k + k <= W && ((uintptr_t)src & 15) == 0;
     for (int j = 0; j < k; j++) {
@@ -728,17 +777,24 @@
         for (int i = 0; i < k / 4; i++) {
           const float4 q = __ldg(row + i);
           m = fmaxf(fmaxf(m, fmaxf(q.x, q.y)), fmaxf(q.z, q.w));
+          if (unkeyed) bad |= not_a_key(q.x) | not_a_key(q.y) | not_a_key(q.z) | not_a_key(q.w);
         }
       } else {
         for (int i = 0; i < k; i++) {
           const int x = bx * k + i;
-          if (x < W) m = fmaxf(m, __ldg(src + (size_t)y * W + x));
+          if (x < W) {
+            const float q = __ldg(src + (size_t)y * W + x);
+            m = fmaxf(m, q);
+            if (unkeyed) bad |= not_a_key(q);
+          }
         }
       }
     }
     float *o = dst + (size_t)by * Wc + bx;
     *o = combine ? fmaxf(*o, m) : m;
   }
+  if (unkeyed && __ballot_sync(0xffffffffu, bad) && (threadIdx.x & 31) == 0 && !*(volatile int *)unkeyed)
+    atomicOr(unkeyed, 1);
 }
 
 __global__ void __launch_bounds__(256) fill_restrict_kernel(const float *__restrict__ Wp, int pitch, int wox, int woy, int W,
@@ -936,6 +992,8 @@
   bool ordered = false;
   int step_mode = 0;
   bool topo4 = false;
+  const volatile int *key_flag = nullptr;
+  bool int_keys = false;
   std::vector<float> levels;
   DevBuf<FillDev> dev;
   CUtensorMap mapW, mapZ;
@@ -1097,6 +1155,7 @@
       for (int tx = 0; tx < tilesX; tx++)
         if (d_coarse || ty == 0 || tx == 0 || ty == tilesY - 1 || tx == tilesX - 1) init.push_back(ty * tilesX + tx);
     seed_worklist(init);
+    int_keys = key_flag && *key_flag == 0 && inplace && c.params.fill_int_keys != 0;
   }
 
   void begin_dist(const uint8_t *d_open, int open_bit, const float *d_winit, int w, int h, int ghost_top = 0,
@@ -1218,6 +1277,10 @@
       a.zcopy = a.coarse ? Zc.p : nullptr;
       const CUtensorMap &mz = a.coarse ? mapZstage : mapZ;
       if (step_mode) fill_sweep_kernel<1><<<grid, FILL_THREADS, 0, c.stream>>>(mapW, mz, mapZ, a);
+      else if (int_keys && a.coarse && topo4) fill_sweep_kernel<0, true, true, true><<<grid, FILL_THREADS, 0, c.stream>>>(mapW, mz, mapZ, a);
+      else if (int_keys && a.coarse) fill_sweep_kernel<0, false, true, true><<<grid, FILL_THREADS, 0, c.stream>>>(mapW, mz, mapZ, a);
+      else if (int_keys && topo4) fill_sweep_kernel<0, true, false, true><<<grid, FILL_THREADS, 0, c.stream>>>(mapW, mz, mapZ, a);
+      else if (int_keys) fill_sweep_kernel<0, false, false, true><<<grid, FILL_THREADS, 0, c.stream>>>(mapW, mz, mapZ, a);
       else if (a.coarse && topo4) fill_sweep_kernel<0, true, true><<<grid, FILL_THREADS, 0, c.stream>>>(mapW, mz, mapZ, a);
       else if (a.coarse) fill_sweep_kernel<0, false, true><<<grid, FILL_THREADS, 0, c.stream>>>(mapW, mz, mapZ, a);
       else if (topo4) fill_sweep_kernel<0, true><<<grid, FILL_THREADS, 0, c.stream>>>(mapW, mz, mapZ, a);
@@ -1228,6 +1291,7 @@
     RDB_CK(cudaGetLastError());
     RDB_CK(cudaMemcpyAsync(c.pinned, dev.p, sizeof(FillDev), cudaMemcpyDeviceToHost, c.stream));
     c.stats.kernel_launches += per_sync;
+    if (int_keys) c.stats.fill_key_rounds += per_sync;
     rounds_run += per_sync;
     if (round > (1 << 30)) fail("fill: round counter overflow");
   }
@@ -1276,13 +1340,19 @@
       fprintf(stderr, "\n");
       fprintf(stderr, "[fill wake] visits=%llu idle_visits=%llu wakes_dropped=%llu\n", hd->visits - prof_seen[0],
               hd->idle_visits - prof_seen[1], hd->wakes_dropped - prof_seen[2]);
+      fprintf(stderr, "[fill engine] %s rounds=%lld\n", int_keys ? "int_keys" : "float", (long long)rounds_run);
+#ifdef RDB_FILL_CLOCKS
+      fprintf(stderr, "[fill clocks] visit=%llu update=%llu\n", hd->clk_visit - prof_seen[3], hd->clk_update - prof_seen[4]);
+      prof_seen[3] = hd->clk_visit;
+      prof_seen[4] = hd->clk_update;
+#endif
       prof_seen[0] = hd->visits;
       prof_seen[1] = hd->idle_visits;
       prof_seen[2] = hd->wakes_dropped;
     }
     return batch_edge | (still_active ? 4 : 0);
   }
-  unsigned long long prof_seen[3] = {0, 0, 0};
+  unsigned long long prof_seen[5] = {0, 0, 0, 0, 0};
 
   void track_dirty() {
     Ctx &c = ctx();
@@ -1484,7 +1554,8 @@
   c.stats.flat_bfs_levels += st[0].live_rounds + st[1].live_rounds;
 }
 
-static void fill_depressions_level(float *d_dem, int w, int h, int depth, bool topo4 = false) {
+static void fill_depressions_level(float *d_dem, int w, int h, int depth, bool topo4 = false,
+                                   const volatile int *key_flag = nullptr) {
   Ctx &c = ctx();
   const int k = (int)c.params.fill_multigrid;
   const int min_side = (int)(c.params.fill_multigrid_min > 0 ? c.params.fill_multigrid_min : 1024);
@@ -1494,9 +1565,21 @@
     const int wc = (w + k - 1) / k, hc = (h + k - 1) / k;
     DevBuf<float> coarse((size_t)wc * hc);
     dim3 blk(256), grd((unsigned)((wc + 255) / 256), (unsigned)(hc < 4096 ? hc : 4096));
-    fill_maxpool_kernel<<<grd, blk, 0, c.stream>>>(d_dem, w, h, 0, coarse.p, wc, hc, k, 0);
+    DevBuf<int> unkeyed;
+    if (depth == 0 && c.params.fill_int_keys != 0) {
+      unkeyed.alloc(1);
+      RDB_CK(cudaMemsetAsync(unkeyed.p, 0, sizeof(int), c.stream));
+    }
+    fill_maxpool_kernel<<<grd, blk, 0, c.stream>>>(d_dem, w, h, 0, coarse.p, wc, hc, k, 0, unkeyed.p);
     RDB_CK(cudaGetLastError());
     count_launch();
+    if (unkeyed.p) {
+      int *h_flag = (int *)((char *)c.pinned + c.pinned_bytes) - 1;
+      *h_flag = 1;
+      RDB_CK(cudaMemcpyAsync(h_flag, unkeyed.p, sizeof(int), cudaMemcpyDeviceToHost, c.stream));
+      key_flag = h_flag;
+    }
+    st.key_flag = key_flag;
     const int every = (int)c.params.fill_vcycle;
     DevBuf<float> zc;
     if (every > 0) {
@@ -1504,7 +1587,7 @@
       RDB_CK(cudaMemcpyAsync(zc.p, coarse.p, (size_t)wc * hc * sizeof(float), cudaMemcpyDeviceToDevice, c.stream));
     }
     const rdb200_stats before = c.stats;
-    fill_depressions_level(coarse.p, wc, hc, depth + 1, topo4);
+    fill_depressions_level(coarse.p, wc, hc, depth + 1, topo4, key_flag);
     rdb200_stats extra = c.stats;
     extra.fill_rounds -= before.fill_rounds;
     extra.fill_tile_visits -= before.fill_tile_visits;
@@ -1515,6 +1598,7 @@
     } else {
       FillState cst;
       cst.topo4 = topo4;
+      cst.key_flag = key_flag;
       cst.begin(zc.p, wc, hc, coarse.p, wc, 1, 0, true);
       cst.run();
       cst.track_dirty();
@@ -1567,6 +1651,7 @@
     return;
   }
   if (w <= 2 || h <= 2) return;
+  st.key_flag = key_flag;
   st.begin(d_dem, w, h, nullptr, 0, 0, 0, true);
   st.run();
   st.finish(d_dem);
@@ -1589,7 +1674,7 @@
 }
 
 void fill_maxpool_rows(const float *d_src, int w, int h, int yoff, float *d_coarse, int wc, int hc, int k, dim3 grd, dim3 blk) {
-  fill_maxpool_kernel<<<grd, blk, 0, ctx().stream>>>(d_src, w, h, yoff, d_coarse, wc, hc, k, 1);
+  fill_maxpool_kernel<<<grd, blk, 0, ctx().stream>>>(d_src, w, h, yoff, d_coarse, wc, hc, k, 1, nullptr);
   RDB_CK(cudaGetLastError());
   count_launch();
 }
diff --git a/richdem_b200/csrc/fill_relax_body.inc b/richdem_b200/csrc/fill_relax_body.inc
--- a/richdem_b200/csrc/fill_relax_body.inc
+++ b/richdem_b200/csrc/fill_relax_body.inc
@@ -1,3 +1,5 @@
+    typedef Lv<KEYS> L;
+    typedef typename L::T V;
     if (sides == 0) sides = SIDE_FULL;
     const int lane = tid & 31, wrp = tid >> 5;
     {
@@ -45,10 +47,10 @@
     }
     __syncthreads();
     if (STAGE && a.use_tma && tid == 0) tma_store_2d(&mapZout, x0, y0, sZ);
-    if constexpr (STAGE && DRAIN_SWEEPS) fill_drain_sweeps<TOPO4>(sW, sZ, y0, a.H, &sFlags, &sKey);
+    if constexpr (STAGE && DRAIN_SWEEPS) fill_drain_sweeps<TOPO4, KEYS>(sW, sZ, y0, a.H, &sFlags, &sKey);
 
     int f = 0;
-    float kmin = __int_as_float(0x7f800000);
+    V kmin = L::of(__int_as_float(0x7f800000));
     int iters = 0;
     int cl = 0;
     bool again = false;
@@ -60,6 +62,9 @@
       nlist += segn[w2];
     }
     while (nlist > 0) {
+#ifdef RDB_FILL_CLOCKS
+      const long long clk_update0 = clock64();
+#endif
       for (int i = tid; i < nlist; i += FILL_THREADS) {
         int seg = 0, off = i;
 #pragma unroll
@@ -72,16 +77,16 @@
         const int b = sList[cl][seg][off];
         const int bx = b % BXN, by = b / BXN;
         const int srow = 4 * by + 1, scol = 4 * bx + PADL;
-        float v[6][6];
-        float z[4][4];
+        V v[6][6];
+        V z[4][4];
         bool at_floor = true;
 #pragma unroll
         for (int j = 0; j < 4; j++) {
           const float4 z4 = *reinterpret_cast<const float4 *>(&sZ[(4 * by + j) * TX + 4 * bx]);
           const float4 m4 = *reinterpret_cast<const float4 *>(&sW[(srow + j) * SP + scol]);
-          z[j][0] = z4.x; z[j][1] = z4.y; z[j][2] = z4.z; z[j][3] = z4.w;
-          v[j + 1][1] = m4.x; v[j + 1][2] = m4.y; v[j + 1][3] = m4.z; v[j + 1][4] = m4.w;
-          at_floor &= (z4.x == m4.x) & (z4.y == m4.y) & (z4.z == m4.z) & (z4.w == m4.w);
+          z[j][0] = L::of(z4.x); z[j][1] = L::of(z4.y); z[j][2] = L::of(z4.z); z[j][3] = L::of(z4.w);
+          v[j + 1][1] = L::of(m4.x); v[j + 1][2] = L::of(m4.y); v[j + 1][3] = L::of(m4.z); v[j + 1][4] = L::of(m4.w);
+          at_floor &= (z[j][0] == v[j + 1][1]) & (z[j][1] == v[j + 1][2]) & (z[j][2] == v[j + 1][3]) & (z[j][3] == v[j + 1][4]);
         }
         if (at_floor) continue;
 #pragma unroll
@@ -89,22 +94,27 @@
           const float *row = &sW[(srow - 1 + j) * SP + scol];
           if (j == 0 || j == 5) {
             const float4 m4 = *reinterpret_cast<const float4 *>(row);
-            v[j][1] = m4.x; v[j][2] = m4.y; v[j][3] = m4.z; v[j][4] = m4.w;
-          }
-          v[j][0] = row[-1];
-          v[j][5] = row[4];
+            v[j][1] = L::of(m4.x); v[j][2] = L::of(m4.y); v[j][3] = L::of(m4.z); v[j][4] = L::of(m4.w);
+          }
+          v[j][0] = L::of(row[-1]);
+          v[j][5] = L::of(row[4]);
         }
         uint32_t ch = 0;
 #pragma unroll
         for (int j = 1; j <= 4; j++) {
 #pragma unroll
           for (int i2 = 1; i2 <= 4; i2++) {
-            const float zz = z[j - 1][i2 - 1];
-            const float others = TOPO4 ? min3f(v[j - 1][i2], v[j + 1][i2], v[j][i2 + 1])
-                                       : min3f(min3f(v[j - 1][i2 - 1], v[j - 1][i2], v[j - 1][i2 + 1]),
-                                               min3f(v[j + 1][i2 - 1], v[j + 1][i2], v[j + 1][i2 + 1]), v[j][i2 + 1]);
-            const float b0 = fminf(v[j][i2], fmaxf(zz, STEP ? others + 1.0f : others));
-            const float nw = fminf(b0, fmaxf(zz, STEP ? v[j][i2 - 1] + 1.0f : v[j][i2 - 1]));
+            const V zz = z[j - 1][i2 - 1];
+            const V others = TOPO4 ? L::mn3(v[j - 1][i2], v[j + 1][i2], v[j][i2 + 1])
+                                   : L::mn3(L::mn3(v[j - 1][i2 - 1], v[j - 1][i2], v[j - 1][i2 + 1]),
+                                            L::mn3(v[j + 1][i2 - 1], v[j + 1][i2], v[j + 1][i2 + 1]), v[j][i2 + 1]);
+            V nw;
+            if constexpr (KEYS) {
+              nw = L::mx(zz, L::mn3(v[j][i2], others, v[j][i2 - 1]));
+            } else {
+              const V b0 = L::mn(v[j][i2], L::mx(zz, step_up<STEP>(others)));
+              nw = L::mn(b0, L::mx(zz, step_up<STEP>(v[j][i2 - 1])));
+            }
             if (nw < v[j][i2]) ch |= 1u << ((j - 1) * 4 + (i2 - 1));
             v[j][i2] = nw;
           }
@@ -113,12 +123,17 @@
         for (int j = 4; j >= 1; j--) {
 #pragma unroll
           for (int i2 = 4; i2 >= 1; i2--) {
-            const float zz = z[j - 1][i2 - 1];
-            const float others = TOPO4 ? min3f(v[j - 1][i2], v[j + 1][i2], v[j][i2 - 1])
-                                       : min3f(min3f(v[j - 1][i2 - 1], v[j - 1][i2], v[j - 1][i2 + 1]),
-                                               min3f(v[j + 1][i2 - 1], v[j + 1][i2], v[j + 1][i2 + 1]), v[j][i2 - 1]);
-            const float b0 = fminf(v[j][i2], fmaxf(zz, STEP ? others + 1.0f : others));
-            const float nw = fminf(b0, fmaxf(zz, STEP ? v[j][i2 + 1] + 1.0f : v[j][i2 + 1]));
+            const V zz = z[j - 1][i2 - 1];
+            const V others = TOPO4 ? L::mn3(v[j - 1][i2], v[j + 1][i2], v[j][i2 - 1])
+                                   : L::mn3(L::mn3(v[j - 1][i2 - 1], v[j - 1][i2], v[j - 1][i2 + 1]),
+                                            L::mn3(v[j + 1][i2 - 1], v[j + 1][i2], v[j + 1][i2 + 1]), v[j][i2 - 1]);
+            V nw;
+            if constexpr (KEYS) {
+              nw = L::mx(zz, L::mn3(v[j][i2], others, v[j][i2 + 1]));
+            } else {
+              const V b0 = L::mn(v[j][i2], L::mx(zz, step_up<STEP>(others)));
+              nw = L::mn(b0, L::mx(zz, step_up<STEP>(v[j][i2 + 1])));
+            }
             if (nw < v[j][i2]) ch |= 1u << ((j - 1) * 4 + (i2 - 1));
             v[j][i2] = nw;
           }
@@ -128,7 +143,7 @@
           for (int j = 0; j < 4; j++) {
             if (ch & (0xFu << (4 * j))) {
               *reinterpret_cast<float4 *>(&sW[(srow + j) * SP + scol]) =
-                  make_float4(v[j + 1][1], v[j + 1][2], v[j + 1][3], v[j + 1][4]);
+                  make_float4(L::to_f(v[j + 1][1]), L::to_f(v[j + 1][2]), L::to_f(v[j + 1][3]), L::to_f(v[j + 1][4]));
             }
           }
           unsigned char *mk = &sMark[(by + 1) * MKP + (bx + 1)];
@@ -161,10 +176,13 @@
             for (int j = 0; j < 4; j++)
 #pragma unroll
               for (int i2 = 0; i2 < 4; i2++)
-                if (ch & (1u << (4 * j + i2))) kmin = fminf(kmin, v[j + 1][i2 + 1]);
-          }
-        }
-      }
+                if (ch & (1u << (4 * j + i2))) kmin = L::mn(kmin, v[j + 1][i2 + 1]);
+          }
+        }
+      }
+#ifdef RDB_FILL_CLOCKS
+      clk_update += clock64() - clk_update0;
+#endif
       if (a.profile && tid == 0) {
         sProf[0] += nlist;
         sProf[1] += (nlist + 31) / 32;
```

Measured after the change: 22840 (median of 6 runs). +2.0%, better.
